# UBC-AWP/vision-sam3-yolo-lameless

Hardware: AMD Instinct MI355X
Metric: frames/sec (whole node) for YOLO+SAM3+DINOv3 feature extraction, 1080p clips (higher is better)
Workload: dtype f16; 1 GPU; BASELINE cfg#5, dense schedule: fused per-frame path on a synthetic 5 s @ 30 fps 1080p clip (150 unique BGR frames resident in HBM): YOLOv8-l detect (letterbox 384x640, NMS, scale_boxes; f16 plan) -> SAM (Hiera-B+ image encoder + FPN at 1024x1024, box-prompted mask decoder, 1080p mask + statistics + contour features) + DINOv3 ViT-L/16 embed (224x224) on EVERY frame; per-frame records packed, gathe; parallelism=one clip per GPU, 1 GPU(s), one gather per step, streams=7

## Files before the change

### include/lmx.h

```cpp
#ifndef LMX_H
#define LMX_H
#include <stdint.h>
#ifdef __cplusplus
extern "C" {
#endif

#define LMX_VERSION 100

#define LMX_OK 0
#define LMX_EINVAL (-1)
#define LMX_EHIP (-2)

typedef void* lmx_stream_t;

int lmx_version(void);
const char* lmx_last_error(void);
int lmx_device_count(void);

enum { LMX_F16 = 0, LMX_F32 = 1 };
enum { LMX_ACT_NONE = 0, LMX_ACT_SILU = 1, LMX_ACT_GELU = 2 , LMX_ACT_RELU = 3,
       LMX_ACT_SWIGLU = 4  };

typedef struct {
  const void* A;
  const void* W;
  const float* bias;
  const float* scale;
  const void* res;
  void* C;
  int64_t lda, ldc, ldr;
  int32_t M, N, K;
  int32_t act;
  int32_t out_dtype;
  int32_t a_mode;
  int32_t H, W_, Cin, conv_stride, Ho, Wo;
  int32_t res_rows;
  int32_t a_rep;
  int32_t split_k;
  int64_t split_stride;
  void* ln_out;
  const float* ln_gamma;
  const float* ln_beta;
  int64_t ld_ln;
  float ln_eps;
} lmx_gemm_desc;
int lmx_k_gemm(const lmx_gemm_desc* d, lmx_stream_t stream);
void lmx_dbg_set_gemm2_variant(int v);
int lmx_h_gemm_route(const lmx_gemm_desc* d, char* name, int cap);

int lmx_k_layernorm(const void* x, int in_dtype, int64_t ldx, const float* gamma, const float* beta,
                    void* y, int out_dtype, int64_t ldy, int rows, int D, float eps, int act, lmx_stream_t stream);
int lmx_h_layernorm_route(int in_dtype, int out_dtype, int rows, int D, int act, char* name, int cap);

int lmx_k_swiglu(const void* gu, int64_t ldg, void* out, int64_t ldo, int rows, int I, lmx_stream_t stream);

int lmx_k_hiera_attn8(const void* h, float* x, int64_t ldx, const float* gamma, const float* beta, float eps, const void* wqkv_p,
                      const float* bqkv_p, const void* wo_p, const float* bo, int n_img, int Gh, int Gw, int D, int heads, float scale,
                      lmx_stream_t stream);

int lmx_k_hiera_attn4(const void* h, float* x, int64_t ldx, const void* w_img, const float* bias, int n_img, int Gh, int Gw, int D,
                      int heads, float scale, lmx_stream_t stream);

int lmx_k_hiera_attn_pool(const void* h, float* out, const void* w_img, const float* bias, int n_img, int Gh, int Gw, int Din, int Dout,
                          int heads, float scale, lmx_stream_t stream);

int lmx_k_ln_mlp(float* x, int64_t ldx, const float* gamma, const float* beta, const void* w1, const float* b1,
                 const void* w2, const float* b2, int64_t rows, int D, float eps, void* workspace, void* x16,
                 const float* gamma_next, const float* beta_next, void* h_next, lmx_stream_t stream);
int lmx_k_ln_mlp_img(float* x, int64_t ldx, const void* w_img, const float* bias, int64_t rows, int D, float eps, void* x16, void* h_next,
                     lmx_stream_t stream);

typedef struct {
  const void* Q; const void* K; const void* V; void* O;
  int64_t ldq, ldk, ldv, ldo;
  int32_t B, H, Tq, Tk, hd;
  float scale;
  int32_t mode;
  int32_t Gh, Gw, ws, q_stride;
  const void* pad_k; const void* pad_v;
  const void* rel; int32_t rel_S;
} lmx_attn_desc;
int lmx_k_attention(const lmx_attn_desc* d, lmx_stream_t stream);
int lmx_h_attn_route(const lmx_attn_desc* d, char* name, int cap);
int lmx_k_relpos_tables(const lmx_attn_desc* d, const float* rel_pos_h, const float* rel_pos_w, int S, void* out,
                        lmx_stream_t stream);

int lmx_k_rope(void* x, int64_t ld, int B, int T, int H, int hd, int n_prefix, const float* cos_t,
               const float* sin_t, lmx_stream_t stream);

int lmx_k_pil_resize_h(const uint8_t* src, uint8_t* dst, int n, int sh, int sw, int dw, const int32_t* bounds,
                       const int32_t* kk, int ksize, int swap_rb, lmx_stream_t stream);
int lmx_k_pil_resize_v(const uint8_t* src, uint8_t* dst, int n, int sh, int dh, int w, const int32_t* bounds,
                       const int32_t* kk, int ksize, lmx_stream_t stream);

int lmx_k_patchify_norm(const uint8_t* img, void* out, int n, int ih, int iw, int top, int left, int gh, int gw,
                        int P, int64_t ldo, const float* lut, lmx_stream_t stream);

// ... 2 lines not shown
                                const float* kk_v, int ksize_v, int seg_cols, float rescale, const float* mean_std,
                                int swap_rb, lmx_stream_t stream);

int lmx_k_assemble_tokens(const void* patch_f16, const float* prefix, const float* pos, float* out, int B, int np,
                          int n_prefix, int D, lmx_stream_t stream);

int lmx_k_token_mean(const void* x, int in_dtype, float* out, int B, int T, int D, lmx_stream_t stream);

int64_t lmx_nms_workspace_bytes(int n, int A);
int lmx_k_nms(const float* pred, int n, int A, int nc, float conf, double iou, int max_det, float max_wh,
              float* boxes, float* scores, int32_t* cls, int32_t* src, int32_t* counts, void* workspace,
              lmx_stream_t stream);

int lmx_k_letterbox(const uint8_t* src, uint8_t* dst, int n, int sh, int sw, int rh, int rw, int top, int left,
                    int oh, int ow, const int32_t* xofs, const int16_t* ialpha, const int32_t* yofs,
                    const int16_t* ibeta, int swap_rb, lmx_stream_t stream);
int lmx_k_stem_conv(const uint8_t* img, const float* w, const float* bias, void* out, int n, int H, int W, int Cout,
                    lmx_stream_t stream);
int lmx_k_maxpool5(const void* src, int64_t lds, void* dst, int64_t ldd, int n, int H, int W, int C,
                   lmx_stream_t stream);
int lmx_k_upsample2(const void* src, int64_t lds, void* dst, int64_t ldd, int n, int H, int W, int C,
                    lmx_stream_t stream);
int lmx_k_detect_decode(const float* head, int64_t ldh, float* pred, int n, int H, int W, int nc, float stride,
                        int a_off, int A, lmx_stream_t stream);
int lmx_k_scale_boxes(float* boxes, int total, float padx, float pady, float gain, float w, float h,
                      lmx_stream_t stream);

int lmx_k_split3(const float* x, int64_t ldx, int act, const void* res3, int64_t ldr, void* out3, int64_t ldo, int64_t rows,
                 int N, int g, int nsum, int64_t sum_stride, lmx_stream_t stream);
int lmx_k_maxpool5_x3(const void* src3, int64_t lds, void* dst3, int64_t ldd, int n, int H, int W, int C, lmx_stream_t stream);
int lmx_k_stem_conv_x3(const uint8_t* img, const float* w, const float* bias, void* out3, int n, int H, int W, int Cout,
                       lmx_stream_t stream);
int lmx_k_attention_f32(const float* q, int64_t ldq, const float* k, int64_t ldk, const float* v, int64_t ldv, float* o,
                        int64_t ldo, int B, int H, int Tq, int Tk, int hd, float scale, lmx_stream_t stream);
int lmx_k_hyper_mask_f32(const float* up, const float* hyper, float* logits, int n, int G, int C, int act, lmx_stream_t stream);

int lmx_k_pose_gather(const float* raw0, const float* raw1, const float* raw2, int64_t ldk, const int32_t* hw,
                      const float* strides, const int32_t* src, const int32_t* counts, int n, int max_det, int K, int ndim,
                      float padx, float pady, float gain, float w, float h, float* out, lmx_stream_t stream);

int lmx_k_im2col_u8(const uint8_t* img, const float* lut, void* out, int n, int rh, int rw, int IH, int IW, int KH,
                    int KW, int stride, int pad, int64_t ldo, lmx_stream_t stream);
int lmx_k_maxpool2(const void* src, int64_t lds, void* dst, int64_t ldd, int dtype, int n, int H, int W, int C,
                   lmx_stream_t stream);
int lmx_k_cast_f32_f16(const float* src, int64_t lds, void* dst, int64_t ldd, int64_t rows, int cols,
                       lmx_stream_t stream);
int lmx_h_hiera_band(const int* window, const int* q_stride, int n_blocks, int grid, int nh, int nw, int* band);
int lmx_h_hiera_bands(const int* window, const int* q_stride, int n_blocks, int grid, int nh, int nw, int* rows);
int lmx_k_band_join(const void* band, const void* table, void* out, int dtype, int n, int H, int Hb, int W, int D,
                    lmx_stream_t stream);

int lmx_k_add_bcast(const void* a, int a_dtype, int64_t lda, const float* b, int64_t ldb, int b_rows, void* out,
                    int out_dtype, int64_t ldo, int64_t rows, int D, lmx_stream_t stream);
int lmx_k_prompt_box(const float* boxes, int64_t ldb, float* sparse, int n, double sx, double sy, float S,
                     const float* gauss, const float* corner, int F, lmx_stream_t stream);
int lmx_k_hyper_mask(const void* up, const float* hyper, float* logits, int n, int G, int C, lmx_stream_t stream);
int lmx_k_mask_post(const float* logits, int n, int L, int T, int nh, int nw, int h, int w, uint8_t* mask,
                    int64_t* stats, float* workspace, lmx_stream_t stream);
int lmx_k_prompt_points(const float* points, const int32_t* labels, int Np, const float* boxes, int64_t ldb, float* sparse, int n,
                        double sx, double sy, float S, const float* gauss, const float* point_embed, const float* not_a_point,
                        const float* corner, int F, lmx_stream_t stream);
#define LMX_MASK_EMBED_PARAMS 4684
int lmx_k_mask_embed(const float* mask_input, const void* emb, int emb_dtype, int64_t lde, const float* params, float* keys,
                     int64_t ldk, int n, int G, lmx_stream_t stream);
int lmx_k_hyper_mask_multi(const void* up, const float* hyper, float* logits, int n, int M, int G, int C, lmx_stream_t stream);
int lmx_k_hyper_mask_multi_f32(const float* up, const float* hyper, float* logits, int n, int M, int G, int C, int act,
                               lmx_stream_t stream);
int lmx_k_mask_logits(const float* logits, int n, int L, int T, int nh, int nw, int h, int w, float* out, lmx_stream_t stream);

int lmx_k_mask_score(const float* logits, int n, int L, int T, int nh, int nw, int h, int w, double thr, double off,
                     const int32_t* idx, int64_t* out, lmx_stream_t stream);
int lmx_k_nms_boxes(const float* boxes, int64_t ldb, const float* scores, const uint8_t* valid, int n, double iou, int32_t* keep_out,
                    int32_t* count_out, void* workspace, lmx_stream_t stream);
int lmx_k_pack_bits(const uint8_t* src, int64_t rows, int w, uint8_t* dst, lmx_stream_t stream);

int64_t lmx_contour_workspace_bytes(int n, int h, int w);
int lmx_k_contour_features(const uint8_t* mask, int n, int h, int w, int64_t* out, void* workspace, lmx_stream_t stream);

int lmx_h_mask_features(const uint8_t* mask_host, int h, int w, double* out_host);

int lmx_h_iou_matrix(const double* a, int n, const double* b, int m, double* out);
int lmx_h_assign(const double* cost, int n, int m, int* row_to_col, int* col_to_row);

enum { LMX_FILT_BILINEAR = 2, LMX_FILT_BICUBIC = 3 };
int lmx_h_pil_tables(int in_size, int out_size, int filt, int32_t* bounds_host, int32_t* kk_host, int64_t cap, int* ksize_host);
int lmx_h_aa_tables(int in_size, int out_size, int filt, int32_t* bounds_host, float* kk_host, int64_t cap, int* ksize_host);
int lmx_h_identity_table(int n, int32_t* bounds_host, int32_t* kk_host);
int lmx_h_segment_cols(const int32_t* bounds_host, int n_out, int tile);

typedef struct lmx_dino lmx_dino;
enum { LMX_DINO_V2 = 0, LMX_DINO_V3 = 1 };
enum { LMX_RECIPE_PIL = 0, LMX_RECIPE_FLOAT = 1 };
typedef struct { int32_t arch, hidden, heads, layers, tokens, image, patch, gated, recipe_kind, max_batch; } lmx_dino_info_t;
int lmx_dino_image_check_host(const char* path_host, lmx_dino_info_t* info_host);
int lmx_dino_open_host(const char* path_host, int max_batch, lmx_dino** out_host);
void lmx_dino_close(lmx_dino* m);
int lmx_dino_info(const lmx_dino* m, lmx_dino_info_t* info_host);
int lmx_dino_prepare(lmx_dino* m, int h, int w);
int lmx_dino_embed(lmx_dino* m, const uint8_t* frames, int n, int h, int w, int rgb, float* emb, lmx_stream_t stream);
int lmx_dino_embed_host(lmx_dino* m, const uint8_t* frames_host, int n, int h, int w, int rgb, float* emb_host);

typedef struct { int32_t sh, sw, rh, rw, top, left, oh, ow; double gain, pad_x, pad_y; } lmx_letterbox_geo_t;
int lmx_h_letterbox_geometry(int sh, int sw, int imgsz, int stride, int auto_, lmx_letterbox_geo_t* out_host);
int lmx_h_letterbox_tables(int sh, int sw, int rh, int rw, int32_t* xofs_host, int16_t* ialpha_host, int32_t* yofs_host, int16_t* ibeta_host);
int lmx_h_conv_split_k(int64_t px_per_frame, int N, int K, int cin);

// ... 22 lines not shown
```

### vision-sam3-yolo-lameless_amd/csrc/attn.hip

```cpp
#include "common.h"
#include <type_traits>
#include <stdlib.h>

#ifdef LMX_DBG_TIMELINE
__device__ unsigned long long lmx_attn_tl[64 * 8 * 8];
extern "C" int lmx_dbg_get_attn_timeline(void* host, int64_t bytes) { return (int)hipMemcpyFromSymbol(host, HIP_SYMBOL(lmx_attn_tl), bytes); }
#define ATL(i) if (blockIdx.x == 0 && lane == 0 && tl_it < 64) lmx_attn_tl[(tl_it * 8 + wave) * 8 + (i)] = __builtin_readcyclecounter()
#else
#define ATL(i)
#endif
namespace {

struct Geo {
  int mode, Tq, Tk, Gh, Gw, ws, nWy, nWx, Gqh, Gqw, wsq;
};

__device__ __forceinline__ int64_t key_row(const Geo& g, int b, int t) {
  if (g.mode == 0) return (int64_t)b * g.Tk + t;
  const int nW = g.nWy * g.nWx;
  const int img = b / nW;
  const int w = b - img * nW;
  const int wy = w / g.nWx, wx = w - wy * g.nWx;
  const int ty = t / g.ws, tx = t - ty * g.ws;
  const int y = wy * g.ws + ty, x = wx * g.ws + tx;
  if (y >= g.Gh || x >= g.Gw) return -1;
  return ((int64_t)img * g.Gh + y) * g.Gw + x;
}
__device__ __forceinline__ int64_t query_row(const Geo& g, int b, int t) {
  if (g.mode == 0) return (int64_t)b * g.Tq + t;
  const int nW = g.nWy * g.nWx;
  const int img = b / nW;
  const int w = b - img * nW;
  const int wy = w / g.nWx, wx = w - wy * g.nWx;
  const int ty = t / g.wsq, tx = t - ty * g.wsq;
  const int y = wy * g.wsq + ty, x = wx * g.wsq + tx;
  if (y >= g.Gqh || x >= g.Gqw) return -1;
  return ((int64_t)img * g.Gqh + y) * g.Gqw + x;
}

typedef __fp16 fp16x4_t __attribute__((__vector_size__(4 * sizeof(__fp16))));
typedef __attribute__((address_space(3))) fp16x4_t* lds_f16x4_ptr;

__device__ __forceinline__ half4_t lds_tr_read(const half_t* p) {
  const fp16x4_t v = __builtin_amdgcn_ds_read_tr16_b64_v4f16((lds_f16x4_ptr)(p));
  half4_t h;
  __builtin_memcpy(&h, &v, 8);
  return h;
}

typedef __attribute__((address_space(3))) const half8_t* lds_h8_cptr;
__device__ __forceinline__ unsigned lds_addr(const half_t* p) {
  unsigned a = (unsigned)(uintptr_t)(__attribute__((address_space(3))) const half_t*)p;
  asm volatile("" : "+v"(a));
  return a;
}
__device__ __forceinline__ half8_t lds_read8(unsigned base, int byte_off) { return *(lds_h8_cptr)(uintptr_t)(base + (unsigned)byte_off); }
__device__ __forceinline__ half4_t lds_tr_read_at(unsigned base, int byte_off) {
  const fp16x4_t v = __builtin_amdgcn_ds_read_tr16_b64_v4f16((lds_f16x4_ptr)(uintptr_t)(base + (unsigned)byte_off));
  half4_t h;
  __builtin_memcpy(&h, &v, 8);
  return h;
}

template <int QB, bool ONES, bool REL, bool DMA, int HDW>
__global__ __launch_bounds__(256, 2) void attn_kernel(const lmx_attn_desc p, const Geo geo, const int nQT) {
#ifndef LMX_ATTN_RING
#define LMX_ATTN_RING 3
#endif
  constexpr int NSL = DMA ? LMX_ATTN_RING : 2;
  constexpr int KS = HDW / 32;
  constexpr int NDB = HDW / 16;
  constexpr int RW = HDW <= 64 ? 64 : 128;
  constexpr int CPR = RW / 8;
  constexpr int NPASS = 64 * CPR / 256;
  static_assert(!(DMA && HDW != 64) && !(ONES && HDW != 64), "LDS-DMA ring and the ones column are built for 64-wide rows");
  __shared__ __attribute__((aligned(16))) half_t Ks[NSL][64 * RW];
  __shared__ __attribute__((aligned(16))) half_t Vs[NSL][64 * RW];
  static_assert(!(DMA && REL), "the relative-position bias is read from global memory inside the loop: vmcnt would not count DMAs only");

  const int tid = threadIdx.x, lane = tid & 63, wave = tid >> 6;
  const int fr = lane & 15, fg = lane >> 4;

  int bid;
  {
    const int n = gridDim.x, xcd = blockIdx.x & 7, idx = blockIdx.x >> 3, q = n >> 3, r = n & 7;
    bid = (xcd < r ? xcd * (q + 1) : r * (q + 1) + (xcd - r) * q) + idx;
  }
  const int nQTa = nQT < 0 ? -nQT : nQT;
  const int qt = bid % nQTa;
  bid /= nQTa;
  const int h = bid % p.H;
  const int b = bid / p.H;

  const half_t* Q = reinterpret_cast<const half_t*>(p.Q);
  const half_t* K = reinterpret_cast<const half_t*>(p.K);
  const half_t* V = reinterpret_cast<const half_t*>(p.V);
  const half_t* padk = reinterpret_cast<const half_t*>(p.pad_k);
  const half_t* padv = reinterpret_cast<const half_t*>(p.pad_v);
  half_t* O = reinterpret_cast<half_t*>(p.O);
  const int hd = p.hd;
  const half8_t zero8 = {0, 0, 0, 0, 0, 0, 0, 0};

  const int q_base = qt * (64 * QB) + wave * (16 * QB);
  half8_t qf[QB][KS];
  int64_t qrow[QB];
#pragma unroll
  for (int qb = 0; qb < QB; ++qb) {
    const int tq = q_base + qb * 16 + fr;
    qrow[qb] = (tq < p.Tq) ? query_row(geo, b, tq) : -1;
#pragma unroll
    for (int ks = 0; ks < KS; ++ks) {
      const int d = ks * 32 + fg * 8;
      const bool ok = qrow[qb] >= 0 && d < hd;
      const half8_t qv = *reinterpret_cast<const half8_t*>(Q + (ok ? qrow[qb] * p.ldq + (int64_t)h * hd + d : 0));
      qf[qb][ks] = ok ? qv : zero8;
    }
  }

  const half_t* relq[QB];
#pragma unroll
  for (int qb = 0; qb < QB; ++qb) {
    const int tq = q_base + qb * 16 + fr;
    relq[qb] = REL ? reinterpret_cast<const half_t*>(p.rel) + (((int64_t)b * p.H + h) * p.Tq + (tq < p.Tq ? tq : 0)) * (2 * p.rel_S)
                   : nullptr;
  }

  f32x4 oacc[QB][NDB];
  float m_run[QB], l_run[QB];
#pragma unroll
  for (int qb = 0; qb < QB; ++qb) {
    m_run[qb] = -INFINITY;
    l_run[qb] = 0.f;
#pragma unroll
    for (int db = 0; db < NDB; ++db) oacc[qb][db] = f32x4{0.f, 0.f, 0.f, 0.f};
  }

  const int sc = tid & (CPR - 1);
  const int sk = tid / CPR;
  constexpr int KPP = 256 / CPR;
  half8_t kst[NPASS], vst[NPASS];
  const int64_t hoff0 = (int64_t)h * hd + sc * 8;
  const half_t* Kb = K + hoff0 + (geo.mode == 0 ? (int64_t)b * p.Tk * p.ldk : 0);
  const half_t* Vb = V + hoff0 + (geo.mode == 0 ? (int64_t)b * p.Tk * p.ldv : 0);
  const bool d_ok = sc * 8 < hd;
  auto load_tile = [&](int t0) {
    if (geo.mode == 0) {
#pragma unroll
      for (int i = 0; i < NPASS; ++i) {
        const int t = t0 + sk + KPP * i;
        const bool in = d_ok && t < p.Tk;
        const int tt = in ? t : 0;
        const half8_t kv = *reinterpret_cast<const half8_t*>(Kb + (int64_t)tt * p.ldk);
        const half8_t vv = *reinterpret_cast<const half8_t*>(Vb + (int64_t)tt * p.ldv);
        kst[i] = in ? kv : zero8;
        vst[i] = in ? vv : zero8;
        if (ONES && sc == 7 && t < p.Tk) vst[i][7] = (half_t)1.0f;
      }
      return;
    }
#pragma unroll
    for (int i = 0; i < NPASS; ++i) {
      const int t = t0 + sk + KPP * i;
      const int d = sc * 8;
      const bool in = (t < p.Tk) && (d < hd);
      const int64_t row = key_row(geo, b, in ? t : 0);
      const bool pad = row < 0;
      const int64_t hoff = (int64_t)h * hd + d;
      const half_t* kp = pad ? (padk ? padk + hoff : K) : K + (in ? row * p.ldk + hoff : 0);
      const half_t* vp = pad ? (padv ? padv + hoff : V) : V + (in ? row * p.ldv + hoff : 0);
      const half8_t kv = *reinterpret_cast<const half8_t*>(kp);
      const half8_t vv = *reinterpret_cast<const half8_t*>(vp);
      kst[i] = (in && (!pad || padk)) ? kv : zero8;
      vst[i] = (in && (!pad || padv)) ? vv : zero8;
      if (ONES && sc == 7 && t < p.Tk) vst[i][7] = (half_t)1.0f;
    }
  };
  auto store_tile = [&](int buf) {
#pragma unroll
    for (int i = 0; i < NPASS; ++i) {
      const int kk = sk + KPP * i;
      const int off = kk * RW + ((sc ^ (kk & (CPR - 1))) << 3);
      *reinterpret_cast<half8_t*>(&Ks[buf][off]) = kst[i];
      *reinterpret_cast<half8_t*>(&Vs[buf][off]) = vst[i];
    }
  };

  const float sl2 = REL ? 1.44269504088896340736f : p.scale * 1.44269504088896340736f;
  const int ntile = (p.Tk + 63) / 64;
  const int q4 = fr >> 2, p4 = fr & 3;
  constexpr int LA = DMA ? NSL - 1 : 2, PT = 4;
  __amdgpu_buffer_rsrc_t k_rs, v_rs;
  unsigned kvo[2], vvo[2];
  if constexpr (DMA) {
    const int64_t kb = ((int64_t)(p.Tk - 1) * p.ldk + hd) * 2, vb = ((int64_t)(p.Tk - 1) * p.ldv + hd) * 2;
    k_rs = __builtin_amdgcn_make_buffer_rsrc(const_cast<half_t*>(K + (int64_t)b * p.Tk * p.ldk + (int64_t)h * hd), 0, (int)kb, 0x00020000);
    v_rs = __builtin_amdgcn_make_buffer_rsrc(const_cast<half_t*>(V + (int64_t)b * p.Tk * p.ldv + (int64_t)h * hd), 0, (int)vb, 0x00020000);
#pragma unroll
    for (int j = 0; j < 2; ++j) {
      const int row = (wave * 2 + j) * 8 + (lane >> 3);
      const int lc = (lane & 7) ^ (row & 7);
      const bool ok = lc * 8 < hd;
      kvo[j] = ok ? (unsigned)(row * (int)p.ldk * 2 + lc * 16) : 0x80000000u;
      vvo[j] = ok ? (unsigned)(row * (int)p.ldv * 2 + lc * 16) : 0x80000000u;
    }
  }
  auto issue = [&](int it, int slot) {
    const unsigned ko = (unsigned)(it * 64 * (int)p.ldk * 2), vo = (unsigned)(it * 64 * (int)p.ldv * 2);
#pragma unroll
    for (int j = 0; j < 2; ++j) {
      lds_dma16(k_rs, reinterpret_cast<char*>(&Ks[slot][0]) + (wave * 2 + j) * 1024, kvo[j] == 0x80000000u ? kvo[j] : kvo[j] + ko, 0);
      lds_dma16(v_rs, reinterpret_cast<char*>(&Vs[slot][0]) + (wave * 2 + j) * 1024, vvo[j] == 0x80000000u ? vvo[j] : vvo[j] + vo, 0);
    }
  };
  if constexpr (DMA) {
#pragma unroll
    for (int t = 0; t < LA; ++t)
      if (t < ntile) issue(t, t);
  } else {
    load_tile(0);
    store_tile(0);
    __syncthreads();
  }
  int k_lane[KS], v_lane[NDB];
#pragma unroll
  for (int ks = 0; ks < KS; ++ks) k_lane[ks] = fr * RW + ((((ks << 2) + fg) ^ (fr & (CPR - 1))) << 3);
#pragma unroll
  for (int db = 0; db < NDB; ++db) {
    const int chunk = db * 2 + (p4 >> 1), rl = fg * 4 + q4;
    v_lane[db] = rl * RW + ((chunk ^ (rl & (CPR - 1))) << 3) + (p4 & 1) * 4;
  }
  auto tile_body = [&](const int it, auto mask_tag) {
    constexpr bool MASK = decltype(mask_tag)::value;
    const int t0 = it * 64;
    int buf;
    if constexpr (DMA) {
      const int left = ntile - 1 - it;
      wait_tiles<PT>(left < LA - 1 ? left : LA - 1);
      __builtin_amdgcn_s_barrier();
      if (it + LA < ntile) issue(it + LA, (it + LA) % NSL);
      buf = it % NSL;
    } else {
      buf = it & 1;
      if (it + 1 < ntile) load_tile(t0 + 64);
    }

    unsigned kbase[KS], vbase[NDB];
#pragma unroll
    for (int ks = 0; ks < KS; ++ks) kbase[ks] = lds_addr(&Ks[buf][k_lane[ks]]);
#pragma unroll
    for (int db = 0; db < NDB; ++db) vbase[db] = lds_addr(&Vs[buf][v_lane[db]]);

    f32x4 sacc[QB][4];
#pragma unroll
    for (int qb = 0; qb < QB; ++qb)
#pragma unroll
      for (int kb = 0; kb < 4; ++kb) sacc[qb][kb] = f32x4{0.f, 0.f, 0.f, 0.f};
#pragma unroll
    for (int ks = 0; ks < KS; ++ks) {
#pragma unroll
      for (int kb = 0; kb < 4; ++kb) {
        const half8_t kf = lds_read8(kbase[ks], kb * 16 * RW * 2);
#pragma unroll
        for (int qb = 0; qb < QB; ++qb)
          sacc[qb][kb] = __builtin_amdgcn_mfma_f32_16x16x32_f16(kf, qf[qb][ks], sacc[qb][kb], 0, 0, 0);
      }
    }

    half8_t pf[QB][2];
#pragma unroll
    for (int qb = 0; qb < QB; ++qb) {
      if (REL) {
        if (p.rel_S == 64) {
          const float by = (float)relq[qb][it];
#pragma unroll
          for (int kb = 0; kb < 4; ++kb) {
            const half4_t bx = *reinterpret_cast<const half4_t*>(relq[qb] + 64 + kb * 16 + fg * 4);
#pragma unroll
            for (int r = 0; r < 4; ++r) sacc[qb][kb][r] = fmaf(sacc[qb][kb][r], p.scale, by + (float)bx[r]);
          }
        } else {
#pragma unroll
          for (int kb = 0; kb < 4; ++kb)
#pragma unroll
            for (int r = 0; r < 4; ++r) {
              int key = t0 + kb * 16 + fg * 4 + r;
              key = key < p.Tk ? key : 0;
              const int ky = key / p.rel_S, kx = key - ky * p.rel_S;
              const float bias = (float)relq[qb][ky] + (float)relq[qb][p.rel_S + kx];
              sacc[qb][kb][r] = fmaf(sacc[qb][kb][r], p.scale, bias);
            }
        }
      }
      if (MASK) {
#pragma unroll
        for (int kb = 0; kb < 4; ++kb)
#pragma unroll
          for (int r = 0; r < 4; ++r)
            if (t0 + kb * 16 + fg * 4 + r >= p.Tk) sacc[qb][kb][r] = -INFINITY;
      }
      float mx = fmaxf(fmaxf(sacc[qb][0][0], sacc[qb][0][1]), fmaxf(sacc[qb][0][2], sacc[qb][0][3]));
#pragma unroll
      for (int kb = 1; kb < 4; ++kb)
        mx = fmaxf(mx, fmaxf(fmaxf(sacc[qb][kb][0], sacc[qb][kb][1]), fmaxf(sacc[qb][kb][2], sacc[qb][kb][3])));
      mx = fmaxf(mx, __shfl_xor(mx, 16, 64));
      mx = fmaxf(mx, __shfl_xor(mx, 32, 64));
      const float m_new = fmaxf(m_run[qb], mx);
      const bool grew = nQT < 0 || __builtin_amdgcn_ballot_w64(m_new > m_run[qb]) != 0;
      const float alpha = grew ? __builtin_amdgcn_exp2f((m_run[qb] - m_new) * sl2) : 1.0f;
      m_run[qb] = m_new;
      const float mb = m_new * sl2;
      float rs = 0.f;
      const half2_t ones2 = {(half_t)1.0f, (half_t)1.0f};
#pragma unroll
      for (int kb = 0; kb < 4; ++kb)
#pragma unroll
        for (int r = 0; r < 4; r += 2) {
          const float e0 = __builtin_amdgcn_exp2f(fmaf(sacc[qb][kb][r], sl2, -mb));
          const float e1 = __builtin_amdgcn_exp2f(fmaf(sacc[qb][kb][r + 1], sl2, -mb));
          const half2_t e = {(half_t)e0, (half_t)e1};
          if (!ONES) rs = __builtin_amdgcn_fdot2(e, ones2, rs, false);
          pf[qb][kb >> 1][(kb & 1) * 4 + r] = e[0];
          pf[qb][kb >> 1][(kb & 1) * 4 + r + 1] = e[1];
        }
      if (!ONES) l_run[qb] = l_run[qb] * alpha + rs;
      if (grew) {
#pragma unroll
        for (int db = 0; db < NDB; ++db) oacc[qb][db] *= alpha;
      }
    }

#pragma unroll
    for (int ks = 0; ks < 2; ++ks) {
#pragma unroll
      for (int db = 0; db < NDB; ++db) {
        const half4_t lo = lds_tr_read_at(vbase[db], ks * 32 * RW * 2);
        const half4_t hi = lds_tr_read_at(vbase[db], (ks * 32 + 16) * RW * 2);
        half8_t vf = {lo[0], lo[1], lo[2], lo[3], hi[0], hi[1], hi[2], hi[3]};
        if (DMA && ONES && db == 3) {
          const half_t one = (half_t)1.0f;
          const half8_t ones8 = {one, one, one, one, one, one, one, one};
          vf = fr == 15 ? ones8 : vf;
        }
#pragma unroll
        for (int qb = 0; qb < QB; ++qb)
          oacc[qb][db] = __builtin_amdgcn_mfma_f32_16x16x32_f16(vf, pf[qb][ks], oacc[qb][db], 0, 0, 0);
      }
    }

    if constexpr (!DMA) {
      if (it + 1 < ntile) store_tile(buf ^ 1);
      __syncthreads();
    }
  };
  for (int it = 0; it + 1 < ntile; ++it) tile_body(it, std::false_type{});
  if (p.Tk & 63)
    tile_body(ntile - 1, std::true_type{});
  else
    tile_body(ntile - 1, std::false_type{});

#pragma unroll
  for (int qb = 0; qb < QB; ++qb) {
    float l;
    if (ONES) {
      l = __shfl(oacc[qb][3][3], 48 + fr, 64);
    } else {
      l = l_run[qb];
      l += __shfl_xor(l, 16, 64);
      l += __shfl_xor(l, 32, 64);
    }
    const float inv = 1.0f / l;
    if (qrow[qb] < 0) continue;
#pragma unroll
    for (int db = 0; db < NDB; ++db) {
      const int d = db * 16 + fg * 4;
      if (d >= hd) continue;
      half4_t o;
#pragma unroll
      for (int r = 0; r < 4; ++r) o[r] = (half_t)(oacc[qb][db][r] * inv);
      *reinterpret_cast<half4_t*>(O + qrow[qb] * p.ldo + (int64_t)h * hd + d) = o;
    }
  }
}


__device__ __forceinline__ float vmax3(float a, float b, float c) {
  return __builtin_amdgcn_fmed3f(__builtin_amdgcn_fmed3f(a, b, INFINITY), c, INFINITY);
}
__device__ __forceinline__ float row_max4(float ma, float mc) {
  typedef unsigned u32x2 __attribute__((ext_vector_type(2)));
  const unsigned u = __builtin_bit_cast(unsigned, fmaxf(ma, mc));
  const u32x2 a = __builtin_amdgcn_permlane16_swap(u, u, false, false);
  const unsigned a0 = a[0], a1 = a[1];
  const unsigned u1 = __builtin_bit_cast(unsigned, fmaxf(__builtin_bit_cast(float, a0), __builtin_bit_cast(float, a1)));
  const u32x2 b = __builtin_amdgcn_permlane32_swap(u1, u1, false, false);
  const unsigned b0 = b[0], b1 = b[1];
  return fmaxf(__builtin_bit_cast(float, b0), __builtin_bit_cast(float, b1));
}

#ifndef LMX_GP_DBG
#define LMX_GP_DBG 0
#endif
typedef unsigned u32x2_t __attribute__((ext_vector_type(2)));
typedef unsigned u32x4_t __attribute__((ext_vector_type(4)));
template <bool ONES, int NWV>
__global__ __launch_bounds__(NWV * 64, 2) void attn_gp_kernel(const lmx_attn_desc p, const int nQT) {
  constexpr int QB = 2, NSL = 3, RW = 64, NJ = 8 / NWV, PT = 2 * NJ;
  extern __shared__ __attribute__((aligned(16))) char smem[];
  half_t (*Ks)[64 * RW] = reinterpret_cast<half_t (*)[64 * RW]>(smem);
  half_t (*Vs)[64 * RW] = reinterpret_cast<half_t (*)[64 * RW]>(smem + NSL * 64 * RW * 2);
  const int tid = threadIdx.x, lane = tid & 63, wave = tid >> 6;
  const int fr = lane & 15, fg = lane >> 4;
// ... 881 lines not shown
        const float inv = 1.0f / l;
        if (qrow[qb] < 0) continue;
#pragma unroll
        for (int db = 0; db < 4; ++db) {
          const int d = db * 16 + fg * 4;
          if (d >= hd) continue;
          half4_t o;
#pragma unroll
          for (int r = 0; r < 4; ++r) o[r] = (half_t)(oacc[qb][db][r] * inv);
          *reinterpret_cast<half4_t*>(O + qrow[qb] * p.ldo + (int64_t)h * hd + d) = o;
        }
      }
      ATL(7);
    } else {
      asm volatile("s_waitcnt vmcnt(0)" ::: "memory");
      ATL(7);
    }
  }
}

}

static int build_geo(const lmx_attn_desc& d, Geo& g);

extern "C" int lmx_k_relpos_tables(const lmx_attn_desc* dp, const float* rel_pos_h, const float* rel_pos_w, int S, void* out,
                                   lmx_stream_t stream) {
  LMX_REQUIRE(dp && rel_pos_h && rel_pos_w && out, "lmx_k_relpos_tables: null pointer");
  const lmx_attn_desc& d = *dp;
  LMX_REQUIRE(d.Q && d.B > 0 && d.H > 0 && d.Tq > 0 && d.hd % 8 == 0 && d.hd <= 96 && d.ldq % 8 == 0 && aligned16(d.Q),
              "lmx_k_relpos_tables: descriptor");
  LMX_REQUIRE(S > 0 && S * S == d.Tq, "lmx_k_relpos_tables: S=%d vs Tq=%d", S, d.Tq);
  Geo g{};
  const int rc = build_geo(d, g);
  if (rc) return rc;
  const int64_t items = (int64_t)d.B * d.H * 2 * S;
  const int64_t grid = (items + 3) / 4;
  LMX_REQUIRE(grid < (1ll << 31) && aligned16(rel_pos_h) && aligned16(rel_pos_w), "lmx_k_relpos_tables: size / alignment");
  hipStream_t st = reinterpret_cast<hipStream_t>(stream);
  if (d.hd <= 64)
    hipLaunchKernelGGL((relpos_tables_kernel<2>), dim3((unsigned)grid), dim3(256), 0, st, d, g, rel_pos_h, rel_pos_w, S,
                       reinterpret_cast<half_t*>(out), items);
  else
    hipLaunchKernelGGL((relpos_tables_kernel<3>), dim3((unsigned)grid), dim3(256), 0, st, d, g, rel_pos_h, rel_pos_w, S,
                       reinterpret_cast<half_t*>(out), items);
  return lmx_launch_check("relpos_tables_kernel");
}

enum AttnKernel { ATTN_SMALL, ATTN_SP, ATTN_SPP, ATTN_GP, ATTN_TILED };
struct AttnRoute {
  AttnKernel kernel;
  int QB = 1;
  bool ONES = false, REL = false, DMA = false;
  int HDW = 64, NWV = 4;
  unsigned grid = 0, block = 256;
  int lds = 0;
  int arg = 0;
};

static int attn_route(const lmx_attn_desc* dp, AttnRoute& r, Geo& g) {
  LMX_REQUIRE(dp != nullptr, "lmx_k_attention: null descriptor");
  const lmx_attn_desc& d = *dp;
  LMX_REQUIRE(d.Q && d.K && d.V && d.O, "lmx_k_attention: null Q/K/V/O");
  LMX_REQUIRE(d.B > 0 && d.H > 0 && d.Tq > 0 && d.Tk > 0, "lmx_k_attention: empty problem");
  LMX_REQUIRE(d.hd % 8 == 0 && d.hd > 0 && d.hd <= 96, "lmx_k_attention: head dim %d (need multiple of 8, <=96)", d.hd);
  LMX_REQUIRE(d.ldq % 8 == 0 && d.ldk % 8 == 0 && d.ldv % 8 == 0 && d.ldo % 4 == 0, "lmx_k_attention: strides");
  LMX_REQUIRE(aligned16(d.Q) && aligned16(d.K) && aligned16(d.V) && ((((uintptr_t)d.O) & 7) == 0),
              "lmx_k_attention: alignment");
  LMX_TRY(build_geo(d, g));
  static const int no_sp = lmx_env_set("LMX_ATTN_NO_SP"), sp_qb = lmx_env_int("LMX_ATTN_SP_QB", 2), no_spp = lmx_env_set("LMX_ATTN_NO_SPP");
  static const int no_dma = lmx_env_set("LMX_ATTN_NO_DMA"), no_lazy = lmx_env_set("LMX_ATTN_NO_LAZY");
  static const int no_gp = lmx_env_set("LMX_ATTN_NO_GP");
  static const int gp_waves = lmx_env_int("LMX_ATTN_GP_WAVES", 4);

  r = AttnRoute{};
  r.ONES = d.hd <= 56;
  const int64_t items = (int64_t)d.B * d.H;
  const bool narrow = !d.rel && d.hd <= 64;
  if (narrow && d.Tq <= 16 && d.Tk <= 16) {
    LMX_REQUIRE(items < (1ll << 31), "lmx_k_attention: grid too large");
    r.kernel = ATTN_SMALL;
    r.ONES = false;
    r.grid = (unsigned)((items + 3) / 4);
    r.arg = (int)items;
    return LMX_OK;
  }
  if (!no_sp && narrow && d.Tk > 128 && d.Tk <= 208 && d.Tq > 64 && d.Tq <= 208) {
    LMX_REQUIRE(items < (1ll << 31), "lmx_k_attention: grid too large");
    r.grid = (unsigned)items;
    if (!no_spp && items >= 64 && (d.mode == 0 || (d.pad_k && d.pad_v))) {
      r.kernel = ATTN_SPP;
      r.block = 512;
      r.lds = 2 * 3 * 208 * 64 * 2;
      r.arg = (int)items;
    } else {
      r.kernel = ATTN_SP;
      r.QB = sp_qb == 2 ? 2 : 1;
    }
    return LMX_OK;
  }
  const bool wide = d.hd > 64;
  const bool big = d.Tq > 64 && !wide;
  const int nQT = (d.Tq + (big ? 128 : 64) - 1) / (big ? 128 : 64);
  const int64_t nblk = items * nQT;
  LMX_REQUIRE(nblk < (1ll << 31), "lmx_k_attention: grid too large");
  if (d.rel)
    LMX_REQUIRE(d.rel_S > 0 && d.rel_S * d.rel_S == d.Tk && d.Tq == d.Tk, "lmx_k_attention: rel_S=%d does not match Tq=%d Tk=%d",
                d.rel_S, d.Tq, d.Tk);
  const bool dma = !no_dma && !wide && d.mode == 0 && !d.rel && big && d.Tk >= 256 && (int64_t)d.Tk * d.ldk * 2 < 0x7fff0000ll &&
                   (int64_t)d.Tk * d.ldv * 2 < 0x7fff0000ll;
  if (dma && !no_gp) {
    r.kernel = ATTN_GP;
    r.NWV = gp_waves == 8 ? 8 : 4;
    const int nQTw = (d.Tq + r.NWV * 32 - 1) / (r.NWV * 32);
    r.grid = (unsigned)(items * nQTw);
    r.block = r.NWV * 64;
    r.lds = 2 * 3 * 64 * 64 * 2;
    r.arg = no_lazy ? -nQTw : nQTw;
    return LMX_OK;
  }
  r.kernel = ATTN_TILED;
  r.QB = big ? 2 : 1;
  r.ONES = r.ONES && !d.rel;
  r.REL = d.rel != nullptr;
  r.DMA = dma;
  r.HDW = wide ? 96 : 64;
  r.grid = (unsigned)nblk;
  r.arg = no_lazy ? -nQT : nQT;
  return LMX_OK;
}

static constexpr int attn_key(int kernel, int QB, bool ONES, bool REL, bool DMA, int HDW, int NWV) {
  return (((((kernel * 4 + QB) * 2 + ONES) * 2 + REL) * 2 + DMA) * 128 + HDW) * 16 + NWV;
}

extern "C" int lmx_k_attention(const lmx_attn_desc* dp, lmx_stream_t stream) {
  AttnRoute r;
  Geo g{};
  LMX_TRY(attn_route(dp, r, g));
  const lmx_attn_desc& d = *dp;
  hipStream_t st = reinterpret_cast<hipStream_t>(stream);
  const dim3 block(r.block);
  dim3 grid(r.grid);
  if (r.kernel == ATTN_SPP) {
    int dev;
    LMX_TRY(lmx_stream_device(st, &dev));
    LMX_TRY(lmx_allow_lds(reinterpret_cast<const void*>(&attn_spp_kernel<true>), r.lds, dev));
    LMX_TRY(lmx_allow_lds(reinterpret_cast<const void*>(&attn_spp_kernel<false>), r.lds, dev));
    LMX_TRY(lmx_persistent_grid(r.grid, dev, &grid.x));
  }
#define LMX_SP(QB, ONES) \
  case attn_key(ATTN_SP, QB, ONES, false, false, 64, 4): hipLaunchKernelGGL((attn_sp_kernel<QB, ONES>), grid, block, 0, st, d, g); break
#define LMX_SPP(ONES) \
  case attn_key(ATTN_SPP, 1, ONES, false, false, 64, 4): hipLaunchKernelGGL((attn_spp_kernel<ONES>), grid, block, r.lds, st, d, g, r.arg); break
#define LMX_GP(ONES, NWV) \
  case attn_key(ATTN_GP, 1, ONES, false, false, 64, NWV): hipLaunchKernelGGL((attn_gp_kernel<ONES, NWV>), grid, block, r.lds, st, d, r.arg); break
#define LMX_TILED(QB, ONES, REL, DMA, HDW) \
  case attn_key(ATTN_TILED, QB, ONES, REL, DMA, HDW, 4): hipLaunchKernelGGL((attn_kernel<QB, ONES, REL, DMA, HDW>), grid, block, 0, st, d, g, r.arg); break
  switch (attn_key(r.kernel, r.QB, r.ONES, r.REL, r.DMA, r.HDW, r.NWV)) {
    case attn_key(ATTN_SMALL, 1, false, false, false, 64, 4): hipLaunchKernelGGL(attn_small_kernel, grid, block, 0, st, d, g, r.arg); break;
    LMX_SPP(true);
    LMX_SPP(false);
    LMX_SP(2, true);
    LMX_SP(1, true);
    LMX_SP(2, false);
    LMX_SP(1, false);
    LMX_TILED(1, false, true, false, 96);
    LMX_TILED(2, false, true, false, 64);
    LMX_TILED(1, false, true, false, 64);
    LMX_TILED(1, false, false, false, 96);
    LMX_GP(true, 8);
    LMX_GP(true, 4);
    LMX_GP(false, 8);
    LMX_GP(false, 4);
    LMX_TILED(2, true, false, true, 64);
    LMX_TILED(2, false, false, true, 64);
    LMX_TILED(2, true, false, false, 64);
    LMX_TILED(2, false, false, false, 64);
    LMX_TILED(1, true, false, false, 64);
    LMX_TILED(1, false, false, false, 64);
    default: LMX_REQUIRE(false, "lmx_k_attention: no kernel for route %d", (int)r.kernel);
  }
#undef LMX_SP
#undef LMX_SPP
#undef LMX_GP
#undef LMX_TILED
  static const char* const what[] = {"attn_small_kernel", "attn_sp_kernel", "attn_spp_kernel", "attn_gp_kernel", "attn_kernel"};
  return lmx_launch_check(what[r.kernel]);
}

extern "C" int lmx_h_attn_route(const lmx_attn_desc* dp, char* name, int cap) {
  AttnRoute r;
  Geo g{};
  LMX_TRY(attn_route(dp, r, g));
  const char* sums = r.ONES ? "ones" : "dot2";
  switch (r.kernel) {
    case ATTN_SMALL: LMX_ROUTE_NAME(name, cap, "small"); break;
    case ATTN_SP: LMX_ROUTE_NAME(name, cap, "sp_qb%d_%s", r.QB, sums); break;
    case ATTN_SPP: LMX_ROUTE_NAME(name, cap, "spp_%s", sums); break;
    case ATTN_GP: LMX_ROUTE_NAME(name, cap, "gp%d_%s", r.NWV, sums); break;
    case ATTN_TILED:
      LMX_ROUTE_NAME(name, cap, "tiled_q%d_%s%s%s_hd%d", r.QB, sums, r.REL ? "_rel" : "", r.DMA ? "_dma" : "", r.HDW);
      break;
  }
  return LMX_OK;
}

static int build_geo(const lmx_attn_desc& d, Geo& g) {
  g.mode = d.mode;
  g.Tq = d.Tq;
  g.Tk = d.Tk;
  if (d.mode == 1) {
    LMX_REQUIRE(d.ws > 0 && d.Gh > 0 && d.Gw > 0, "lmx_k_attention: window geometry");
    const int qs = d.q_stride > 0 ? d.q_stride : 1;
    LMX_REQUIRE(qs == 1 || qs == 2, "lmx_k_attention: q_stride %d", qs);
    LMX_REQUIRE(d.ws % qs == 0 && d.Gh % qs == 0 && d.Gw % qs == 0, "lmx_k_attention: q_stride must divide ws/Gh/Gw");
    g.Gh = d.Gh;
    g.Gw = d.Gw;
    g.ws = d.ws;
    g.nWy = (d.Gh + d.ws - 1) / d.ws;
    g.nWx = (d.Gw + d.ws - 1) / d.ws;
    g.Gqh = d.Gh / qs;
    g.Gqw = d.Gw / qs;
    g.wsq = d.ws / qs;
    LMX_REQUIRE(d.Tk == d.ws * d.ws && d.Tq == g.wsq * g.wsq, "lmx_k_attention: Tq/Tk do not match window size");
    LMX_REQUIRE(d.B % (g.nWy * g.nWx) == 0, "lmx_k_attention: B=%d not a multiple of windows per image %d", d.B,
                g.nWy * g.nWx);
    if (d.pad_k) LMX_REQUIRE(aligned16(d.pad_k), "lmx_k_attention: pad_k alignment");
    if (d.pad_v) LMX_REQUIRE(aligned16(d.pad_v), "lmx_k_attention: pad_v alignment");
  } else {
    LMX_REQUIRE(d.mode == 0, "lmx_k_attention: bad mode %d", d.mode);
  }
  return LMX_OK;
}
```

### vision-sam3-yolo-lameless_amd/csrc/gemm.hip

```cpp
#include "common.h"
#include <stdlib.h>

namespace {

constexpr int BK = 64;

template <int BM, int BN, int AMODE, int OUT_DT>
__global__ __launch_bounds__(256, 2) void gemm_kernel(const lmx_gemm_desc p) {
  extern __shared__ __attribute__((aligned(16))) char smem[];
  half_t* As = reinterpret_cast<half_t*>(smem);
  half_t* Ws = As + 2 * BM * BK;
  constexpr int FM = BM / 32;
  constexpr int FN = BN / 32;
  constexpr int AI = BM / 32;
  constexpr int WI = BN / 32;

  const int tid = threadIdx.x;
  const int lane = tid & 63;
  const int wave = tid >> 6;
  const int wm = wave & 1, wn = wave >> 1;

  const int nwg = gridDim.x;
  const int bid = blockIdx.x;
  const int q = nwg >> 3, r = nwg & 7, xcd = bid & 7;
// ... 174 lines not shown
#pragma unroll
        for (int e = 0; e < 4; ++e) v[e] = __fmul_rn(v[e], s[e]);
      }
      if (OUT_DT == LMX_F32) {
        float* C = reinterpret_cast<float*>(p.C);
        if (p.res) {
          const f32x4 rr = *reinterpret_cast<const f32x4*>(reinterpret_cast<const float*>(p.res) + (int64_t)mr * p.ldr + n);
#pragma unroll
          for (int e = 0; e < 4; ++e) v[e] = __fadd_rn(v[e], rr[e]);
        }
        *reinterpret_cast<f32x4*>(C + (int64_t)m * p.ldc + n) = v;
      } else {
        half_t* C = reinterpret_cast<half_t*>(p.C);
        if (p.res) {
          const half4_t rr =
              *reinterpret_cast<const half4_t*>(reinterpret_cast<const half_t*>(p.res) + (int64_t)mr * p.ldr + n);
#pragma unroll
          for (int e = 0; e < 4; ++e) v[e] = __fadd_rn((float)(half_t)v[e], (float)rr[e]);
        }
        half4_t o;
#pragma unroll
        for (int e = 0; e < 4; ++e) o[e] = (half_t)v[e];
        *reinterpret_cast<half4_t*>(C + (int64_t)m * p.ldc + n) = o;
      }
    }
  }
}

template <int BM, int BN, int AMODE, int OUT_DT>
int launch(const lmx_gemm_desc& d, hipStream_t st) {
  const int MT = (d.M + BM - 1) / BM, NT = (d.N + BN - 1) / BN;
  const size_t smem = (size_t)2 * (BM + BN) * BK * sizeof(half_t);
  int dev;
  LMX_TRY(lmx_stream_device(st, &dev));
  LMX_TRY(lmx_allow_lds(reinterpret_cast<const void*>(&gemm_kernel<BM, BN, AMODE, OUT_DT>), (int)smem, dev));
  hipLaunchKernelGGL((gemm_kernel<BM, BN, AMODE, OUT_DT>), dim3(MT * NT), dim3(256), smem, st, d);
  return lmx_launch_check("gemm_kernel");
}

}

GemmRoute lmx_gemm2_tiling(const lmx_gemm_desc& d);
int lmx_gemm2_launch(const lmx_gemm_desc& d, const GemmRoute& r, hipStream_t st);

static bool dma_ok(const lmx_gemm_desc& d, int m_min, int n_min) {
  const bool a_ok = d.a_mode != 1 || (d.Cin % 32 == 0 && d.H < 32768 && d.W_ < 32768);
  return a_ok && d.M >= m_min && d.N >= n_min && d.N % 8 == 0 && d.ldc % 8 == 0 && aligned16(d.C) &&
         (!d.res || (d.ldr % 8 == 0 && aligned16(d.res)));
}

static int gemm_route(const lmx_gemm_desc* dp, GemmRoute& r) {
  LMX_REQUIRE(dp != nullptr, "lmx_k_gemm: null descriptor");
  const lmx_gemm_desc& d = *dp;
  LMX_REQUIRE(d.A && d.W && d.C, "lmx_k_gemm: null A/W/C");
  LMX_REQUIRE(d.M > 0 && d.N > 0 && d.K > 0, "lmx_k_gemm: empty problem M=%d N=%d K=%d", d.M, d.N, d.K);
  LMX_REQUIRE(d.K % 8 == 0, "lmx_k_gemm: K=%d must be a multiple of 8", d.K);
  LMX_REQUIRE(d.N % 4 == 0, "lmx_k_gemm: N=%d must be a multiple of 4", d.N);
  LMX_REQUIRE(d.lda % 8 == 0, "lmx_k_gemm: lda=%lld must be a multiple of 8", (long long)d.lda);
  const bool gated = d.act == LMX_ACT_SWIGLU;
  LMX_REQUIRE(d.ldc % 4 == 0 && d.ldc >= (gated ? d.N / 2 : d.N), "lmx_k_gemm: bad ldc=%lld", (long long)d.ldc);
  LMX_REQUIRE(aligned16(d.A) && aligned16(d.W), "lmx_k_gemm: A/W must be 16-byte aligned");
  LMX_REQUIRE((((uintptr_t)d.C) & 7) == 0, "lmx_k_gemm: C must be 8-byte aligned");
  LMX_REQUIRE(d.out_dtype == LMX_F16 || d.out_dtype == LMX_F32, "lmx_k_gemm: bad out_dtype %d", d.out_dtype);
  LMX_REQUIRE(d.out_dtype == LMX_F16 || aligned16(d.C), "lmx_k_gemm: f32 C must be 16-byte aligned");
  LMX_REQUIRE(d.act >= LMX_ACT_NONE && d.act <= LMX_ACT_SWIGLU, "lmx_k_gemm: bad act %d", d.act);
  if (gated) {
    LMX_REQUIRE(d.N % 32 == 0, "lmx_k_gemm: LMX_ACT_SWIGLU: N=%d (gate + up rows, interleaved by 16) must be a multiple of 32", d.N);
    LMX_REQUIRE(!d.res, "lmx_k_gemm: LMX_ACT_SWIGLU takes no residual");
    LMX_REQUIRE(d.a_mode == 0 && d.a_rep <= 1 && d.split_k <= 1, "lmx_k_gemm: LMX_ACT_SWIGLU: dense A only (a_mode 0; no pooled rows, convolution, a_rep or split_k); a_mode=%d", d.a_mode);
    LMX_REQUIRE(d.out_dtype == LMX_F16, "lmx_k_gemm: LMX_ACT_SWIGLU writes f16 (one rounding of the f32 product)");
  }
  if (d.bias) LMX_REQUIRE(aligned16(d.bias), "lmx_k_gemm: bias must be 16-byte aligned");
  if (d.scale) LMX_REQUIRE(aligned16(d.scale), "lmx_k_gemm: scale must be 16-byte aligned");
  if (d.res) LMX_REQUIRE(d.ldr % 4 == 0 && d.ldr >= d.N, "lmx_k_gemm: bad ldr=%lld", (long long)d.ldr);
  LMX_REQUIRE(d.res_rows >= 0, "lmx_k_gemm: res_rows");
  if (d.a_mode == 0) {
    LMX_REQUIRE(d.a_rep > 1 || d.lda >= d.K, "lmx_k_gemm: lda=%lld < K=%d", (long long)d.lda, d.K);
  } else if (d.a_mode == 1) {
    LMX_REQUIRE(d.Cin > 0 && d.Cin % 8 == 0, "lmx_k_gemm: conv Cin=%d must be a multiple of 8", d.Cin);
    LMX_REQUIRE(d.K == 9 * d.Cin, "lmx_k_gemm: conv K=%d != 9*Cin=%d", d.K, 9 * d.Cin);
    LMX_REQUIRE(d.conv_stride == 1 || d.conv_stride == 2, "lmx_k_gemm: conv stride %d", d.conv_stride);
    LMX_REQUIRE(d.H > 0 && d.W_ > 0, "lmx_k_gemm: conv H/W");
    LMX_REQUIRE(d.Ho == (d.H + 2 - 3) / d.conv_stride + 1 && d.Wo == (d.W_ + 2 - 3) / d.conv_stride + 1,
                "lmx_k_gemm: conv Ho/Wo (%d,%d) inconsistent with H/W (%d,%d) stride %d", d.Ho, d.Wo, d.H, d.W_,
                d.conv_stride);
    LMX_REQUIRE(d.M % (d.Ho * d.Wo) == 0, "lmx_k_gemm: conv M=%d not a multiple of Ho*Wo", d.M);
    LMX_REQUIRE(d.lda >= d.Cin, "lmx_k_gemm: conv pixel stride lda=%lld < Cin=%d", (long long)d.lda, d.Cin);
  } else if (d.a_mode == 2) {
    LMX_REQUIRE(d.lda >= d.K, "lmx_k_gemm: lda=%lld < K=%d", (long long)d.lda, d.K);
    LMX_REQUIRE(d.H > 0 && d.W_ > 0 && d.H % 2 == 0 && d.W_ % 2 == 0 && d.M % (d.H * d.W_) == 0,
                "lmx_k_gemm: pooled rows need an even H x W token grid that divides M (H=%d W=%d M=%d)", d.H, d.W_, d.M);
    LMX_REQUIRE(!d.res && !d.scale && d.act == LMX_ACT_NONE, "lmx_k_gemm: pooled rows: no residual / scale / activation");
    LMX_REQUIRE(((int64_t)d.M * d.lda + d.K) * 2 < 0x7fffffffll, "lmx_k_gemm: pooled rows: A must be smaller than 2 GB");
    LMX_REQUIRE(dma_ok(d, 512, 96),
                "lmx_k_gemm: pooled rows are built for the LDS-DMA kernel (M >= 512, N >= 96, N %% 8 == 0): use GEMM + maxpool2 for M=%d N=%d", d.M, d.N);
  } else {
    LMX_REQUIRE(false, "lmx_k_gemm: bad a_mode %d", d.a_mode);
  }
  LMX_REQUIRE(d.a_rep >= 0 && d.a_rep <= 3, "lmx_k_gemm: a_rep=%d (0..3)", d.a_rep);
  LMX_REQUIRE(d.split_k >= 0 && d.split_k <= 64, "lmx_k_gemm: split_k=%d (0..64)", d.split_k);
  static const int v1 = lmx_env_char("LMX_GEMM_V1") == '1';
  static const int n64 = lmx_env_char("LMX_GEMM_N64") != '0';
  if (d.ln_out) {
    LMX_REQUIRE(d.out_dtype == LMX_F32 && d.res && d.res_rows == 0, "lmx_k_gemm: ln_out needs f32 output with a full residual (out_dtype=%d res_rows=%d)", d.out_dtype, d.res_rows);
    LMX_REQUIRE(d.N <= 448 && d.N % 16 == 0 && d.K <= 448, "lmx_k_gemm: ln_out: a tile holds whole rows of N <= 448 (N %% 16 == 0) over K <= 448; N=%d K=%d", d.N, d.K);
    LMX_REQUIRE(d.a_mode == 0 && d.a_rep <= 1 && d.split_k <= 1, "lmx_k_gemm: ln_out: dense A only (a_mode=%d a_rep=%d split_k=%d)", d.a_mode, d.a_rep, d.split_k);
    LMX_REQUIRE(d.act == LMX_ACT_NONE && !d.scale, "lmx_k_gemm: ln_out takes no activation and no scale");
    LMX_REQUIRE(d.ln_gamma && d.ln_beta && aligned16(d.ln_gamma) && aligned16(d.ln_beta), "lmx_k_gemm: ln_gamma / ln_beta must be given, 16-byte aligned");
    LMX_REQUIRE(d.ld_ln % 4 == 0 && d.ld_ln >= d.N && (((uintptr_t)d.ln_out) & 7) == 0, "lmx_k_gemm: ln_out must be 8-byte aligned with ld_ln=%lld a multiple of 4, >= N", (long long)d.ld_ln);
    LMX_REQUIRE(aligned16(d.res), "lmx_k_gemm: ln_out: the residual must be 16-byte aligned");
    r = GemmRoute{true, 128, 448, BK, 2, 0, true};
    return LMX_OK;
  }
  bool dma;
  if (d.split_k > 1) {
    LMX_REQUIRE(d.out_dtype == LMX_F32 && d.act == LMX_ACT_NONE && d.a_mode != 2 && d.a_rep <= 1, "lmx_k_gemm: split_k needs f32 output, no activation, a_mode 0 or 1");
    LMX_REQUIRE(d.split_stride >= (int64_t)(d.M - 1) * d.ldc + d.N && d.split_stride % 4 == 0, "lmx_k_gemm: split_stride=%lld", (long long)d.split_stride);
    LMX_REQUIRE((d.K + 63) / 64 >= d.split_k, "lmx_k_gemm: split_k=%d exceeds the k-tiles of K=%d", d.split_k, d.K);
    LMX_REQUIRE(dma_ok(d, 1, 64),
                "lmx_k_gemm: split_k is built into the LDS-DMA kernel only (N >= 64, N %% 8 == 0; conv: Cin %% 32 == 0); M=%d N=%d", d.M, d.N);
    dma = true;
  } else if (d.a_rep > 1) {
    LMX_REQUIRE(d.a_mode == 0 && d.K % d.a_rep == 0 && (d.K / d.a_rep) % 64 == 0, "lmx_k_gemm: a_rep=%d needs a_mode 0 and K / a_rep a multiple of 64 (K=%d)", d.a_rep, d.K);
    LMX_REQUIRE(d.lda >= d.K / d.a_rep, "lmx_k_gemm: lda=%lld < K / a_rep", (long long)d.lda);
    LMX_REQUIRE(dma_ok(d, 512, 96),
                "lmx_k_gemm: a_rep is built into the LDS-DMA kernel only (M >= 512, N >= 96, N %% 8 == 0); M=%d N=%d", d.M, d.N);
    dma = true;
  } else if (d.a_mode == 2) {
    dma = true;
  } else {
    dma = !v1 && dma_ok(d, 512, d.a_mode == 1 && n64 && d.M >= 65536 ? 64 : 96);
  }
  if (dma) {
    r = lmx_gemm2_tiling(d);
  } else {
    const bool narrow = d.N <= 64 || (d.N < 128 && d.N % 128 != 0);
    r = GemmRoute{false, 128, narrow ? 64 : 128, BK, 2, 0};
  }
  return LMX_OK;
}

static constexpr int v1_key(int BN, int a_mode, int out_dtype) { return BN * 4 + a_mode * 2 + out_dtype; }

extern "C" int lmx_k_gemm(const lmx_gemm_desc* dp, lmx_stream_t stream) {
  GemmRoute r;
  LMX_TRY(gemm_route(dp, r));
  const lmx_gemm_desc& d = *dp;
  hipStream_t st = reinterpret_cast<hipStream_t>(stream);
  if (r.dma) return lmx_gemm2_launch(d, r, st);
#define LMX_V1(BN, AMODE, OUT_DT) \
  case v1_key(BN, AMODE, OUT_DT): return launch<128, BN, AMODE, OUT_DT>(d, st)
  switch (v1_key(r.BN, d.a_mode, d.out_dtype)) {
    LMX_V1(64, 0, LMX_F16);
    LMX_V1(128, 0, LMX_F16);
    LMX_V1(64, 0, LMX_F32);
    LMX_V1(128, 0, LMX_F32);
    LMX_V1(64, 1, LMX_F16);
    LMX_V1(128, 1, LMX_F16);
    LMX_V1(64, 1, LMX_F32);
    LMX_V1(128, 1, LMX_F32);
  }
#undef LMX_V1
  LMX_REQUIRE(false, "lmx_k_gemm: no register-staged kernel 128x%d for a_mode %d, out_dtype %d", r.BN, d.a_mode, d.out_dtype);
// ... 14 lines not shown
```

### vision-sam3-yolo-lameless_amd/csrc/gemm2.hip

```cpp
#include "common.h"
#include <stdlib.h>
#include <type_traits>

#ifdef LMX_DBG_TIMELINE
__device__ unsigned long long lmx_tl[8 * 16384];
extern "C" int lmx_dbg_get_timeline(void* host, int64_t bytes) { return (int)hipMemcpyFromSymbol(host, HIP_SYMBOL(lmx_tl), bytes); }
#define TL(i, v) if (threadIdx.x == 0 && swz < 16384) lmx_tl[swz * 8 + (i)] = (v)
#else
#define TL(i, v)
#endif
namespace lmx_gemm2 {

__device__ __forceinline__ float act_apply(float v, int act) { return lmx_act(v, act); }

constexpr int smem_bytes(int BM, int BN, int BK, int NSTAGE) { return NSTAGE * (BM + BN) * BK * 2 + 2 * BN * 4; }
constexpr int waves_per_simd(int BM, int BN, int BK, int NSTAGE) {
  const int smem = smem_bytes(BM, BN, BK, NSTAGE), nwave = (BM / 64) * (BN / 64);
  const int wps = (smem <= 80 * 1024 ? 2 : 1) * nwave / 4;
  return wps < 1 ? 1 : wps;
}
template <int OUT_DT, int BM, int BN, int BK, int NSTAGE, int AMODE, int STAG, bool GATED = false>
__global__ __launch_bounds__(waves_per_simd(BM, BN, BK, NSTAGE) * 256) void gemm2_kernel(const lmx_gemm_desc p, const int ntiles, const int nt_ok) {
  constexpr int NWAVE = (BM / 64) * (BN / 64);
  constexpr int STAGE_BYTES = (BM + BN) * BK * 2;
// ... 408 lines not shown
    }
  }
  __builtin_amdgcn_s_barrier();
  TL(4, wall_clock64());
  }
}

template <int BM, int BN, int BK, int NSTAGE, int AMODE, int STAG = 0>
int launch2(const lmx_gemm_desc& d, hipStream_t st) {
  const int MT = (d.M + BM - 1) / BM, NT = (d.N + BN - 1) / BN;
  const size_t smem = smem_bytes(BM, BN, BK, NSTAGE);
  int dev;
  LMX_TRY(lmx_stream_device(st, &dev));
  LMX_TRY(lmx_allow_lds(reinterpret_cast<const void*>(&gemm2_kernel<LMX_F16, BM, BN, BK, NSTAGE, AMODE, STAG>), (int)smem, dev));
  LMX_TRY(lmx_allow_lds(reinterpret_cast<const void*>(&gemm2_kernel<LMX_F32, BM, BN, BK, NSTAGE, AMODE, STAG>), (int)smem, dev));
  const int ntiles = MT * NT * (d.split_k > 1 ? d.split_k : 1);
  int grid = ntiles;
  static const int persist = lmx_env_int("LMX_GEMM2_PERSIST", 0);
  static const int nt_ok = !lmx_env_set("LMX_GEMM2_NO_NT");
  if (persist > 0 && grid > 256 * persist) grid = 256 * persist;
  if (d.act == LMX_ACT_SWIGLU) {
    if constexpr (AMODE == 0) {
      LMX_TRY(lmx_allow_lds(reinterpret_cast<const void*>(&gemm2_kernel<LMX_F16, BM, BN, BK, NSTAGE, AMODE, STAG, true>), (int)smem, dev));
      hipLaunchKernelGGL((gemm2_kernel<LMX_F16, BM, BN, BK, NSTAGE, AMODE, STAG, true>), dim3(grid), dim3(BM * BN / 64), smem, st, d, ntiles, nt_ok);
      return lmx_launch_check("gemm2_kernel (gated)");
    } else {
      return LMX_EINVAL;
    }
  }
  if (d.out_dtype == LMX_F16)
    hipLaunchKernelGGL((gemm2_kernel<LMX_F16, BM, BN, BK, NSTAGE, AMODE, STAG>), dim3(grid), dim3(BM * BN / 64), smem, st, d, ntiles, nt_ok);
  else
    hipLaunchKernelGGL((gemm2_kernel<LMX_F32, BM, BN, BK, NSTAGE, AMODE, STAG>), dim3(grid), dim3(BM * BN / 64), smem, st, d, ntiles, nt_ok);
  return lmx_launch_check("gemm2_kernel");
}

constexpr int RL_BM = 128, RL_BN = 448, RL_BK = 64, RL_NSTAGE = 2;
constexpr int RL_STAGE_BYTES = (RL_BM + RL_BN) * RL_BK * 2;
constexpr int RL_RS = RL_BN + 4;
constexpr int RL_SMEM = RL_NSTAGE * RL_STAGE_BYTES + 3 * RL_BN * 4;
static_assert(2 * 32 * RL_RS * 4 <= RL_NSTAGE * RL_STAGE_BYTES, "two 32-row epilogue buffers inside the ring");

__device__ __forceinline__ void wave_sum4(float (&v)[4]) {
#pragma unroll
  for (int o = 32; o > 0; o >>= 1) {
    float t[4];
#pragma unroll
    for (int r = 0; r < 4; ++r) t[r] = __shfl_xor(v[r], o, 64);
#pragma unroll
    for (int r = 0; r < 4; ++r) v[r] += t[r];
  }
}

__global__ __launch_bounds__(512) void gemm2_rowln_kernel(const lmx_gemm_desc p) {
  constexpr int BM = RL_BM, BN = RL_BN, BK = RL_BK, NSTAGE = RL_NSTAGE, STAGE_BYTES = RL_STAGE_BYTES;
  constexpr int NWAVE = 8;
  constexpr int A_INSTR = BM * BK * 2 / 1024 / NWAVE;
  constexpr int W_INSTR = BN * BK * 2 / 1024 / NWAVE;
  constexpr int FJ = BN / 4 / 16;
  extern __shared__ __attribute__((aligned(16))) char smem[];
  const int tid = threadIdx.x;
  const int lane = tid & 63;
  const int wave = __builtin_amdgcn_readfirstlane(tid >> 6);
  const int wm = wave & 1, wn = wave >> 1;
  const int swz = blockIdx.x;
  const int m0 = swz * BM;
  TL(0, (unsigned long long)__builtin_amdgcn_s_getreg((31 << 11) | 4));
  TL(1, (unsigned long long)__builtin_amdgcn_s_getreg((31 << 11) | 20));
  TL(2, wall_clock64());
  TL(5, (unsigned long long)swz);

  const char* Ab = reinterpret_cast<const char*>(p.A) + (int64_t)m0 * p.lda * 2;
  int64_t a_bytes = ((int64_t)(p.M - m0 - 1) * p.lda + p.K) * 2;
  if (a_bytes > 0x7FFFFFF0ll) a_bytes = 0x7FFFFFF0ll;
  const int w_bytes = p.N * p.K * 2;
  const __amdgpu_buffer_rsrc_t a_rs = __builtin_amdgcn_make_buffer_rsrc(const_cast<char*>(Ab), 0, (int)a_bytes, 0x00020000);
  const __amdgpu_buffer_rsrc_t w_rs = __builtin_amdgcn_make_buffer_rsrc(const_cast<void*>(p.W), 0, w_bytes, 0x00020000);

  const int lrow = lane >> 3;
  const int lchunk = (lane & 7) ^ lrow;
  unsigned a_off[A_INSTR], w_off[W_INSTR];
#pragma unroll
  for (int j = 0; j < A_INSTR; ++j) a_off[j] = (unsigned)(((wave * A_INSTR + j) * 8 + lrow) * (int)p.lda * 2 + lchunk * 16);
#pragma unroll
  for (int j = 0; j < W_INSTR; ++j) w_off[j] = (unsigned)(((wave * W_INSTR + j) * 8 + lrow) * p.K * 2 + lchunk * 16);
  const unsigned OOB = 0x80000000u;
  const int nk = (p.K + BK - 1) / BK;
  const bool k_tail_lane = (nk - 1) * BK + lchunk * 8 >= p.K;
  auto issue = [&](int kt, int slot) {
    char* st = smem + slot * STAGE_BYTES;
    const bool kill = (kt == nk - 1) && k_tail_lane;
    const int soff = kt * (BK * 2);
#pragma unroll
    for (int j = 0; j < A_INSTR; ++j) lds_dma16(a_rs, st + (wave * A_INSTR + j) * 1024, kill ? OOB : a_off[j], soff);
#pragma unroll
    for (int j = 0; j < W_INSTR; ++j) lds_dma16(w_rs, st + BM * BK * 2 + (wave * W_INSTR + j) * 1024, kill ? OOB : w_off[j], soff);
  };

  f32x4 acc[4][FJ];
#pragma unroll
  for (int i = 0; i < 4; ++i)
#pragma unroll
    for (int j = 0; j < FJ; ++j) acc[i][j] = f32x4{0.f, 0.f, 0.f, 0.f};

  float* bl = reinterpret_cast<float*>(smem + NSTAGE * STAGE_BYTES);
  float bias_v = 0.f, gamma_v = 0.f, beta_v = 0.f;
  if (tid < p.N) {
    if (p.bias) bias_v = p.bias[tid];
    gamma_v = p.ln_gamma[tid];
    beta_v = p.ln_beta[tid];
  }

  issue(0, 0);
  const int frow = lane & 15, fq = lane >> 4;
  const int fsw = frow & 7;
  for (int kt = 0; kt < nk; ++kt) {
    wait_vmcnt<0>();
    __builtin_amdgcn_s_barrier();
    if (kt + 1 < nk) issue(kt + 1, (kt + 1) % NSTAGE);
    const char* st = smem + (kt % NSTAGE) * STAGE_BYTES;
    const half_t* as = reinterpret_cast<const half_t*>(st) + (wm * 64 + frow) * BK;
    const half_t* ws = reinterpret_cast<const half_t*>(st + BM * BK * 2) + (wn * (BN / 4) + frow) * BK;
#pragma unroll
    for (int ks = 0; ks < BK / 32; ++ks) {
      const int coff = (((ks << 2) + fq) ^ fsw) << 3;
      half8_t af[4], wf[FJ];
#pragma unroll
      for (int j = 0; j < FJ; ++j) wf[j] = *reinterpret_cast<const half8_t*>(ws + j * 16 * BK + coff);
#pragma unroll
      for (int i = 0; i < 4; ++i) af[i] = *reinterpret_cast<const half8_t*>(as + i * 16 * BK + coff);
      __builtin_amdgcn_s_setprio(1);
#pragma unroll
      for (int i = 0; i < 4; ++i)
#pragma unroll
        for (int j = 0; j < FJ; ++j)
          acc[i][j] = __builtin_amdgcn_mfma_f32_16x16x32_f16(wf[j], af[i], acc[i][j], 0, 0, 0);
      __builtin_amdgcn_s_setprio(0);
    }
  }

  if (tid < BN) {
    bl[tid] = bias_v;
    bl[BN + tid] = gamma_v;
    bl[2 * BN + tid] = beta_v;
  }
  asm volatile("s_waitcnt lgkmcnt(0)" ::: "memory");
  __builtin_amdgcn_s_barrier();
  TL(3, wall_clock64());

  const int D = p.N;
  const int c0 = lane * 4, c1 = (64 + lane) * 4;
  const bool ok0 = c0 < D, ok1 = c1 < D;
  const f32x4 z4 = {0.f, 0.f, 0.f, 0.f};
  const f32x4 g0 = ok0 ? *reinterpret_cast<const f32x4*>(bl + BN + c0) : z4, g1 = ok1 ? *reinterpret_cast<const f32x4*>(bl + BN + c1) : z4;
  const f32x4 b0 = ok0 ? *reinterpret_cast<const f32x4*>(bl + 2 * BN + c0) : z4, b1 = ok1 ? *reinterpret_cast<const f32x4*>(bl + 2 * BN + c1) : z4;
  const float* blj = bl + wn * (BN / 4) + fq * 4;
  const float* res = reinterpret_cast<const float*>(p.res);
  float* Cf = reinterpret_cast<float*>(p.C);
  half_t* Lh = reinterpret_cast<half_t*>(p.ln_out);
#pragma unroll
  for (int ps = 0; ps < 4; ++ps) {
    float* buf = reinterpret_cast<float*>(smem) + (ps & 1) * 32 * RL_RS;
    f32x4 r0[4], r1[4];
#pragma unroll
    for (int rr = 0; rr < 4; ++rr) {
      const int lr = wave * 4 + rr;
      const int m = m0 + (lr >> 4) * 64 + ps * 16 + (lr & 15);
      r0[rr] = r1[rr] = z4;
      if (m < p.M) {
        if (ok0) r0[rr] = *reinterpret_cast<const f32x4*>(res + (int64_t)m * p.ldr + c0);
        if (ok1) r1[rr] = *reinterpret_cast<const f32x4*>(res + (int64_t)m * p.ldr + c1);
      }
    }
#pragma unroll
    for (int j = 0; j < FJ; ++j)
      *reinterpret_cast<f32x4*>(buf + (wm * 16 + frow) * RL_RS + wn * (BN / 4) + j * 16 + fq * 4) = acc[ps][j] + *reinterpret_cast<const f32x4*>(blj + j * 16);
    asm volatile("s_waitcnt lgkmcnt(0)" ::: "memory");
    __builtin_amdgcn_s_barrier();
    f32x4 v0[4], v1[4];
    float s[4], q[4], mean[4], rstd[4];
#pragma unroll
    for (int rr = 0; rr < 4; ++rr) {
      const int lr = wave * 4 + rr;
      const f32x4 t0 = *reinterpret_cast<const f32x4*>(buf + lr * RL_RS + (ok0 ? c0 : 0)), t1 = *reinterpret_cast<const f32x4*>(buf + lr * RL_RS + (ok1 ? c1 : 0));
      v0[rr] = (ok0 ? t0 : z4) + r0[rr];
      v1[rr] = (ok1 ? t1 : z4) + r1[rr];
      s[rr] = 0.f;
      s[rr] += (v0[rr][0] + v0[rr][1]) + (v0[rr][2] + v0[rr][3]);
      s[rr] += (v1[rr][0] + v1[rr][1]) + (v1[rr][2] + v1[rr][3]);
    }
    wave_sum4(s);
#pragma unroll
    for (int rr = 0; rr < 4; ++rr) {
      mean[rr] = s[rr] / (float)D;
      q[rr] = 0.f;
      {
        const f32x4 dlt = v0[rr] - mean[rr];
        const float t = (dlt[0] * dlt[0] + dlt[1] * dlt[1]) + (dlt[2] * dlt[2] + dlt[3] * dlt[3]);
        q[rr] += ok0 ? t : 0.f;
      }
      {
        const f32x4 dlt = v1[rr] - mean[rr];
        const float t = (dlt[0] * dlt[0] + dlt[1] * dlt[1]) + (dlt[2] * dlt[2] + dlt[3] * dlt[3]);
        q[rr] += ok1 ? t : 0.f;
      }
    }
    wave_sum4(q);
#pragma unroll
    for (int rr = 0; rr < 4; ++rr) {
      const int lr = wave * 4 + rr;
      const int m = m0 + (lr >> 4) * 64 + ps * 16 + (lr & 15);
      rstd[rr] = 1.0f / sqrtf(q[rr] / (float)D + p.ln_eps);
      if (m < p.M) {
        if (ok0) *reinterpret_cast<f32x4*>(Cf + (int64_t)m * p.ldc + c0) = v0[rr];
        if (ok1) *reinterpret_cast<f32x4*>(Cf + (int64_t)m * p.ldc + c1) = v1[rr];
        if (ok0) {
          const f32x4 o = (v0[rr] - mean[rr]) * rstd[rr] * g0 + b0;
          *reinterpret_cast<half4_t*>(Lh + (int64_t)m * p.ld_ln + c0) = half4_t{(half_t)o[0], (half_t)o[1], (half_t)o[2], (half_t)o[3]};
        }
        if (ok1) {
          const f32x4 o = (v1[rr] - mean[rr]) * rstd[rr] * g1 + b1;
          *reinterpret_cast<half4_t*>(Lh + (int64_t)m * p.ld_ln + c1) = half4_t{(half_t)o[0], (half_t)o[1], (half_t)o[2], (half_t)o[3]};
        }
      }
    }
  }
  TL(4, wall_clock64());
}

int launch_rowln(const lmx_gemm_desc& d, hipStream_t st) {
  int dev;
  LMX_TRY(lmx_stream_device(st, &dev));
  LMX_TRY(lmx_allow_lds(reinterpret_cast<const void*>(&gemm2_rowln_kernel), RL_SMEM, dev));
  hipLaunchKernelGGL(gemm2_rowln_kernel, dim3((d.M + RL_BM - 1) / RL_BM), dim3(512), RL_SMEM, st, d);
  return lmx_launch_check("gemm2_rowln_kernel");
}

}
using namespace lmx_gemm2;

static int g_variant = -1;
extern "C" void lmx_dbg_set_gemm2_variant(int v) { g_variant = v; }

static constexpr GemmRoute tiling(int BM, int BN, int BK, int NSTAGE, int STAG = 0) { return GemmRoute{true, BM, BN, BK, NSTAGE, STAG}; }

GemmRoute lmx_gemm2_tiling(const lmx_gemm_desc& d) {
  if (g_variant < 0) g_variant = lmx_env_char("LMX_GEMM2_VARIANT");
  if (d.a_mode == 2) return tiling(256, 256, 64, 2);
  if (d.a_mode == 1) {
    static const int conv_small = lmx_env_set("LMX_GEMM2_CONV_SMALL");
    const int64_t t256 = (int64_t)((d.M + 255) / 256) * ((d.N + 255) / 256);
    const double q256 = (double)t256 / (double)(((t256 + 255) / 256) * 256);
    if (!conv_small && d.N % 256 == 0 && t256 >= 230 && q256 >= 0.75) return tiling(256, 256, 32, 3, 1);
    return tiling(256, 128, 32, 3);
  }
  switch (g_variant) {
    case 'A': return tiling(256, 128, 64, 3);
    case 'B': return tiling(128, 128, 64, 2);
    case 'C': return tiling(256, 128, 32, 3);
    case 'D': return tiling(256, 128, 32, 2);
    case 'E': return tiling(256, 256, 32, 3);
    case 'F': return tiling(256, 256, 32, 4);
    case 'H': return tiling(128, 128, 32, 2);
    case 'I': return tiling(128, 128, 32, 3);
    case 'S': return tiling(256, 128, 32, 6, 1);
    case 'T': return tiling(256, 128, 64, 3, 1);
    case 'U': return tiling(256, 128, 32, 3, 1);
    case 'V': return tiling(256, 128, 32, 4, 1);
    case 'W': return tiling(256, 256, 32, 4, 1);
    case 'Y': return tiling(256, 256, 32, 3, 1);
    case 'Z': return tiling(256, 256, 64, 2);
  }
  const int64_t nt256 = (d.N + 255) / 256, tiles256 = (int64_t)((d.M + 255) / 256) * nt256;
  const double nfrac = (double)d.N / (double)(nt256 * 256);
  const double q256 = (double)tiles256 / (double)(((tiles256 + 255) / 256) * 256);
  if (d.K >= 448 && tiles256 >= 200 && q256 >= 0.75 && nfrac >= 0.85) {
    return tiling(256, 256, 64, 2);
  }
  if (d.K < 448 && d.N >= 224 && d.N <= 1536 && d.N % 256 != 0 && nfrac >= 0.85 && tiles256 >= 200 && q256 >= 0.75)
    return d.K > 128 ? tiling(256, 256, 32, 3) : tiling(256, 256, 64, 2);
  const int64_t tiles = (int64_t)((d.M + 255) / 256) * ((d.N + 127) / 128);
  return (d.K >= 1792 || tiles <= 256) ? tiling(256, 128, 64, 3, 1) : tiling(256, 128, 32, 3);
}

static constexpr int64_t tiling_key(int BM, int BN, int BK, int NSTAGE, int a_mode, int STAG) {
  return ((((int64_t)BM * 1024 + BN) * 1024 + BK) * 16 + NSTAGE) * 16 + a_mode * 2 + STAG;
}
// ... 29 lines not shown
```

### vision-sam3-yolo-lameless_amd/csrc/sam.hip

```cpp
#include "common.h"

namespace {

inline int grid_for(int64_t total, int block = 256) {
  int64_t g = (total + block - 1) / block;
  if (g > 256 * 8) g = 256 * 8;
  if (g < 1) g = 1;
  return (int)g;
}

template <int KW_T>
__global__ __launch_bounds__(256) void im2col_u8_kernel(const uint8_t* __restrict__ img, const float* __restrict__ lut,
                                                        half_t* __restrict__ out, int n, int rh, int rw, int OH, int OW, int KH,
                                                        int KW_rt, int stride, int pad, int64_t ldo) {
  __shared__ float lut_s[768];
  for (int i = threadIdx.x; i < 768; i += blockDim.x) lut_s[i] = lut[i];
  __syncthreads();
  const int KW = KW_T > 0 ? KW_T : KW_rt;
  const int chunks = (int)(ldo / 8);
  const int K = KH * KW * 3;
  const int64_t total = (int64_t)n * OH * OW * chunks;
  for (int64_t i = (int64_t)blockIdx.x * blockDim.x + threadIdx.x; i < total; i += (int64_t)gridDim.x * blockDim.x) {
    const int ck = (int)(i % chunks);
    const int64_t tok = i / chunks;
// ... 42 lines not shown
    for (int e = 0; e < VEC; ++e) {
      T t0 = a0[e] > a1[e] ? a0[e] : a1[e];
      T t1 = a2[e] > a3[e] ? a2[e] : a3[e];
      m[e] = t0 > t1 ? t0 : t1;
    }
    *reinterpret_cast<vec_t*>(dst + p * ldd + c) = m;
  }
}

__global__ __launch_bounds__(256) void cast_kernel(const float* __restrict__ src, int64_t lds, half_t* __restrict__ dst, int64_t ldd,
                                                   int64_t rows, int cols) {
  const int cc = cols / 4;
  const int64_t total = rows * cc;
  for (int64_t i = (int64_t)blockIdx.x * blockDim.x + threadIdx.x; i < total; i += (int64_t)gridDim.x * blockDim.x) {
    const int c = (int)(i % cc) * 4;
    const int64_t r = i / cc;
    const f32x4 v = *reinterpret_cast<const f32x4*>(src + r * lds + c);
    half4_t h = {(half_t)v[0], (half_t)v[1], (half_t)v[2], (half_t)v[3]};
    *reinterpret_cast<half4_t*>(dst + r * ldd + c) = h;
  }
}

__global__ __launch_bounds__(256) void band_join_kernel(const u32x4* __restrict__ band, const u32x4* __restrict__ table,
                                                        u32x4* __restrict__ out, int64_t ci, int64_t cb) {
  const u32x4* bsrc = band + (int64_t)blockIdx.y * cb;
  u32x4* o = out + (int64_t)blockIdx.y * ci;
  for (int64_t i = (int64_t)blockIdx.x * blockDim.x + threadIdx.x; i < ci; i += (int64_t)gridDim.x * blockDim.x)
    o[i] = i < cb ? bsrc[i] : table[i - cb];
}

template <int IN_DT, int OUT_DT>
__global__ __launch_bounds__(256) void add_bcast_kernel(const void* __restrict__ av, int64_t lda, const float* __restrict__ b,
                                                        int64_t ldb, int b_rows, void* __restrict__ out, int64_t ldo, int64_t rows,
                                                        int D) {
  const int cc = D / 4;
  const int64_t total = rows * cc;
  for (int64_t i = (int64_t)blockIdx.x * blockDim.x + threadIdx.x; i < total; i += (int64_t)gridDim.x * blockDim.x) {
    const int c = (int)(i % cc) * 4;
    const int64_t r = i / cc;
    f32x4 v;
    if (IN_DT == LMX_F32) {
      v = *reinterpret_cast<const f32x4*>(reinterpret_cast<const float*>(av) + r * lda + c);
    } else {
      const half4_t hv = *reinterpret_cast<const half4_t*>(reinterpret_cast<const half_t*>(av) + r * lda + c);
      v = f32x4{(float)hv[0], (float)hv[1], (float)hv[2], (float)hv[3]};
    }
    v += *reinterpret_cast<const f32x4*>(b + (r % b_rows) * ldb + c);
    if (OUT_DT == LMX_F32) {
      *reinterpret_cast<f32x4*>(reinterpret_cast<float*>(out) + r * ldo + c) = v;
    } else {
      half4_t h = {(half_t)v[0], (half_t)v[1], (half_t)v[2], (half_t)v[3]};
      *reinterpret_cast<half4_t*>(reinterpret_cast<half_t*>(out) + r * ldo + c) = h;
    }
  }
}

__global__ __launch_bounds__(256) void hyper_mask_kernel(const half_t* __restrict__ up, const float* __restrict__ hyper,
                                                         float* __restrict__ logits, int n, int G, int C) {
  const int64_t total = (int64_t)n * G * G * 16;
  const int S = 4 * G;
  for (int64_t i = (int64_t)blockIdx.x * blockDim.x + threadIdx.x; i < total; i += (int64_t)gridDim.x * blockDim.x) {
    const int q2 = (int)(i & 3), q1 = (int)((i >> 2) & 3);
    const int64_t cell = i >> 4;
    const int x = (int)(cell % G);
    const int64_t r = cell / G;
    const int y = (int)(r % G);
    const int b = (int)(r / G);
    const half_t* u = up + i * C;
    const float* hy = hyper + (int64_t)b * C;
    float acc = 0.f;
    for (int c = 0; c < C; c += 8) {
      const half8_t v = *reinterpret_cast<const half8_t*>(u + c);
#pragma unroll
      for (int e = 0; e < 8; ++e) acc = fmaf((float)v[e], hy[c + e], acc);
    }
    const int Y = 4 * y + 2 * (q1 >> 1) + (q2 >> 1), X = 4 * x + 2 * (q1 & 1) + (q2 & 1);
    logits[((int64_t)b * S + Y) * S + X] = acc;
  }
}

template <int DBG>
__global__ __launch_bounds__(256) void mask_mid_kernel(const float* __restrict__ logits, float* __restrict__ mid, int n, int L,
                                                       int T, int nh, int nw, unsigned long long* dbg) {
  const float sLT = (float)L / (float)T;
  const int64_t total = (int64_t)n * nh * nw;
  for (int64_t i = (int64_t)blockIdx.x * blockDim.x + threadIdx.x; i < total; i += (int64_t)gridDim.x * blockDim.x) {
    const int X = (int)(i % nw);
    const int64_t r = i / nw;
    const int Y = (int)(r % nh);
    const int b = (int)(r / nh);
    mid[i] = sample_mid(logits + (int64_t)b * L * L, L, T, sLT, Y, X);
  }
  if (DBG == 2) {
    __threadfence();
    __syncthreads();
    if (threadIdx.x == 0) atomicAdd(&dbg[7], 1ull);
  }
  if (DBG == 3 || DBG == 5) __atomic_thread_fence(__ATOMIC_RELEASE);
}

template <int DBG>
__device__ __forceinline__ float ld_mid(const float* p) {
  if (DBG == 9) return __hip_atomic_load(p, __ATOMIC_RELAXED, __HIP_MEMORY_SCOPE_SYSTEM);
  if (DBG == 6) return __hip_atomic_load(p, __ATOMIC_RELAXED, __HIP_MEMORY_SCOPE_AGENT);
  if (DBG == 7) return __hip_atomic_load(p, __ATOMIC_RELAXED, __HIP_MEMORY_SCOPE_WORKGROUP);
  return *p;
// ... 258 lines not shown
    }
  }
  return LMX_OK;
}

extern "C" int lmx_k_band_join(const void* band, const void* table, void* out, int dtype, int n, int H, int Hb, int W, int D,
                               lmx_stream_t stream) {
  LMX_REQUIRE(band && table && out, "lmx_k_band_join: null pointer");
  LMX_REQUIRE(dtype == LMX_F16 || dtype == LMX_F32, "lmx_k_band_join: dtype %d", dtype);
  LMX_REQUIRE(n > 0 && n <= 65535 && H > 0 && W > 0 && D > 0, "lmx_k_band_join: n=%d H=%d W=%d D=%d", n, H, W, D);
  LMX_REQUIRE(Hb >= 1 && Hb <= H - 1, "lmx_k_band_join: Hb=%d outside 1 .. H - 1 = %d", Hb, H - 1);
  const int64_t row_bytes = (int64_t)D * (dtype == LMX_F32 ? 4 : 2);
  LMX_REQUIRE(row_bytes % 16 == 0, "lmx_k_band_join: a row of %lld bytes is not a multiple of 16", (long long)row_bytes);
  LMX_REQUIRE(aligned16(band) && aligned16(table) && aligned16(out), "lmx_k_band_join: alignment");
  const int64_t ci = (int64_t)H * W * (row_bytes / 16), cb = (int64_t)Hb * W * (row_bytes / 16);
  int gx = grid_for(ci);
  const int cap = 256 * 32 / n > 0 ? 256 * 32 / n : 1;
  if (gx > cap) gx = cap;
  hipLaunchKernelGGL(band_join_kernel, dim3(gx, n), dim3(256), 0, reinterpret_cast<hipStream_t>(stream),
                     reinterpret_cast<const u32x4*>(band), reinterpret_cast<const u32x4*>(table), reinterpret_cast<u32x4*>(out), ci, cb);
  return lmx_launch_check("band_join_kernel");
}

extern "C" int lmx_k_prompt_box(const float* boxes, int64_t ldb, float* sparse, int n, double sx, double sy, float S,
                                const float* gauss, const float* corner, int F, lmx_stream_t stream) {
  LMX_REQUIRE(boxes && sparse && gauss && corner && n > 0 && F > 0 && ldb >= 4 && S > 0.f, "lmx_k_prompt_box: arguments");
  hipLaunchKernelGGL(prompt_box_kernel, dim3((n * 2 * F + 255) / 256), dim3(256), 0, reinterpret_cast<hipStream_t>(stream), boxes, ldb,
                     sparse, n, sx, sy, S, gauss, corner, F);
  return lmx_launch_check("prompt_box_kernel");
}

extern "C" int lmx_k_add_bcast(const void* a, int a_dtype, int64_t lda, const float* b, int64_t ldb, int b_rows, void* out,
                               int out_dtype, int64_t ldo, int64_t rows, int D, lmx_stream_t stream) {
  LMX_REQUIRE(a && b && out, "lmx_k_add_bcast: null pointer");
  LMX_REQUIRE(rows > 0 && D > 0 && D % 4 == 0 && b_rows > 0 && lda >= D && ldb >= D && ldo >= D && lda % 4 == 0 && ldb % 4 == 0 &&
                  ldo % 4 == 0, "lmx_k_add_bcast: shape");
  LMX_REQUIRE(((((uintptr_t)a) & (a_dtype == LMX_F32 ? 15 : 7)) == 0) && aligned16(b) &&
                  ((((uintptr_t)out) & (out_dtype == LMX_F32 ? 15 : 7)) == 0), "lmx_k_add_bcast: alignment");
  hipStream_t st = reinterpret_cast<hipStream_t>(stream);
  const int g = grid_for(rows * (D / 4));
  if (a_dtype == LMX_F32 && out_dtype == LMX_F32)
    hipLaunchKernelGGL((add_bcast_kernel<LMX_F32, LMX_F32>), dim3(g), dim3(256), 0, st, a, lda, b, ldb, b_rows, out, ldo, rows, D);
  else if (a_dtype == LMX_F32 && out_dtype == LMX_F16)
    hipLaunchKernelGGL((add_bcast_kernel<LMX_F32, LMX_F16>), dim3(g), dim3(256), 0, st, a, lda, b, ldb, b_rows, out, ldo, rows, D);
  else if (a_dtype == LMX_F16 && out_dtype == LMX_F32)
    hipLaunchKernelGGL((add_bcast_kernel<LMX_F16, LMX_F32>), dim3(g), dim3(256), 0, st, a, lda, b, ldb, b_rows, out, ldo, rows, D);
  else if (a_dtype == LMX_F16 && out_dtype == LMX_F16)
    hipLaunchKernelGGL((add_bcast_kernel<LMX_F16, LMX_F16>), dim3(g), dim3(256), 0, st, a, lda, b, ldb, b_rows, out, ldo, rows, D);
  else
    LMX_REQUIRE(false, "lmx_k_add_bcast: dtypes %d -> %d", a_dtype, out_dtype);
  return lmx_launch_check("add_bcast_kernel");
}

extern "C" int lmx_k_hyper_mask(const void* up, const float* hyper, float* logits, int n, int G, int C, lmx_stream_t stream) {
  LMX_REQUIRE(up && hyper && logits, "lmx_k_hyper_mask: null pointer");
  LMX_REQUIRE(n > 0 && G > 0 && C > 0 && C % 8 == 0 && C <= 64 && aligned16(up), "lmx_k_hyper_mask: shape");
  hipLaunchKernelGGL(hyper_mask_kernel, dim3(grid_for((int64_t)n * G * G * 16)), dim3(256), 0, reinterpret_cast<hipStream_t>(stream),
                     reinterpret_cast<const half_t*>(up), hyper, logits, n, G, C);
  return lmx_launch_check("hyper_mask_kernel");
}

extern "C" int lmx_k_mask_post(const float* logits, int n, int L, int T, int nh, int nw, int h, int w, uint8_t* mask, int64_t* stats,
                               float* workspace, lmx_stream_t stream) {
  LMX_REQUIRE(logits && mask && stats && workspace, "lmx_k_mask_post: null pointer");
  LMX_REQUIRE(n > 0 && L > 0 && T >= L && nh > 0 && nw > 0 && nh <= T && nw <= T && h > 0 && w > 0 &&
                  (int64_t)h * ((w + 3) / 4) < 0x7fffffffll - 96 * 256 && n <= 65535, "lmx_k_mask_post: geometry");
  hipStream_t st = reinterpret_cast<hipStream_t>(stream);
  hipLaunchKernelGGL(mask_stats_init_kernel, dim3((n * 8 + 255) / 256), dim3(256), 0, st, reinterpret_cast<long long*>(stats), n);
  int gx = (int)(((int64_t)h * ((w + 3) / 4) + 255) / 256);
  if (gx > 96) gx = 96;
  const unsigned gmid = grid_for((int64_t)n * nh * nw);
  unsigned long long* su = reinterpret_cast<unsigned long long*>(stats);
#ifdef LMX_DBG_VARIANTS
  static const int dbg = lmx_env_int("LMX_DBG_MASK", 0);
#define LMX_MASK_VARIANT(M, P)                                                                                         \
  {                                                                                                                    \
    hipLaunchKernelGGL(mask_mid_kernel<M>, dim3(gmid), dim3(256), 0, st, logits, workspace, n, L, T, nh, nw, su);      \
    hipLaunchKernelGGL(mask_post_kernel<P>, dim3(gx, n), dim3(256), 0, st, workspace, n, nh, nw, h, w, mask, su, gmid); \
  }
  if (dbg == 2 && n >= 2) LMX_MASK_VARIANT(2, 2)
  else if (dbg == 3) LMX_MASK_VARIANT(3, 3)
  else if (dbg == 4) LMX_MASK_VARIANT(4, 4)
  else if (dbg == 5) LMX_MASK_VARIANT(5, 5)
  else if (dbg == 8) LMX_MASK_VARIANT(1, 8)
  else if (dbg == 6) LMX_MASK_VARIANT(1, 6)
  else if (dbg == 7) LMX_MASK_VARIANT(1, 7)
  else if (dbg == 1) LMX_MASK_VARIANT(1, 1)
  else if (dbg == 9) LMX_MASK_VARIANT(1, 9)
  else LMX_MASK_VARIANT(0, 0)
#undef LMX_MASK_VARIANT
#else
  hipLaunchKernelGGL(mask_mid_kernel<0>, dim3(gmid), dim3(256), 0, st, logits, workspace, n, L, T, nh, nw, su);
  hipLaunchKernelGGL(mask_post_kernel<0>, dim3(gx, n), dim3(256), 0, st, workspace, n, nh, nw, h, w, mask, su, gmid);
#endif
  return lmx_launch_check("mask_post_kernel");
}

extern "C" int lmx_k_pack_bits(const uint8_t* src, int64_t rows, int w, uint8_t* dst, lmx_stream_t stream) {
  LMX_REQUIRE(src && dst, "lmx_k_pack_bits: null pointer");
  LMX_REQUIRE(rows > 0 && w > 0, "lmx_k_pack_bits: rows=%lld w=%d", (long long)rows, w);
  const int wb = (w + 7) / 8;
  hipLaunchKernelGGL(pack_bits_kernel, dim3(grid_for(rows * wb)), dim3(256), 0, reinterpret_cast<hipStream_t>(stream), src, rows, w, wb, dst);
  return lmx_launch_check("pack_bits_kernel");
}
```

### vision-sam3-yolo-lameless_amd/lmx/_lib.py

```python
import ctypes as C
import os

_HERE = os.path.dirname(os.path.abspath(__file__))
LIB_PATH = os.environ.get("LMX_LIB") or os.path.join(_HERE, "liblmx.so")


class LmxError(RuntimeError):
    pass


class GemmDesc(C.Structure):
    _fields_ = [
        ("A", C.c_void_p), ("W", C.c_void_p), ("bias", C.c_void_p), ("scale", C.c_void_p), ("res", C.c_void_p),
        ("C", C.c_void_p),
        ("lda", C.c_int64), ("ldc", C.c_int64), ("ldr", C.c_int64),
        ("M", C.c_int32), ("N", C.c_int32), ("K", C.c_int32),
        ("act", C.c_int32), ("out_dtype", C.c_int32), ("a_mode", C.c_int32),
        ("H", C.c_int32), ("W_", C.c_int32), ("Cin", C.c_int32), ("conv_stride", C.c_int32),
        ("Ho", C.c_int32), ("Wo", C.c_int32), ("res_rows", C.c_int32), ("a_rep", C.c_int32), ("split_k", C.c_int32), ("split_stride", C.c_int64),
        ("ln_out", C.c_void_p), ("ln_gamma", C.c_void_p), ("ln_beta", C.c_void_p), ("ld_ln", C.c_int64), ("ln_eps", C.c_float),
    ]


class DinoInfo(C.Structure):
    _fields_ = [(n, C.c_int32) for n in ("arch", "hidden", "heads", "layers", "tokens", "image", "patch", "gated", "recipe_kind", "max_batch")]


class YoloInfo(C.Structure):
    _fields_ = [(n, C.c_int32) for n in ("scale", "nc", "imgsz", "kpt_k", "kpt_ndim", "plans", "max_batch")]


class LetterboxGeo(C.Structure):
    _fields_ = [(n, C.c_int32) for n in ("sh", "sw", "rh", "rw", "top", "left", "oh", "ow")] + [(n, C.c_double) for n in ("gain", "pad_x", "pad_y")]


class AttnDesc(C.Structure):
    _fields_ = [
        ("Q", C.c_void_p), ("K", C.c_void_p), ("V", C.c_void_p), ("O", C.c_void_p),
        ("ldq", C.c_int64), ("ldk", C.c_int64), ("ldv", C.c_int64), ("ldo", C.c_int64),
        ("B", C.c_int32), ("H", C.c_int32), ("Tq", C.c_int32), ("Tk", C.c_int32), ("hd", C.c_int32),
        ("scale", C.c_float), ("mode", C.c_int32),
        ("Gh", C.c_int32), ("Gw", C.c_int32), ("ws", C.c_int32), ("q_stride", C.c_int32),
        ("pad_k", C.c_void_p), ("pad_v", C.c_void_p),
        ("rel", C.c_void_p), ("rel_S", C.c_int32),
    ]


_VP, _I, _I64, _F, _D = C.c_void_p, C.c_int, C.c_int64, C.c_float, C.c_double
SIGNATURES = {
    "lmx_version": (_I, []),
    "lmx_last_error": (C.c_char_p, []),
    "lmx_device_count": (_I, []),
    "lmx_k_gemm": (_I, [C.POINTER(GemmDesc), _VP]),
    "lmx_dbg_set_gemm2_variant": (None, [_I]),
    "lmx_h_gemm_route": (_I, [C.POINTER(GemmDesc), C.c_char_p, _I]),
    "lmx_h_attn_route": (_I, [C.POINTER(AttnDesc), C.c_char_p, _I]),
    "lmx_h_layernorm_route": (_I, [_I, _I, _I, _I, _I, C.c_char_p, _I]),
    "lmx_k_pose_gather": (_I, [_VP, _VP, _VP, _I64, _VP, _VP, _VP, _VP, _I, _I, _I, _I, _F, _F, _F, _F, _F, _VP, _VP]),
    "lmx_k_pack_bits": (_I, [_VP, _I64, _I, _VP, _VP]),
    "lmx_k_ln_mlp": (_I, [_VP, _I64, _VP, _VP, _VP, _VP, _VP, _VP, _I64, _I, _F, _VP, _VP, _VP, _VP, _VP, _VP]),
    "lmx_k_hiera_attn8": (_I, [_VP, _VP, _I64, _VP, _VP, _F, _VP, _VP, _VP, _VP, _I, _I, _I, _I, _I, _F, _VP]),
    "lmx_k_hiera_attn4": (_I, [_VP, _VP, _I64, _VP, _VP, _I, _I, _I, _I, _I, _F, _VP]),
    "lmx_k_hiera_attn_pool": (_I, [_VP, _VP, _VP, _VP, _I, _I, _I, _I, _I, _I, _F, _VP]),
    "lmx_k_ln_mlp_img": (_I, [_VP, _I64, _VP, _VP, _I64, _I, _F, _VP, _VP, _VP]),
    "lmx_k_layernorm": (_I, [_VP, _I, _I64, _VP, _VP, _VP, _I, _I64, _I, _I, _F, _I, _VP]),
    "lmx_k_attention": (_I, [C.POINTER(AttnDesc), _VP]),
    "lmx_k_relpos_tables": (_I, [C.POINTER(AttnDesc), _VP, _VP, _I, _VP, _VP]),
    "lmx_k_rope": (_I, [_VP, _I64, _I, _I, _I, _I, _I, _VP, _VP, _VP]),
    "lmx_k_pil_resize_h": (_I, [_VP, _VP, _I, _I, _I, _I, _VP, _VP, _I, _I, _VP]),
    "lmx_k_pil_resize_v": (_I, [_VP, _VP, _I, _I, _I, _I, _VP, _VP, _I, _VP]),
    "lmx_k_patchify_norm": (_I, [_VP, _VP, _I, _I, _I, _I, _I, _I, _I, _I, _I64, _VP, _VP]),
    "lmx_k_float_resize_patchify": (_I, [_VP, _VP, _I, _I, _I, _I, _I, _I, _I64, _VP, _VP, _I, _VP, _VP, _I, _I, _F, _VP, _I, _VP]),
    "lmx_k_assemble_tokens": (_I, [_VP, _VP, _VP, _VP, _I, _I, _I, _I, _VP]),
    "lmx_k_token_mean": (_I, [_VP, _I, _VP, _I, _I, _I, _VP]),
    "lmx_k_swiglu": (_I, [_VP, _I64, _VP, _I64, _I, _I, _VP]),
    "lmx_nms_workspace_bytes": (_I64, [_I, _I]),
    "lmx_k_nms": (_I, [_VP, _I, _I, _I, _F, _D, _I, _F, _VP, _VP, _VP, _VP, _VP, _VP, _VP]),
    "lmx_k_letterbox": (_I, [_VP, _VP, _I, _I, _I, _I, _I, _I, _I, _I, _I, _VP, _VP, _VP, _VP, _I, _VP]),
    "lmx_k_stem_conv": (_I, [_VP, _VP, _VP, _VP, _I, _I, _I, _I, _VP]),
    "lmx_k_split3": (_I, [_VP, _I64, _I, _VP, _I64, _VP, _I64, _I64, _I, _I, _I, _I64, _VP]),
    "lmx_k_maxpool5_x3": (_I, [_VP, _I64, _VP, _I64, _I, _I, _I, _I, _VP]),
    "lmx_k_stem_conv_x3": (_I, [_VP, _VP, _VP, _VP, _I, _I, _I, _I, _VP]),
    "lmx_k_attention_f32": (_I, [_VP, _I64, _VP, _I64, _VP, _I64, _VP, _I64, _I, _I, _I, _I, _I, _F, _VP]),
    "lmx_k_hyper_mask_f32": (_I, [_VP, _VP, _VP, _I, _I, _I, _I, _VP]),
    "lmx_k_maxpool5": (_I, [_VP, _I64, _VP, _I64, _I, _I, _I, _I, _VP]),
    "lmx_k_upsample2": (_I, [_VP, _I64, _VP, _I64, _I, _I, _I, _I, _VP]),
    "lmx_k_detect_decode": (_I, [_VP, _I64, _VP, _I, _I, _I, _I, _F, _I, _I, _VP]),
    "lmx_k_scale_boxes": (_I, [_VP, _I, _F, _F, _F, _F, _F, _VP]),
    "lmx_k_im2col_u8": (_I, [_VP, _VP, _VP, _I, _I, _I, _I, _I, _I, _I, _I, _I, _I64, _VP]),
    "lmx_k_maxpool2": (_I, [_VP, _I64, _VP, _I64, _I, _I, _I, _I, _I, _VP]),
    "lmx_k_cast_f32_f16": (_I, [_VP, _I64, _VP, _I64, _I64, _I, _VP]),
    "lmx_h_hiera_band": (_I, [C.POINTER(C.c_int), C.POINTER(C.c_int), _I, _I, _I, _I, C.POINTER(C.c_int)]),
    "lmx_h_hiera_bands": (_I, [C.POINTER(C.c_int), C.POINTER(C.c_int), _I, _I, _I, _I, C.POINTER(C.c_int)]),
    "lmx_k_band_join": (_I, [_VP, _VP, _VP, _I, _I, _I, _I, _I, _I, _VP]),
    "lmx_k_add_bcast":(_I, [_VP, _I, _I64, _VP, _I64, _I, _VP, _I, _I64, _I64, _I, _VP]),
    "lmx_h_mask_features": (_I, [_VP, _I, _I, _VP]),
    "lmx_h_iou_matrix": (_I, [_VP, _I, _VP, _I, _VP]),
    "lmx_h_assign": (_I, [_VP, _I, _I, _VP, _VP]),
    "lmx_contour_workspace_bytes": (_I64, [_I, _I, _I]),
    "lmx_k_contour_features": (_I, [_VP, _I, _I, _I, _VP, _VP, _VP]),
    "lmx_k_prompt_box": (_I, [_VP, _I64, _VP, _I, _D, _D, _F, _VP, _VP, _I, _VP]),
    "lmx_k_hyper_mask": (_I, [_VP, _VP, _VP, _I, _I, _I, _VP]),
    "lmx_k_mask_post": (_I, [_VP, _I, _I, _I, _I, _I, _I, _I, _VP, _VP, _VP, _VP]),
    "lmx_k_prompt_points": (_I, [_VP, _VP, _I, _VP, _I64, _VP, _I, _D, _D, _F, _VP, _VP, _VP, _VP, _I, _VP]),
    "lmx_k_mask_embed": (_I, [_VP, _VP, _I, _I64, _VP, _VP, _I64, _I, _I, _VP]),
    "lmx_k_hyper_mask_multi": (_I, [_VP, _VP, _VP, _I, _I, _I, _I, _VP]),
    "lmx_k_hyper_mask_multi_f32": (_I, [_VP, _VP, _VP, _I, _I, _I, _I, _I, _VP]),
    "lmx_k_mask_logits": (_I, [_VP, _I, _I, _I, _I, _I, _I, _I, _VP, _VP]),
    "lmx_k_mask_score": (_I, [_VP, _I, _I, _I, _I, _I, _I, _I, _D, _D, _VP, _VP, _VP]),
    "lmx_k_nms_boxes": (_I, [_VP, _I64, _VP, _VP, _I, _D, _VP, _VP, _VP, _VP]),
    "lmx_h_pil_tables": (_I, [_I, _I, _I, _VP, _VP, _I64, C.POINTER(C.c_int)]),
    "lmx_h_aa_tables": (_I, [_I, _I, _I, _VP, _VP, _I64, C.POINTER(C.c_int)]),
    "lmx_h_identity_table": (_I, [_I, _VP, _VP]),
    "lmx_h_segment_cols": (_I, [_VP, _I, _I]),
    "lmx_dino_image_check_host": (_I, [C.c_char_p, C.POINTER(DinoInfo)]),
    "lmx_dino_open_host": (_I, [C.c_char_p, _I, C.POINTER(_VP)]),
    "lmx_dino_close": (None, [_VP]),
    "lmx_dino_info": (_I, [_VP, C.POINTER(DinoInfo)]),
    "lmx_dino_prepare": (_I, [_VP, _I, _I]),
    "lmx_dino_embed": (_I, [_VP, _VP, _I, _I, _I, _I, _VP, _VP]),
    "lmx_dino_embed_host": (_I, [_VP, _VP, _I, _I, _I, _I, _VP]),
    "lmx_h_letterbox_geometry": (_I, [_I, _I, _I, _I, _I, C.POINTER(LetterboxGeo)]),
    "lmx_h_letterbox_tables": (_I, [_I, _I, _I, _I, _VP, _VP, _VP, _VP]),
    "lmx_h_conv_split_k": (_I, [_I64, _I, _I, _I]),
    "lmx_yolo_image_check_host": (_I, [C.c_char_p, C.POINTER(YoloInfo)]),
    "lmx_yolo_open_host": (_I, [C.c_char_p, _I, C.POINTER(_VP)]),
    "lmx_yolo_close": (None, [_VP]),
    "lmx_yolo_info": (_I, [_VP, C.POINTER(YoloInfo)]),
    "lmx_yolo_class_name": (C.c_char_p, [_VP, _I]),
    "lmx_yolo_prepare": (_I, [_VP, _I, _I, _I]),
    "lmx_yolo_anchors": (_I, [_VP, _I, _I, C.POINTER(C.c_int), C.POINTER(C.c_int), C.POINTER(C.c_int)]),
    "lmx_yolo_predict": (_I, [_VP, _VP, _I, _I, _I, _I, _VP, _VP]),
    "lmx_yolo_detect": (_I, [_VP, _VP, _I, _I, _I, _I, _F, _D, _I, _VP, _VP, _VP, _VP, _VP, _VP, _VP]),
    "lmx_yolo_detect_host": (_I, [_VP, _VP, _I, _I, _I, _I, _F, _D, _I, _VP, _VP, _VP, _VP, _VP, _VP]),
}

_lib = None


def load():
    global _lib
    if _lib is not None:
        return _lib
    if not os.path.exists(LIB_PATH):
        raise ImportError(
            f"{LIB_PATH} not found: build it with `python -c 'import __graft_entry__ as g; g.build()'` "
            "(hipcc --offload-arch=gfx950).  lmx has no CPU fallback.")
    import torch
# ... 15 lines not shown
```

### vision-sam3-yolo-lameless_amd/lmx/kernels.py

```python
import ctypes as C
import os
import threading

import torch

from . import _lib
from ._lib import AttnDesc, GemmDesc, LmxError, check

F16, F32 = 0, 1
ACT_NONE, ACT_SILU, ACT_GELU, ACT_RELU, ACT_SWIGLU = 0, 1, 2, 3, 4
_DT = {torch.float16: F16, torch.float32: F32}


_tls = threading.local()


def _stream(dev):
    _tls.dev = dev
    return C.c_void_p(torch.cuda.current_stream(dev).cuda_stream)


def _ptr(t):
    return C.c_void_p(t.data_ptr()) if t is not None else C.c_void_p(0)


def _dev(*ts):
    dev = None
    for t in ts:
        if t is None:
            continue
        if not t.is_cuda:
            raise LmxError("lmx kernels take device (HBM) tensors only; got a CPU tensor")
        if dev is None:
            dev = t.device
        elif t.device != dev:
            raise LmxError(f"lmx kernels: operands on different devices ({dev} and {t.device})")
    if dev is None:
        raise LmxError("lmx kernels: no device operand")
    return dev


def _rows(t, what):
    if t.dim() != 2 or t.stride(1) != 1:
        raise LmxError(f"{what}: expected a 2-D tensor with contiguous last dim, got shape {tuple(t.shape)} "
                       f"strides {t.stride()}")
    return t.shape[0], t.shape[1], t.stride(0)


_ROUTE_PTR = 4096


def _route_name(fn, *args):
    name = C.create_string_buffer(64)
    check(fn(*args, name, len(name)), fn.__name__)
    return name.value.decode()


def gemm_route(M, N, K, *, out_dtype=torch.float16, act=ACT_NONE, scale=False, res=False, res_rows=0, a_rep=1, pool_hw=None,
               lda=None, ldc=None, ldr=None, ln_out=False, split_k=1):
    d = GemmDesc()
    d.A = d.W = d.C = d.bias = _ROUTE_PTR
    d.scale = _ROUTE_PTR if scale else None
    d.res = _ROUTE_PTR if res else None
    d.M, d.N, d.K = M, N, a_rep * K
    d.lda = K if lda is None else lda
    d.ldc = (N // 2 if act == ACT_SWIGLU else N) if ldc is None else ldc
    d.ldr = (N if ldr is None else ldr) if res else 0
    d.res_rows, d.a_rep = res_rows, a_rep
    d.act, d.out_dtype, d.a_mode = act, _DT[out_dtype], 0
    if pool_hw:
        d.a_mode, d.H, d.W_ = 2, int(pool_hw[0]), int(pool_hw[1])
    if ln_out:
        d.ln_out = d.ln_gamma = d.ln_beta = _ROUTE_PTR
        d.ld_ln, d.ln_eps = N, 1e-6
    if split_k > 1:
        d.split_k, d.split_stride = split_k, M * d.ldc
    return _route_name(_lib.load().lmx_h_gemm_route, C.byref(d))


def conv3x3_route(n, H, W, cin, cout, *, stride=1, out_dtype=torch.float16, act=ACT_SILU, res=False, scale=False, split_k=1):
    Ho, Wo = (H + 2 - 3) // stride + 1, (W + 2 - 3) // stride + 1
    d = GemmDesc()
    d.A = d.W = d.C = d.bias = _ROUTE_PTR
    d.scale = _ROUTE_PTR if scale else None
    d.res = _ROUTE_PTR if res else None
    d.lda, d.ldc, d.ldr = cin, cout, (cout if res else 0)
    d.M, d.N, d.K = n * Ho * Wo, cout, 9 * cin
    d.act, d.out_dtype, d.a_mode = act, _DT[out_dtype], 1
    d.H, d.W_, d.Cin, d.conv_stride, d.Ho, d.Wo = H, W, cin, stride, Ho, Wo
    if split_k > 1:
        d.split_k, d.split_stride = split_k, n * Ho * Wo * cout
    return _route_name(_lib.load().lmx_h_gemm_route, C.byref(d))


def attention_route(B, H, Tq, Tk, hd, *, window=None, pad=False, rel_S=0, ld=None):
    d = AttnDesc()
    d.Q = d.K = d.V = d.O = _ROUTE_PTR
    d.ldq = d.ldk = d.ldv = d.ldo = H * hd if ld is None else ld
    d.B, d.H, d.Tq, d.Tk, d.hd = B, H, Tq, Tk, hd
    d.scale = 1.0
    if window is not None:
        d.mode = 1
        d.Gh, d.Gw, d.ws, d.q_stride = window["Gh"], window["Gw"], window["ws"], window.get("q_stride", 1)
        d.pad_k = d.pad_v = _ROUTE_PTR if pad else None
    if rel_S:
        d.rel, d.rel_S = _ROUTE_PTR, rel_S
    return _route_name(_lib.load().lmx_h_attn_route, C.byref(d))


def layernorm_route(rows, D, in_dtype=torch.float32, out_dtype=torch.float16, act=ACT_NONE):
    return _route_name(_lib.load().lmx_h_layernorm_route, _DT[in_dtype], _DT[out_dtype], rows, D, act)


def pooled_gemm_ok(M, N):
    return M >= 512 and N >= 96 and N % 8 == 0


def gemm(a, w, bias=None, act=ACT_NONE, scale=None, res=None, out=None, out_dtype=torch.float16, res_rows=0, pool_hw=None, a_rep=1,
         ln_out=None):
    dev = _dev(a, w, bias, scale, res, out, *(ln_out[:3] if ln_out is not None else ()))
    M, K, lda = _rows(a, "gemm A")
    N, K2, ldw = _rows(w, "gemm W")
    if K2 != a_rep * K or ldw != K2:
        raise LmxError(f"gemm: W must be contiguous [N,{a_rep}*K]; A K={K}, W shape {tuple(w.shape)}")
    if a.dtype != torch.float16 or w.dtype != torch.float16:
        raise LmxError("gemm: A and W must be float16")
    Mout = M // 4 if pool_hw else M
    Nout = N // 2 if act == ACT_SWIGLU else N
    if out is None:
        out = torch.empty((Mout, Nout), dtype=out_dtype, device=a.device)
    Mo, No, ldc = _rows(out, "gemm C")
    if (Mo, No) != (Mout, Nout):
        raise LmxError(f"gemm: out shape {tuple(out.shape)} != ({Mout},{Nout})")
    d = GemmDesc()
    d.A, d.W, d.C = a.data_ptr(), w.data_ptr(), out.data_ptr()
    d.bias = bias.data_ptr() if bias is not None else None
    d.scale = scale.data_ptr() if scale is not None else None
    d.lda, d.ldc, d.ldr = lda, ldc, 0
    if bias is not None and (bias.dtype != torch.float32 or bias.numel() != N):
        raise LmxError("gemm: bias must be float32 [N]")
    if scale is not None and (scale.dtype != torch.float32 or scale.numel() != Nout):
        raise LmxError("gemm: scale must be float32 [N] (ACT_SWIGLU: [N/2])")
    if res is not None:
        Mr, Nr, ldr = _rows(res, "gemm res")
        if (Mr, Nr) != ((res_rows or M), N) or res.dtype != out.dtype:
            raise LmxError("gemm: residual must match out's shape and dtype")
        d.res, d.ldr = res.data_ptr(), ldr
    d.res_rows = res_rows
    d.M, d.N, d.K = M, N, a_rep * K
    d.act, d.out_dtype, d.a_mode, d.a_rep = act, _DT[out.dtype], 0, a_rep
    if pool_hw:
        d.a_mode, d.H, d.W_ = 2, int(pool_hw[0]), int(pool_hw[1])
    if ln_out is not None:
        h, g, b, eps = ln_out
        Mh, Nh, ldh = _rows(h, "gemm ln_out")
        if (Mh, Nh) != (Mout, Nout) or h.dtype != torch.float16:
            raise LmxError(f"gemm: ln_out must be float16 [{Mout},{Nout}], got {h.dtype} {tuple(h.shape)}")
        if any(t.dtype != torch.float32 or t.numel() != Nout or not t.is_contiguous() for t in (g, b)):
            raise LmxError("gemm: ln_out's gamma and beta must be contiguous float32 [N]")
        d.ln_out, d.ln_gamma, d.ln_beta, d.ld_ln, d.ln_eps = h.data_ptr(), g.data_ptr(), b.data_ptr(), ldh, float(eps)
    check(_lib.load().lmx_k_gemm(C.byref(d), _stream(dev)), "lmx_k_gemm")
    return out


def im2col_u8(img, lut, IH, IW, KH, KW, stride, pad, ldo):
    dev = _dev(img, lut)
    n, rh, rw, c = img.shape
    if c != 3 or img.dtype != torch.uint8 or not img.is_contiguous():
        raise LmxError("im2col_u8: img must be contiguous uint8 [n,h,w,3]")
    OH, OW = (IH + 2 * pad - KH) // stride + 1, (IW + 2 * pad - KW) // stride + 1
    out = torch.empty((n * OH * OW, ldo), dtype=torch.float16, device=img.device)
    check(_lib.load().lmx_k_im2col_u8(_ptr(img), _ptr(lut), _ptr(out), n, rh, rw, IH, IW, KH, KW, stride, pad, ldo,
                                      _stream(dev)), "lmx_k_im2col_u8")
    return out


def maxpool2(x, out):
    dev = _dev(x, out)
    n, H, W, Cc, ps = _nhwc(x, "maxpool2 x")
    no, Ho, Wo, Co, pso = _nhwc(out, "maxpool2 out")
    if (no, Ho, Wo, Co) != (n, H // 2, W // 2, Cc) or x.dtype != out.dtype:
        raise LmxError("maxpool2: shape/dtype mismatch")
    check(_lib.load().lmx_k_maxpool2(_ptr(x), ps, _ptr(out), pso, _DT[x.dtype], n, H, W, Cc, _stream(dev)), "lmx_k_maxpool2")
    return out


def cast_f16(x, out=None):
    dev = _dev(x, out)
    rows, cols, lds = _rows(x, "cast src")
    if out is None:
        out = torch.empty((rows, cols), dtype=torch.float16, device=x.device)
    check(_lib.load().lmx_k_cast_f32_f16(_ptr(x), lds, _ptr(out), out.stride(0), rows, cols, _stream(dev)),
          "lmx_k_cast_f32_f16")
    return out


def hiera_band(windows, q_strides, grid, nh, nw):
    nb = len(windows)
    if nb != len(q_strides):
        raise LmxError("hiera_band: windows and q_strides must be the same length")
    band = C.c_int(0)
    check(_lib.load().lmx_h_hiera_band((C.c_int * nb)(*windows), (C.c_int * nb)(*q_strides), nb, grid, nh, nw, C.byref(band)),
          "lmx_h_hiera_band")
    return band.value


def hiera_bands(windows, q_strides, grid, nh, nw):
    nb = len(windows)
    if nb != len(q_strides):
        raise LmxError("hiera_bands: windows and q_strides must be the same length")
    rows = (C.c_int * nb)()
    check(_lib.load().lmx_h_hiera_bands((C.c_int * nb)(*windows), (C.c_int * nb)(*q_strides), nb, grid, nh, nw, rows), "lmx_h_hiera_bands")
    return tuple(rows)


def band_join(band, table, H):
    dev = _dev(band, table)
# ... 460 lines not shown

def detect_decode(head, pred, nc, stride, a_off):
    dev = _dev(head, pred)
    n, H, W, ldh = head.shape
    A = pred.shape[1]
    if not head.is_contiguous() or not pred.is_contiguous() or pred.shape[2] != 4 + nc:
        raise LmxError("detect_decode: head/pred must be dense")
    check(_lib.load().lmx_k_detect_decode(_ptr(head), ldh, _ptr(pred), n, H, W, nc, float(stride), a_off, A, _stream(dev)),
          "lmx_k_detect_decode")
    return pred


def scale_boxes(boxes, padx, pady, gain, w, h):
    dev = _dev(boxes)
    if boxes.dtype != torch.float32 or not boxes.is_contiguous() or boxes.shape[-1] != 4:
        raise LmxError("scale_boxes: boxes must be dense float32 [...,4]")
    check(_lib.load().lmx_k_scale_boxes(_ptr(boxes), boxes.numel() // 4, float(padx), float(pady), float(gain), float(w),
                                        float(h), _stream(dev)), "lmx_k_scale_boxes")
    return boxes


def pose_gather(raws, strides, src, counts, kpt_shape, padx, pady, gain, w, h):
    dev = _dev(*raws, src, counts)
    K_, ndim = kpt_shape
    ldk = raws[0].shape[-1]
    for r in raws:
        if r.dtype != torch.float32 or not r.is_contiguous() or r.dim() != 4 or r.shape[-1] != ldk:
            raise LmxError("pose_gather: levels must be dense float32 [n,h,w,ldk]")
    if src.dtype != torch.int32 or counts.dtype != torch.int32 or not src.is_contiguous():
        raise LmxError("pose_gather: src / counts must be int32")
    n, max_det = src.shape
    hw = (C.c_int32 * 6)(*[v for r in raws for v in (r.shape[1], r.shape[2])])
    st = (C.c_float * 3)(*[float(v) for v in strides])
    out = torch.empty((n, max_det, K_, ndim), dtype=torch.float32, device=src.device)
    check(_lib.load().lmx_k_pose_gather(_ptr(raws[0]), _ptr(raws[1]), _ptr(raws[2]), ldk, C.cast(hw, C.c_void_p),
                                        C.cast(st, C.c_void_p), _ptr(src), _ptr(counts), n, max_det, K_, ndim, float(padx),
                                        float(pady), float(gain), float(w), float(h), _ptr(out), _stream(dev)), "lmx_k_pose_gather")
    return out


def add_bcast(a, b, out=None, out_dtype=torch.float32):
    dev = _dev(a, b, out)
    rows, D_, lda = _rows(a, "add_bcast a")
    b_rows, Db, ldb = _rows(b, "add_bcast b")
    if Db != D_ or a.dtype not in _DT or b.dtype != torch.float32:
        raise LmxError("add_bcast: a must be float16/float32, b float32, equal width")
    if out is None:
        out = torch.empty((rows, D_), dtype=out_dtype, device=a.device)
    check(_lib.load().lmx_k_add_bcast(_ptr(a), _DT[a.dtype], lda, _ptr(b), ldb, b_rows, _ptr(out), _DT[out.dtype], out.stride(0),
                                      rows, D_, _stream(dev)), "lmx_k_add_bcast")
    return out


def attention_f32(q, k, v, B, H, Tq, Tk, hd, scale):
    dev = _dev(q, k, v)
    for t in (q, k, v):
        if t.dtype != torch.float32 or t.dim() != 2 or t.stride(1) != 1:
            raise LmxError("attention_f32: q/k/v must be float32 2-D row views")
    out = torch.empty((B * Tq, H * hd), dtype=torch.float32, device=q.device)
    check(_lib.load().lmx_k_attention_f32(_ptr(q), q.stride(0), _ptr(k), k.stride(0), _ptr(v), v.stride(0), _ptr(out), out.stride(0),
                                          B, H, Tq, Tk, hd, float(scale), _stream(dev)), "lmx_k_attention_f32")
    return out


def hyper_mask_f32(up, hyper, n, G, C_, act=ACT_NONE):
    dev = _dev(up, hyper)
    if up.dtype != torch.float32 or not up.is_contiguous():
        raise LmxError("hyper_mask_f32: up must be contiguous float32")
    logits = torch.empty((n, 4 * G, 4 * G), dtype=torch.float32, device=up.device)
    check(_lib.load().lmx_k_hyper_mask_f32(_ptr(up), _ptr(hyper), _ptr(logits), n, G, C_, act, _stream(dev)), "lmx_k_hyper_mask_f32")
    return logits


def split3_rows(x, act=ACT_NONE):
    dev = _dev(x)
    rows, N, ldx = _rows(x, "split3_rows x")
    if x.dtype != torch.float32 or N % 8:
        raise LmxError("split3_rows: float32 rows with N % 8 == 0 expected")
    out = torch.empty((rows, 3 * N), dtype=torch.float16, device=x.device)
    check(_lib.load().lmx_k_split3(_ptr(x), ldx, act, None, 0, _ptr(out), 3 * N, rows, N, N, 1, 0, _stream(dev)), "lmx_k_split3")
    return out


def prompt_box(boxes, sx, sy, S, gauss, corner):
    dev = _dev(boxes, gauss, corner)
    n = boxes.shape[0]
    Fq = gauss.shape[1]
    out = torch.empty((n, 2, 2 * Fq), dtype=torch.float32, device=boxes.device)
    check(_lib.load().lmx_k_prompt_box(_ptr(boxes), boxes.stride(0), _ptr(out), n, float(sx), float(sy), float(S), _ptr(gauss),
                                       _ptr(corner), Fq, _stream(dev)), "lmx_k_prompt_box")
    return out


def hyper_mask(up, hyper, n, G, C_):
    dev = _dev(up, hyper)
    logits = torch.empty((n, 4 * G, 4 * G), dtype=torch.float32, device=up.device)
    check(_lib.load().lmx_k_hyper_mask(_ptr(up), _ptr(hyper), _ptr(logits), n, G, C_, _stream(dev)), "lmx_k_hyper_mask")
    return logits


def mask_post(logits, T, nh, nw, h, w):
    dev = _dev(logits)
    n, L, _ = logits.shape
    mask = torch.empty((n, h, w), dtype=torch.uint8, device=logits.device)
    stats = torch.empty((n, 8), dtype=torch.int64, device=logits.device)
    ws = torch.empty((n, nh, nw), dtype=torch.float32, device=logits.device)
# ... 93 lines not shown
        src = logits[s:s + k] if idx is None else logits
        check(lib.lmx_k_mask_score(_ptr(src), k, L, T, nh, nw, h, w, float(thr), float(off), _ptr(None if idx is None else idx[s:s + k]),
                                   _ptr(out[s:s + k]), _stream(dev)), "lmx_k_mask_score")
    return out


NMS_BOXES_MAX = 16384


def nms_boxes(boxes, scores, iou, valid=None):
    dev = _dev(boxes, scores, valid)
    n, cols, ldb = _rows(boxes, "nms_boxes boxes")
    if boxes.dtype != torch.float32 or cols < 4 or scores.dtype != torch.float32 or tuple(scores.shape) != (n,) or not scores.is_contiguous():
        raise LmxError("nms_boxes: boxes f32 [n,>=4] and scores contiguous f32 [n] expected")
    if not 0 < n <= NMS_BOXES_MAX:
        raise LmxError(f"nms_boxes: {n} candidates (1..{NMS_BOXES_MAX})")
    if valid is not None:
        if valid.dtype not in (torch.bool, torch.uint8) or tuple(valid.shape) != (n,):
            raise LmxError("nms_boxes: valid must be bool / uint8 [n]")
        valid = valid.contiguous().view(torch.uint8)
    keep = torch.empty((n,), dtype=torch.int32, device=boxes.device)
    count = torch.empty((1,), dtype=torch.int32, device=boxes.device)
    ws = torch.empty((n * 5,), dtype=torch.float32, device=boxes.device)
    check(_lib.load().lmx_k_nms_boxes(_ptr(boxes), ldb, _ptr(scores), _ptr(valid), n, float(iou), _ptr(keep), _ptr(count), _ptr(ws),
                                      _stream(dev)), "lmx_k_nms_boxes")
    return keep, count


def contour_features(mask):
    dev = _dev(mask)
    if mask.dtype != torch.uint8 or mask.dim() != 3 or not mask.is_contiguous():
        raise LmxError("contour_features: mask must be contiguous uint8 [n,h,w]")
    n, h, w = mask.shape
    lib = _lib.load()
    ws = torch.empty((int(lib.lmx_contour_workspace_bytes(n, h, w)),), dtype=torch.uint8, device=mask.device)
    out = torch.empty((n, 8), dtype=torch.int64, device=mask.device)
    check(lib.lmx_k_contour_features(_ptr(mask), n, h, w, _ptr(out), _ptr(ws), _stream(dev)), "lmx_k_contour_features")
    return out


LAUNCH_TRACE = None
_raw_lib = None
RIDGE_FLOP_PER_BYTE = 2500e12 / 8e12


def _work(name, args):
    if name == "lmx_k_gemm":
        d = args[0]._obj
        M, N, Kd = d.M, d.N, d.K
        osz = 4 if d.out_dtype == F32 else 2
        a_bytes = 2 * M * (Kd // max(d.a_rep, 1))
        if d.a_mode == 1:
            a_bytes = 2 * (M // max(d.Ho * d.Wo, 1)) * d.H * d.W_ * d.Cin
        by = a_bytes + 2 * N * Kd + osz * (M // 4 if d.a_mode == 2 else M) * (N // 2 if d.act == ACT_SWIGLU else N) + (osz * (d.res_rows or M) * N if d.res else 0)
        by += 2 * M * N if d.ln_out else 0
        fl = 2.0 * M * N * Kd
        key = f"gemm M={M} N={N} K={Kd} out={'f32' if osz == 4 else 'f16'} conv3x3={d.a_mode} act={d.act} res={int(bool(d.res))}" + (" ln_out" if d.ln_out else "")
        return ("gemm/mfma-bound" if fl / by >= RIDGE_FLOP_PER_BYTE else "gemm/hbm-bound"), fl, by, key
    if name == "lmx_k_attention":
        d = args[0]._obj
        fl = 4.0 * d.B * d.H * d.Tq * d.Tk * d.hd
        by = 2 * d.H * d.hd * d.B * (2 * d.Tq + 2 * d.Tk)
        key = f"attention B={d.B} H={d.H} Tq={d.Tq} Tk={d.Tk} hd={d.hd} mode={d.mode} ws={d.ws} qs={d.q_stride} rel={int(bool(d.rel))}"
        return ("attention/mfma-bound" if fl / by >= RIDGE_FLOP_PER_BYTE else "attention/hbm-bound"), fl, by, key
    if name == "lmx_k_layernorm":
        in_dt, out_dt, rows, D = args[1], args[6], args[8], args[9]
        return "layernorm", 0.0, rows * D * ((4 if in_dt == F32 else 2) + (4 if out_dt == F32 else 2)), f"layernorm rows={rows} D={D} in={in_dt} out={out_dt}"
    if name == "lmx_k_ln_mlp_img":
        rows, D = args[4], args[5]
        return "fused ln+mlp", 16.0 * D * D * rows, (8 + (2 if args[7] else 0) + (2 if args[8] else 0)) * D * rows, f"ln_mlp_img rows={rows} D={D}"
    if name == "lmx_k_ln_mlp":
        rows, D = args[8], args[9]
        return "fused ln+mlp", 16.0 * D * D * rows, (16 + (2 if args[12] else 0) + (2 if args[15] else 0)) * D * rows, f"ln_mlp rows={rows} D={D}"
    if name == "lmx_k_hiera_attn8":
        n_, Gh, Gw, D = args[10], args[11], args[12], args[13]
        rows = n_ * Gh * Gw
        return "fused attention half", rows * (8.0 * D * D + 256.0 * D), rows * D * (8 + (2 if args[0] else 0)), f"hiera_attn8 rows={rows} D={D} ln_inside={int(not args[0])}"
    if name == "lmx_k_hiera_attn4":
        n_, Gh, Gw, D = args[5], args[6], args[7], args[8]
        rows = n_ * Gh * Gw
        return "fused attention half", rows * (8.0 * D * D + 64.0 * D), rows * D * 10, f"hiera_attn4 rows={rows} D={D}"
    if name == "lmx_k_hiera_attn_pool":
        n_, Gh, Gw, Di, Do = args[4], args[5], args[6], args[7], args[8]
        rows = n_ * Gh * Gw
        keys = 64 if Di == 112 else 16
        return "fused attention half", rows * (8.0 * Di * Do + keys * Do + 0.5 * Do * Do), rows * (2 * Di + Do), f"hiera_attn_pool rows={rows} {Di}->{Do}"
    if name == "lmx_k_cast_f32_f16":
        rows, cols = args[4], args[5]
        return "streaming glue", 0.0, 6 * rows * cols, f"cast_f32_f16 rows={rows} cols={cols}"
    if name == "lmx_k_maxpool2":
        dt, n_, H, W, C_ = args[4], args[5], args[6], args[7], args[8]
        esz = 4 if dt == F32 else 2
        return "streaming glue", 0.0, esz * n_ * H * W * C_ * 5 // 4, f"maxpool2 n={n_} H={H} W={W} C={C_} dtype={dt}"
    if name == "lmx_k_upsample2":
        n_, H, W, C_ = args[4], args[5], args[6], args[7]
        return "streaming glue", 0.0, 2 * n_ * H * W * C_ * 5, f"upsample2 n={n_} H={H} W={W} C={C_}"
    if name == "lmx_k_add_bcast":
        a_dt, o_dt, rows, D = args[1], args[7], args[9], args[10]
        return "streaming glue", 0.0, rows * D * ((4 if a_dt == F32 else 2) + (4 if o_dt == F32 else 2)), f"add_bcast rows={rows} D={D}"
    if name == "lmx_k_band_join":
        dt, n_, H, Hb, W, D = args[3:9]
        return "streaming glue", 0.0, 2 * (4 if dt == F32 else 2) * n_ * H * W * D, f"band_join n={n_} H={H} Hb={Hb} W={W} D={D} dtype={dt}"
    if name == "lmx_k_rope":
        B, T, H, hd = args[2], args[3], args[4], args[5]
        return "streaming glue", 0.0, 2 * 2 * 2 * B * T * H * hd, f"rope B={B} T={T} H={H} hd={hd}"
    return "pre/post-processing and glue", 0.0, None, name


def _install_trace():
    global _raw_lib
    if _raw_lib is not None:
        return
    lib = _raw_lib = _lib.load()

    def make(name, fn):
        def traced(*args):
            if LAUNCH_TRACE is None:
                return fn(*args)
            cls, fl, by, key = _work(name, args)
            st = torch.cuda.current_stream(_tls.dev)
            e0, e1 = torch.cuda.Event(enable_timing=True), torch.cuda.Event(enable_timing=True)
            e0.record(st)
            rc = fn(*args)
            e1.record(st)
            LAUNCH_TRACE.append((cls, key, fl, by, e0, e1))
            return rc

        return traced

    class _Proxy:
        def __getattr__(self, name):
            fn = getattr(lib, name)
            if name.startswith("lmx_k_"):
                fn = make(name, fn)
            setattr(self, name, fn)
            return fn

    _lib._lib = _Proxy()


def start_launch_trace():
    global LAUNCH_TRACE
    _install_trace()
    LAUNCH_TRACE = []


def stop_launch_trace(by_shape=False):
    global LAUNCH_TRACE
    tr, LAUNCH_TRACE = LAUNCH_TRACE or [], None
    torch.cuda.synchronize()
    out, shapes = {}, {}
    for cls, key, fl, by, e0, e1 in tr:
# ... 9 lines not shown
```

### vision-sam3-yolo-lameless_amd/lmx/sam_decoder.py

```python
import math

import numpy as np
import torch

from . import kernels as K

D = 256
HEADS = 8


def param_spec():
    s = {}
    s["shared_image_embedding.positional_embedding"] = ((2, 128), "tok")
    s["prompt_encoder.shared_embedding.positional_embedding"] = ((2, 128), "tok")
    s["prompt_encoder.no_mask_embed.weight"] = ((1, D), "tok")
    for i in range(4):
        s[f"prompt_encoder.point_embed.{i}.weight"] = ((1, D), "tok")
    s["prompt_encoder.not_a_point_embed.weight"] = ((1, D), "tok")
    s["mask_decoder.iou_token.weight"] = ((1, D), "tok")
    s["mask_decoder.mask_tokens.weight"] = ((4, D), "tok")

    def attn(p, inner):
        for n_ in ("q_proj", "k_proj", "v_proj"):
            s[p + n_ + ".weight"] = ((inner, D), "w")
# ... 58 lines not shown
    sd = weights.synth_state_dict(param_spec(), seed)
    sd["prompt_encoder.shared_embedding.positional_embedding"] = sd["shared_image_embedding.positional_embedding"].copy()
    return sd


class MaskDecoder:

    def __init__(self, state_dict, device="cuda", image_size=1024, grid=64, precision="exact"):
        if precision not in ("exact", "f16"):
            raise ValueError(f"precision {precision!r}: expected 'exact' or 'f16'")
        self.precision = precision
        self.device = torch.device(device)
        self.S, self.G = image_size, grid
        dev = self.device
        sd = state_dict
        self._sd = {k: np.asarray(v, np.float32) for k, v in sd.items() if k.startswith("mask_decoder.")}
        self._wx = {}

        def t32(a):
            return torch.from_numpy(np.ascontiguousarray(a, dtype=np.float32)).to(dev)

        def t16(a):
            return t32(a).to(torch.float16).contiguous()

        gauss = sd["shared_image_embedding.positional_embedding"].astype(np.float32)
        self.gauss = t32(gauss)
        self.corner = t32(np.concatenate([sd["prompt_encoder.point_embed.2.weight"], sd["prompt_encoder.point_embed.3.weight"]], 0))
        g = torch.ones((grid, grid), dtype=torch.float32)
        yx = torch.stack([(g.cumsum(1) - 0.5) / grid, (g.cumsum(0) - 0.5) / grid], -1)
        c = 2 * np.pi * ((2 * yx - 1) @ torch.from_numpy(gauss))
        self.key_pe = torch.cat([torch.sin(c), torch.cos(c)], -1).reshape(grid * grid, D).contiguous().to(dev)
        self.no_mask = t32(sd["prompt_encoder.no_mask_embed.weight"])
        self.point_embed = t32(np.concatenate([sd["prompt_encoder.point_embed.0.weight"], sd["prompt_encoder.point_embed.1.weight"]], 0))
        self.not_a_point = t32(sd["prompt_encoder.not_a_point_embed.weight"][0])
        me = mask_embed_param_spec()
        self.mask_params = t32(np.concatenate([np.asarray(sd[k], np.float32).ravel() for k in me])) if all(k in sd for k in me) else None
        self.out_tokens = t32(np.concatenate([sd["mask_decoder.iou_token.weight"], sd["mask_decoder.mask_tokens.weight"]], 0))

        def attn(p):
            return {n_: (t16(sd[p + n_ + ".weight"]), t32(sd[p + n_ + ".bias"])) for n_ in ("q_proj", "k_proj", "v_proj", "out_proj")}

        def ln(p):
            return t32(sd[p + "weight"]), t32(sd[p + "bias"])

        self.layers = []
        for i in range(2):
            p = f"mask_decoder.transformer.layers.{i}."
            self.layers.append(dict(sa=attn(p + "self_attn."), ln1=ln(p + "layer_norm1."),
                                    t2i=attn(p + "cross_attn_token_to_image."), ln2=ln(p + "layer_norm2."),
                                    w1=(t16(sd[p + "mlp.lin1.weight"]), t32(sd[p + "mlp.lin1.bias"])),
                                    w2=(t16(sd[p + "mlp.lin2.weight"]), t32(sd[p + "mlp.lin2.bias"])),
                                    ln3=ln(p + "layer_norm3."), ln4=ln(p + "layer_norm4."),
                                    i2t=attn(p + "cross_attn_image_to_token.")))
        self.final = attn("mask_decoder.transformer.final_attn_token_to_image.")
        self.ln_final = ln("mask_decoder.transformer.layer_norm_final_attn.")
        w1 = sd["mask_decoder.upscale_conv1.weight"]
        w2 = sd["mask_decoder.upscale_conv2.weight"]
        self.up1 = (t16(np.transpose(w1, (2, 3, 1, 0)).reshape(4 * w1.shape[1], w1.shape[0])), t32(np.tile(sd["mask_decoder.upscale_conv1.bias"], 4)))
        self.up2 = (t16(np.transpose(w2, (2, 3, 1, 0)).reshape(4 * w2.shape[1], w2.shape[0])), t32(np.tile(sd["mask_decoder.upscale_conv2.bias"], 4)))
        self.up_ln = ln("mask_decoder.upscale_layer_norm.")

        def ffn(p):
            return [(t16(sd[p + n_ + ".weight"]), t32(sd[p + n_ + ".bias"])) for n_ in ("proj_in", "layers.0", "proj_out")]

        self.hypers = [ffn(f"mask_decoder.output_hypernetworks_mlps.{m}.") for m in range(4)]
        self.iou_head = ffn("mask_decoder.iou_prediction_head.")

    def _attn(self, W, q16, k16, v16, n, tq, tk, res):
        q = K.gemm(q16, *W["q_proj"])
        k = K.gemm(k16, *W["k_proj"])
        v = K.gemm(v16, *W["v_proj"])
        inner = q.shape[1]
        hd = inner // HEADS
        a = torch.empty((n * tq, inner), dtype=torch.float16, device=q.device)
        K.attention(q, k, v, a, n, HEADS, tq, tk, hd, hd ** -0.5)
        return K.gemm(a, W["out_proj"][0], bias=W["out_proj"][1], res=res, out_dtype=torch.float32)

    @staticmethod
    def _ffn(layers, x16):
        h = K.gemm(x16, *layers[0], act=K.ACT_RELU)
        h = K.gemm(h, *layers[1], act=K.ACT_RELU)
        return K.gemm(h, *layers[2], out_dtype=torch.float32)

    def lowres(self, emb, sparse, keys=None, masks=None):
        n = sparse.shape[0]
        T, P = 5 + sparse.shape[1], self.G * self.G
        sel = (0,) if masks is None else tuple(masks)
        eps = 1e-6
        tokens = torch.cat([self.out_tokens[None].expand(n, -1, -1), sparse], dim=1).reshape(n * T, D).contiguous()
        if keys is None:
            keys = K.add_bcast(emb, self.no_mask)
        queries, qpe = tokens, tokens
        for i, L in enumerate(self.layers):
            if i == 0:
                q16 = K.cast_f16(queries)
                queries = self._attn(L["sa"], q16, q16, q16, n, T, T, None)
            else:
                q16 = K.add_bcast(queries, qpe, out_dtype=torch.float16)
                queries = self._attn(L["sa"], q16, q16, K.cast_f16(queries), n, T, T, queries)
            queries = K.layernorm(queries, *L["ln1"], eps, out_dtype=torch.float32)
            q16 = K.add_bcast(queries, qpe, out_dtype=torch.float16)
            k16 = K.add_bcast(keys, self.key_pe, out_dtype=torch.float16)
            queries = self._attn(L["t2i"], q16, k16, K.cast_f16(keys), n, T, P, queries)
            queries = K.layernorm(queries, *L["ln2"], eps, out_dtype=torch.float32)
            h = K.gemm(K.cast_f16(queries), *L["w1"], act=K.ACT_RELU)
            queries = K.gemm(h, *L["w2"], res=queries, out_dtype=torch.float32)
            queries = K.layernorm(queries, *L["ln3"], eps, out_dtype=torch.float32)
            q16 = K.add_bcast(queries, qpe, out_dtype=torch.float16)
            keys = self._attn(L["i2t"], k16, q16, K.cast_f16(queries), n, P, T, keys)
            keys = K.layernorm(keys, *L["ln4"], eps, out_dtype=torch.float32)
        q16 = K.add_bcast(queries, qpe, out_dtype=torch.float16)
        k16 = K.add_bcast(keys, self.key_pe, out_dtype=torch.float16)
        keys16 = K.cast_f16(keys)
        queries = self._attn(self.final, q16, k16, keys16, n, T, P, queries)
        queries = K.layernorm(queries, *self.ln_final, 1e-5, out_dtype=torch.float32)
        q3 = queries.view(n, T, D)
        iou_tok = K.cast_f16(q3[:, 0].contiguous())
        u = K.gemm(keys16, *self.up1, out_dtype=torch.float32)
        u = K.layernorm(u.view(n * P * 4, 64), *self.up_ln, eps, act=K.ACT_GELU)
        u = K.gemm(u, *self.up2, act=K.ACT_GELU)
        hs = [self._ffn(self.hypers[m], K.cast_f16(q3[:, 1 + m].contiguous())) for m in sel]
        hyper = hs[0][:, None] if len(hs) == 1 else torch.stack(hs, 1)
        logits = K.hyper_mask_multi(u, hyper, n, self.G, 32)
        iou = self._ffn(self.iou_head, iou_tok)
        return (logits[:, 0], iou[:, 0]) if masks is None else (logits, iou)

    def _lin(self, x, name, act_in=K.ACT_NONE, act=K.ACT_NONE, res=None, w2d=None, bias=None):
        from .exact import split_rows_x3

        if name not in self._wx:
            w = self._sd[name + ".weight"] if w2d is None else w2d
            b = self._sd[name + ".bias"] if bias is None else bias
            x3, sc, e = split_rows_x3(w, [w.shape[1]])
            dev = self.device
            self._wx[name] = (torch.from_numpy(x3).to(dev), torch.from_numpy(np.ldexp(b.astype(np.float32), e).astype(np.float32)).to(dev),
                              torch.from_numpy(sc).to(dev))
        w3, b3, sc = self._wx[name]
        return K.gemm(K.split3_rows(x, act_in), w3, bias=b3, act=act, scale=sc, res=res, out_dtype=torch.float32)

    def _attn_exact(self, p, q_in, k_in, v_in, n, tq, tk, res):
        q = self._lin(q_in, p + "q_proj")
        k = self._lin(k_in, p + "k_proj")
        v = self._lin(v_in, p + "v_proj")
        hd = q.shape[1] // HEADS
        a = K.attention_f32(q, k, v, n, HEADS, tq, tk, hd, hd ** -0.5)
        return self._lin(a, p + "out_proj", res=res)

    def _ffn_exact(self, p, x):
        h = self._lin(x, p + "proj_in", act=K.ACT_RELU)
        h = self._lin(h, p + "layers.0", act=K.ACT_RELU)
        return self._lin(h, p + "proj_out")

    def lowres_exact(self, emb, sparse, keys=None, masks=None):
        n = sparse.shape[0]
        T, P = 5 + sparse.shape[1], self.G * self.G
        sel = (0,) if masks is None else tuple(masks)
        eps = 1e-6
        f32 = torch.float32
        tokens = torch.cat([self.out_tokens[None].expand(n, -1, -1), sparse], dim=1).reshape(n * T, D).contiguous()
        if keys is None:
            keys = K.add_bcast(emb, self.no_mask)
        queries, qpe = tokens, tokens
        for i in range(2):
            p = f"mask_decoder.transformer.layers.{i}."
            L = self.layers[i]
            if i == 0:
                queries = self._attn_exact(p + "self_attn.", queries, queries, queries, n, T, T, None)
            else:
                q_ = K.add_bcast(queries, qpe, out_dtype=f32)
                queries = self._attn_exact(p + "self_attn.", q_, q_, queries, n, T, T, queries)
            queries = K.layernorm(queries, *L["ln1"], eps, out_dtype=f32)
            q_ = K.add_bcast(queries, qpe, out_dtype=f32)
# ... 86 lines not shown
```

Before: 802.4 frames/s.

## Fuse SAM decoder glue into GEMM-LayerNorm epilogues and add register-ring K/V prefetch

The SAM mask decoder now fuses several small glue kernels into existing kernels. The i2t out-projection GEMM's LayerNorm epilogue writes f32 keys, f16 keys and keys+PE together. A new add_bcast3 kernel produces keys, keys16 and keys+PE in one pass. The t2i k_proj and i2t q_proj are merged into one concatenated GEMM, and the upscale conv1 GEMM applies a grouped LayerNorm+GELU epilogue. Separately, the tiled attention kernel gains a 4-slot register ring that prefetches K/V tiles several iterations ahead for small grids, which raises register pressure and template complexity.

```diff
diff --git a/include/lmx.h b/include/lmx.h
--- a/include/lmx.h
+++ b/include/lmx.h
@@ -43,6 +43,14 @@
   const float* ln_beta;
   int64_t ld_ln;
   float ln_eps;
+  void* ln_out_f32;
+  int64_t ld_ln_f32;
+  void* ln_out_add;
+  int64_t ld_ln_add;
+  const float* ln_add;
+  int64_t ld_add;
+  int32_t ln_add_rows;
+  int32_t ln_group;
 } lmx_gemm_desc;
 int lmx_k_gemm(const lmx_gemm_desc* d, lmx_stream_t stream);
 void lmx_dbg_set_gemm2_variant(int v);
@@ -151,6 +159,9 @@
 
 int lmx_k_add_bcast(const void* a, int a_dtype, int64_t lda, const float* b, int64_t ldb, int b_rows, void* out,
                     int out_dtype, int64_t ldo, int64_t rows, int D, lmx_stream_t stream);
+int lmx_k_add_bcast3(const void* a, int a_dtype, int64_t lda, const float* b, int64_t ldb, int b_rows, const float* pe, int64_t ldp,
+                     int pe_rows, float* keys, int64_t ldk, void* keys16, int64_t ld16, void* kpe16, int64_t ldkp, int64_t rows, int D,
+                     lmx_stream_t stream);
 int lmx_k_prompt_box(const float* boxes, int64_t ldb, float* sparse, int n, double sx, double sy, float S,
                      const float* gauss, const float* corner, int F, lmx_stream_t stream);
 int lmx_k_hyper_mask(const void* up, const float* hyper, float* logits, int n, int G, int C, lmx_stream_t stream);
diff --git a/vision-sam3-yolo-lameless_amd/csrc/attn.hip b/vision-sam3-yolo-lameless_amd/csrc/attn.hip
--- a/vision-sam3-yolo-lameless_amd/csrc/attn.hip
+++ b/vision-sam3-yolo-lameless_amd/csrc/attn.hip
@@ -62,7 +62,7 @@
   return h;
 }
 
-template <int QB, bool ONES, bool REL, bool DMA, int HDW>
+template <int QB, bool ONES, bool REL, bool DMA, int HDW, int RING = 1>
 __global__ __launch_bounds__(256, 2) void attn_kernel(const lmx_attn_desc p, const Geo geo, const int nQT) {
 #ifndef LMX_ATTN_RING
 #define LMX_ATTN_RING 3
@@ -138,12 +138,52 @@
   const int sc = tid & (CPR - 1);
   const int sk = tid / CPR;
   constexpr int KPP = 256 / CPR;
-  half8_t kst[NPASS], vst[NPASS];
+  static_assert(RING == 1 || (!DMA && !REL && QB == 1 && HDW == 64), "the ring is built (and its registers budgeted) for the one-block forms at 64-half rows");
+  static_assert(RING >= 1 && RING <= 4, "for_slots below spells out four slots");
+  half8_t kst[RING][NPASS], vst[RING][NPASS];
+  unsigned stm[RING];
   const int64_t hoff0 = (int64_t)h * hd + sc * 8;
   const half_t* Kb = K + hoff0 + (geo.mode == 0 ? (int64_t)b * p.Tk * p.ldk : 0);
   const half_t* Vb = V + hoff0 + (geo.mode == 0 ? (int64_t)b * p.Tk * p.ldv : 0);
   const bool d_ok = sc * 8 < hd;
-  auto load_tile = [&](int t0) {
+  auto load_tile = [&](int t0, auto slot_tag) {
+    constexpr int SL = decltype(slot_tag)::value;
+    if constexpr (RING > 1) {
+      typedef const __attribute__((address_space(1))) half8_t* gptr8;
+      gptr8 kp[NPASS], vp[NPASS];
+      unsigned m = 0;
+      if (geo.mode == 0) {
+#pragma unroll
+        for (int i = 0; i < NPASS; ++i) {
+          const int t = t0 + sk + KPP * i;
+          const bool in = d_ok && t < p.Tk;
+          const int tt = in ? t : 0;
+          kp[i] = (gptr8)(Kb + (int64_t)tt * p.ldk);
+          vp[i] = (gptr8)(Vb + (int64_t)tt * p.ldv);
+          m |= (in ? 0x101u << i : 0u) | (ONES && sc == 7 && t < p.Tk ? 0x10000u << i : 0u);
+        }
+      } else {
+#pragma unroll
+        for (int i = 0; i < NPASS; ++i) {
+          const int t = t0 + sk + KPP * i;
+          const int d = sc * 8;
+          const bool in = (t < p.Tk) && (d < hd);
+          const int64_t row = key_row(geo, b, in ? t : 0);
+          const bool pad = row < 0;
+          const int64_t hoff = (int64_t)h * hd + d;
+          kp[i] = (gptr8)(pad ? (padk ? padk + hoff : K) : K + (in ? row * p.ldk + hoff : 0));
+          vp[i] = (gptr8)(pad ? (padv ? padv + hoff : V) : V + (in ? row * p.ldv + hoff : 0));
+          m |= ((in && (!pad || padk)) ? 1u << i : 0u) | ((in && (!pad || padv)) ? 0x100u << i : 0u) | (ONES && sc == 7 && t < p.Tk ? 0x10000u << i : 0u);
+        }
+      }
+#pragma unroll
+      for (int i = 0; i < NPASS; ++i) {
+        kst[SL][i] = *kp[i];
+        vst[SL][i] = *vp[i];
+      }
+      stm[SL] = m;
+      return;
+    }
     if (geo.mode == 0) {
 #pragma unroll
       for (int i = 0; i < NPASS; ++i) {
@@ -152,9 +192,9 @@
         const int tt = in ? t : 0;
         const half8_t kv = *reinterpret_cast<const half8_t*>(Kb + (int64_t)tt * p.ldk);
         const half8_t vv = *reinterpret_cast<const half8_t*>(Vb + (int64_t)tt * p.ldv);
-        kst[i] = in ? kv : zero8;
-        vst[i] = in ? vv : zero8;
-        if (ONES && sc == 7 && t < p.Tk) vst[i][7] = (half_t)1.0f;
+        kst[SL][i] = in ? kv : zero8;
+        vst[SL][i] = in ? vv : zero8;
+        if (ONES && sc == 7 && t < p.Tk) vst[SL][i][7] = (half_t)1.0f;
       }
       return;
     }
@@ -170,19 +210,34 @@
       const half_t* vp = pad ? (padv ? padv + hoff : V) : V + (in ? row * p.ldv + hoff : 0);
       const half8_t kv = *reinterpret_cast<const half8_t*>(kp);
       const half8_t vv = *reinterpret_cast<const half8_t*>(vp);
-      kst[i] = (in && (!pad || padk)) ? kv : zero8;
-      vst[i] = (in && (!pad || padv)) ? vv : zero8;
-      if (ONES && sc == 7 && t < p.Tk) vst[i][7] = (half_t)1.0f;
+      kst[SL][i] = (in && (!pad || padk)) ? kv : zero8;
+      vst[SL][i] = (in && (!pad || padv)) ? vv : zero8;
+      if (ONES && sc == 7 && t < p.Tk) vst[SL][i][7] = (half_t)1.0f;
     }
   };
-  auto store_tile = [&](int buf) {
+  auto store_tile = [&](int buf, auto slot_tag) {
+    constexpr int SL = decltype(slot_tag)::value;
 #pragma unroll
     for (int i = 0; i < NPASS; ++i) {
       const int kk = sk + KPP * i;
       const int off = kk * RW + ((sc ^ (kk & (CPR - 1))) << 3);
-      *reinterpret_cast<half8_t*>(&Ks[buf][off]) = kst[i];
-      *reinterpret_cast<half8_t*>(&Vs[buf][off]) = vst[i];
-    }
+      if constexpr (RING == 1) {
+        *reinterpret_cast<half8_t*>(&Ks[buf][off]) = kst[SL][i];
+        *reinterpret_cast<half8_t*>(&Vs[buf][off]) = vst[SL][i];
+      } else {
+        const unsigned m = stm[SL];
+        half8_t vv = (m >> (8 + i)) & 1 ? vst[SL][i] : zero8;
+        if (ONES && ((m >> (16 + i)) & 1)) vv[7] = (half_t)1.0f;
+        *reinterpret_cast<half8_t*>(&Ks[buf][off]) = (m >> i) & 1 ? kst[SL][i] : zero8;
+        *reinterpret_cast<half8_t*>(&Vs[buf][off]) = vv;
+      }
+    }
+  };
+  auto for_slots = [&](auto f) {
+    f(std::integral_constant<int, 0>{});
+    if constexpr (RING > 1) f(std::integral_constant<int, 1>{});
+    if constexpr (RING > 2) f(std::integral_constant<int, 2>{});
+    if constexpr (RING > 3) f(std::integral_constant<int, 3>{});
   };
 
   const float sl2 = REL ? 1.44269504088896340736f : p.scale * 1.44269504088896340736f;
@@ -217,8 +272,14 @@
     for (int t = 0; t < LA; ++t)
       if (t < ntile) issue(t, t);
   } else {
-    load_tile(0);
-    store_tile(0);
+    load_tile(0, std::integral_constant<int, 0>{});
+    store_tile(0, std::integral_constant<int, 0>{});
+    if constexpr (RING > 1) {
+      for_slots([&](auto j) {
+        constexpr int t = decltype(j)::value + 1;
+        load_tile(t * 64, std::integral_constant<int, t % RING>{});
+      });
+    }
     __syncthreads();
   }
   int k_lane[KS], v_lane[NDB];
@@ -229,7 +290,7 @@
     const int chunk = db * 2 + (p4 >> 1), rl = fg * 4 + q4;
     v_lane[db] = rl * RW + ((chunk ^ (rl & (CPR - 1))) << 3) + (p4 & 1) * 4;
   }
-  auto tile_body = [&](const int it, auto mask_tag) {
+  auto tile_body = [&](const int it, auto mask_tag, auto slot_tag) {
     constexpr bool MASK = decltype(mask_tag)::value;
     const int t0 = it * 64;
     int buf;
@@ -241,7 +302,9 @@
       buf = it % NSL;
     } else {
       buf = it & 1;
-      if (it + 1 < ntile) load_tile(t0 + 64);
+      if constexpr (RING == 1) {
+        if (it + 1 < ntile) load_tile(t0 + 64, slot_tag);
+      }
     }
 
     unsigned kbase[KS], vbase[NDB];
@@ -348,15 +411,27 @@
     }
 
     if constexpr (!DMA) {
-      if (it + 1 < ntile) store_tile(buf ^ 1);
+      if (it + 1 < ntile) {
+        store_tile(buf ^ 1, slot_tag);
+        if constexpr (RING > 1) load_tile(t0 + (1 + RING) * 64, slot_tag);
+      }
       __syncthreads();
     }
   };
-  for (int it = 0; it + 1 < ntile; ++it) tile_body(it, std::false_type{});
+  const std::integral_constant<int, 0> slot0{};
+  if constexpr (RING == 1) {
+    for (int it = 0; it + 1 < ntile; ++it) tile_body(it, std::false_type{}, slot0);
+  } else {
+    for (int it0 = 0; it0 + 1 < ntile; it0 += RING)
+      for_slots([&](auto j) {
+        constexpr int J = decltype(j)::value;
+        if (it0 + J + 1 < ntile) tile_body(it0 + J, std::false_type{}, std::integral_constant<int, (J + 1) % RING>{});
+      });
+  }
   if (p.Tk & 63)
-    tile_body(ntile - 1, std::true_type{});
+    tile_body(ntile - 1, std::true_type{}, slot0);
   else
-    tile_body(ntile - 1, std::false_type{});
+    tile_body(ntile - 1, std::false_type{}, slot0);
 
 #pragma unroll
   for (int qb = 0; qb < QB; ++qb) {
@@ -1344,6 +1419,7 @@
   int QB = 1;
   bool ONES = false, REL = false, DMA = false;
   int HDW = 64, NWV = 4;
+  int RING = 1;
   unsigned grid = 0, block = 256;
   int lds = 0;
   int arg = 0;
@@ -1418,11 +1494,12 @@
   r.HDW = wide ? 96 : 64;
   r.grid = (unsigned)nblk;
   r.arg = no_lazy ? -nQT : nQT;
+  if (r.QB == 1 && !r.REL && !r.DMA && r.HDW == 64 && nblk <= 512 && (d.Tk + 63) / 64 > 4) r.RING = 4;
   return LMX_OK;
 }
 
-static constexpr int attn_key(int kernel, int QB, bool ONES, bool REL, bool DMA, int HDW, int NWV) {
-  return (((((kernel * 4 + QB) * 2 + ONES) * 2 + REL) * 2 + DMA) * 128 + HDW) * 16 + NWV;
+static constexpr int attn_key(int kernel, int QB, bool ONES, bool REL, bool DMA, int HDW, int NWV, int RING = 1) {
+  return ((((((kernel * 4 + QB) * 2 + ONES) * 2 + REL) * 2 + DMA) * 128 + HDW) * 16 + NWV) * 8 + RING;
 }
 
 extern "C" int lmx_k_attention(const lmx_attn_desc* dp, lmx_stream_t stream) {
@@ -1448,7 +1525,9 @@
   case attn_key(ATTN_GP, 1, ONES, false, false, 64, NWV): hipLaunchKernelGGL((attn_gp_kernel<ONES, NWV>), grid, block, r.lds, st, d, r.arg); break
 #define LMX_TILED(QB, ONES, REL, DMA, HDW) \
   case attn_key(ATTN_TILED, QB, ONES, REL, DMA, HDW, 4): hipLaunchKernelGGL((attn_kernel<QB, ONES, REL, DMA, HDW>), grid, block, 0, st, d, g, r.arg); break
-  switch (attn_key(r.kernel, r.QB, r.ONES, r.REL, r.DMA, r.HDW, r.NWV)) {
+#define LMX_TILED_RING(ONES) \
+  case attn_key(ATTN_TILED, 1, ONES, false, false, 64, 4, 4): hipLaunchKernelGGL((attn_kernel<1, ONES, false, false, 64, 4>), grid, block, 0, st, d, g, r.arg); break
+  switch (attn_key(r.kernel, r.QB, r.ONES, r.REL, r.DMA, r.HDW, r.NWV, r.RING)) {
     case attn_key(ATTN_SMALL, 1, false, false, false, 64, 4): hipLaunchKernelGGL(attn_small_kernel, grid, block, 0, st, d, g, r.arg); break;
     LMX_SPP(true);
     LMX_SPP(false);
@@ -1470,12 +1549,15 @@
     LMX_TILED(2, false, false, false, 64);
     LMX_TILED(1, true, false, false, 64);
     LMX_TILED(1, false, false, false, 64);
+    LMX_TILED_RING(true);
+    LMX_TILED_RING(false);
     default: LMX_REQUIRE(false, "lmx_k_attention: no kernel for route %d", (int)r.kernel);
   }
 #undef LMX_SP
 #undef LMX_SPP
 #undef LMX_GP
 #undef LMX_TILED
+#undef LMX_TILED_RING
   static const char* const what[] = {"attn_small_kernel", "attn_sp_kernel", "attn_spp_kernel", "attn_gp_kernel", "attn_kernel"};
   return lmx_launch_check(what[r.kernel]);
 }
diff --git a/vision-sam3-yolo-lameless_amd/csrc/gemm.hip b/vision-sam3-yolo-lameless_amd/csrc/gemm.hip
--- a/vision-sam3-yolo-lameless_amd/csrc/gemm.hip
+++ b/vision-sam3-yolo-lameless_amd/csrc/gemm.hip
@@ -250,13 +250,15 @@
 static int gemm_route(const lmx_gemm_desc* dp, GemmRoute& r) {
   LMX_REQUIRE(dp != nullptr, "lmx_k_gemm: null descriptor");
   const lmx_gemm_desc& d = *dp;
-  LMX_REQUIRE(d.A && d.W && d.C, "lmx_k_gemm: null A/W/C");
+  const bool ln_req = d.ln_out || d.ln_out_f32 || d.ln_out_add;
+  LMX_REQUIRE(d.A && d.W && (d.C || ln_req), "lmx_k_gemm: null A/W/C (C may be null only beside a LayerNorm output)");
+  LMX_REQUIRE(ln_req || (!d.ln_add && d.ln_group == 0), "lmx_k_gemm: ln_add / ln_group without a LayerNorm output");
   LMX_REQUIRE(d.M > 0 && d.N > 0 && d.K > 0, "lmx_k_gemm: empty problem M=%d N=%d K=%d", d.M, d.N, d.K);
   LMX_REQUIRE(d.K % 8 == 0, "lmx_k_gemm: K=%d must be a multiple of 8", d.K);
   LMX_REQUIRE(d.N % 4 == 0, "lmx_k_gemm: N=%d must be a multiple of 4", d.N);
   LMX_REQUIRE(d.lda % 8 == 0, "lmx_k_gemm: lda=%lld must be a multiple of 8", (long long)d.lda);
   const bool gated = d.act == LMX_ACT_SWIGLU;
-  LMX_REQUIRE(d.ldc % 4 == 0 && d.ldc >= (gated ? d.N / 2 : d.N), "lmx_k_gemm: bad ldc=%lld", (long long)d.ldc);
+  LMX_REQUIRE(!d.C || (d.ldc % 4 == 0 && d.ldc >= (gated ? d.N / 2 : d.N)), "lmx_k_gemm: bad ldc=%lld", (long long)d.ldc);
   LMX_REQUIRE(aligned16(d.A) && aligned16(d.W), "lmx_k_gemm: A/W must be 16-byte aligned");
   LMX_REQUIRE((((uintptr_t)d.C) & 7) == 0, "lmx_k_gemm: C must be 8-byte aligned");
   LMX_REQUIRE(d.out_dtype == LMX_F16 || d.out_dtype == LMX_F32, "lmx_k_gemm: bad out_dtype %d", d.out_dtype);
@@ -299,14 +301,29 @@
   LMX_REQUIRE(d.split_k >= 0 && d.split_k <= 64, "lmx_k_gemm: split_k=%d (0..64)", d.split_k);
   static const int v1 = lmx_env_char("LMX_GEMM_V1") == '1';
   static const int n64 = lmx_env_char("LMX_GEMM_N64") != '0';
-  if (d.ln_out) {
-    LMX_REQUIRE(d.out_dtype == LMX_F32 && d.res && d.res_rows == 0, "lmx_k_gemm: ln_out needs f32 output with a full residual (out_dtype=%d res_rows=%d)", d.out_dtype, d.res_rows);
+  if (ln_req) {
+    LMX_REQUIRE(d.out_dtype == LMX_F32, "lmx_k_gemm: ln_out needs out_dtype f32 (out_dtype=%d)", d.out_dtype);
     LMX_REQUIRE(d.N <= 448 && d.N % 16 == 0 && d.K <= 448, "lmx_k_gemm: ln_out: a tile holds whole rows of N <= 448 (N %% 16 == 0) over K <= 448; N=%d K=%d", d.N, d.K);
     LMX_REQUIRE(d.a_mode == 0 && d.a_rep <= 1 && d.split_k <= 1, "lmx_k_gemm: ln_out: dense A only (a_mode=%d a_rep=%d split_k=%d)", d.a_mode, d.a_rep, d.split_k);
     LMX_REQUIRE(d.act == LMX_ACT_NONE && !d.scale, "lmx_k_gemm: ln_out takes no activation and no scale");
     LMX_REQUIRE(d.ln_gamma && d.ln_beta && aligned16(d.ln_gamma) && aligned16(d.ln_beta), "lmx_k_gemm: ln_gamma / ln_beta must be given, 16-byte aligned");
-    LMX_REQUIRE(d.ld_ln % 4 == 0 && d.ld_ln >= d.N && (((uintptr_t)d.ln_out) & 7) == 0, "lmx_k_gemm: ln_out must be 8-byte aligned with ld_ln=%lld a multiple of 4, >= N", (long long)d.ld_ln);
-    LMX_REQUIRE(aligned16(d.res), "lmx_k_gemm: ln_out: the residual must be 16-byte aligned");
+    if (d.ln_out)
+      LMX_REQUIRE(d.ld_ln % 4 == 0 && d.ld_ln >= d.N && (((uintptr_t)d.ln_out) & 7) == 0, "lmx_k_gemm: ln_out must be 8-byte aligned with ld_ln=%lld a multiple of 4, >= N", (long long)d.ld_ln);
+    if (d.ln_group) {
+      LMX_REQUIRE(d.ln_group == 64 && d.N % 64 == 0, "lmx_k_gemm: ln_group=%d: groups of 64 columns, N=%d a multiple of 64", d.ln_group, d.N);
+      LMX_REQUIRE(d.ln_out && !d.ln_out_f32 && !d.ln_out_add && !d.ln_add, "lmx_k_gemm: ln_group writes ln_out (f16) only");
+      LMX_REQUIRE(!d.res && !d.C, "lmx_k_gemm: ln_group takes no residual and stores no C");
+    } else {
+      LMX_REQUIRE(d.res && d.res_rows == 0, "lmx_k_gemm: ln_out needs a full residual (res_rows=%d)", d.res_rows);
+      LMX_REQUIRE(aligned16(d.res), "lmx_k_gemm: ln_out: the residual must be 16-byte aligned");
+      if (d.ln_out_f32)
+        LMX_REQUIRE(d.ld_ln_f32 % 4 == 0 && d.ld_ln_f32 >= d.N && aligned16(d.ln_out_f32), "lmx_k_gemm: ln_out_f32 must be 16-byte aligned with ld_ln_f32=%lld a multiple of 4, >= N", (long long)d.ld_ln_f32);
+      LMX_REQUIRE(!d.ln_out_add == !d.ln_add, "lmx_k_gemm: ln_out_add and ln_add go together");
+      if (d.ln_out_add) {
+        LMX_REQUIRE(d.ld_ln_add % 4 == 0 && d.ld_ln_add >= d.N && (((uintptr_t)d.ln_out_add) & 7) == 0, "lmx_k_gemm: ln_out_add must be 8-byte aligned with ld_ln_add=%lld a multiple of 4, >= N", (long long)d.ld_ln_add);
+        LMX_REQUIRE(d.ln_add_rows > 0 && d.ld_add % 4 == 0 && d.ld_add >= d.N && aligned16(d.ln_add), "lmx_k_gemm: ln_add must be 16-byte aligned [ln_add_rows=%d][N] with ld_add=%lld a multiple of 4, >= N", d.ln_add_rows, (long long)d.ld_add);
+      }
+    }
     r = GemmRoute{true, 128, 448, BK, 2, 0, true};
     return LMX_OK;
   }
diff --git a/vision-sam3-yolo-lameless_amd/csrc/gemm2.hip b/vision-sam3-yolo-lameless_amd/csrc/gemm2.hip
--- a/vision-sam3-yolo-lameless_amd/csrc/gemm2.hip
+++ b/vision-sam3-yolo-lameless_amd/csrc/gemm2.hip
@@ -484,6 +484,7 @@
   }
 }
 
+template <int MODE>
 __global__ __launch_bounds__(512) void gemm2_rowln_kernel(const lmx_gemm_desc p) {
   constexpr int BM = RL_BM, BN = RL_BN, BK = RL_BK, NSTAGE = RL_NSTAGE, STAGE_BYTES = RL_STAGE_BYTES;
   constexpr int NWAVE = 8;
@@ -539,8 +540,10 @@
   float bias_v = 0.f, gamma_v = 0.f, beta_v = 0.f;
   if (tid < p.N) {
     if (p.bias) bias_v = p.bias[tid];
-    gamma_v = p.ln_gamma[tid];
-    beta_v = p.ln_beta[tid];
+    if (MODE != 2 || tid < 64) {
+      gamma_v = p.ln_gamma[tid];
+      beta_v = p.ln_beta[tid];
+    }
   }
 
   issue(0, 0);
@@ -584,12 +587,15 @@
   const int c0 = lane * 4, c1 = (64 + lane) * 4;
   const bool ok0 = c0 < D, ok1 = c1 < D;
   const f32x4 z4 = {0.f, 0.f, 0.f, 0.f};
-  const f32x4 g0 = ok0 ? *reinterpret_cast<const f32x4*>(bl + BN + c0) : z4, g1 = ok1 ? *reinterpret_cast<const f32x4*>(bl + BN + c1) : z4;
-  const f32x4 b0 = ok0 ? *reinterpret_cast<const f32x4*>(bl + 2 * BN + c0) : z4, b1 = ok1 ? *reinterpret_cast<const f32x4*>(bl + 2 * BN + c1) : z4;
+  const int gc0 = MODE == 2 ? (c0 & 63) : c0, gc1 = MODE == 2 ? (c1 & 63) : c1;
+  const f32x4 g0 = ok0 ? *reinterpret_cast<const f32x4*>(bl + BN + gc0) : z4, g1 = ok1 ? *reinterpret_cast<const f32x4*>(bl + BN + gc1) : z4;
+  const f32x4 b0 = ok0 ? *reinterpret_cast<const f32x4*>(bl + 2 * BN + gc0) : z4, b1 = ok1 ? *reinterpret_cast<const f32x4*>(bl + 2 * BN + gc1) : z4;
   const float* blj = bl + wn * (BN / 4) + fq * 4;
   const float* res = reinterpret_cast<const float*>(p.res);
   float* Cf = reinterpret_cast<float*>(p.C);
   half_t* Lh = reinterpret_cast<half_t*>(p.ln_out);
+  float* Lf = reinterpret_cast<float*>(p.ln_out_f32);
+  half_t* La = reinterpret_cast<half_t*>(p.ln_out_add);
 #pragma unroll
   for (int ps = 0; ps < 4; ++ps) {
     float* buf = reinterpret_cast<float*>(smem) + (ps & 1) * 32 * RL_RS;
@@ -599,9 +605,23 @@
       const int lr = wave * 4 + rr;
       const int m = m0 + (lr >> 4) * 64 + ps * 16 + (lr & 15);
       r0[rr] = r1[rr] = z4;
-      if (m < p.M) {
+      if (MODE != 2 && m < p.M) {
         if (ok0) r0[rr] = *reinterpret_cast<const f32x4*>(res + (int64_t)m * p.ldr + c0);
         if (ok1) r1[rr] = *reinterpret_cast<const f32x4*>(res + (int64_t)m * p.ldr + c1);
+      }
+    }
+    f32x4 a0[MODE == 1 ? 4 : 1], a1[MODE == 1 ? 4 : 1];
+    if constexpr (MODE == 1) {
+#pragma unroll
+      for (int rr = 0; rr < 4; ++rr) {
+        const int lr = wave * 4 + rr;
+        const int m = m0 + (lr >> 4) * 64 + ps * 16 + (lr & 15);
+        a0[rr] = a1[rr] = z4;
+        if (La && m < p.M) {
+          const float* ar = p.ln_add + (int64_t)(m % p.ln_add_rows) * p.ld_add;
+          if (ok0) a0[rr] = *reinterpret_cast<const f32x4*>(ar + c0);
+          if (ok1) a1[rr] = *reinterpret_cast<const f32x4*>(ar + c1);
+        }
       }
     }
 #pragma unroll
@@ -609,50 +629,94 @@
       *reinterpret_cast<f32x4*>(buf + (wm * 16 + frow) * RL_RS + wn * (BN / 4) + j * 16 + fq * 4) = acc[ps][j] + *reinterpret_cast<const f32x4*>(blj + j * 16);
     asm volatile("s_waitcnt lgkmcnt(0)" ::: "memory");
     __builtin_amdgcn_s_barrier();
-    f32x4 v0[4], v1[4];
-    float s[4], q[4], mean[4], rstd[4];
-#pragma unroll
-    for (int rr = 0; rr < 4; ++rr) {
-      const int lr = wave * 4 + rr;
-      const f32x4 t0 = *reinterpret_cast<const f32x4*>(buf + lr * RL_RS + (ok0 ? c0 : 0)), t1 = *reinterpret_cast<const f32x4*>(buf + lr * RL_RS + (ok1 ? c1 : 0));
-      v0[rr] = (ok0 ? t0 : z4) + r0[rr];
-      v1[rr] = (ok1 ? t1 : z4) + r1[rr];
-      s[rr] = 0.f;
-      s[rr] += (v0[rr][0] + v0[rr][1]) + (v0[rr][2] + v0[rr][3]);
-      s[rr] += (v1[rr][0] + v1[rr][1]) + (v1[rr][2] + v1[rr][3]);
-    }
-    wave_sum4(s);
-#pragma unroll
-    for (int rr = 0; rr < 4; ++rr) {
-      mean[rr] = s[rr] / (float)D;
-      q[rr] = 0.f;
-      {
-        const f32x4 dlt = v0[rr] - mean[rr];
-        const float t = (dlt[0] * dlt[0] + dlt[1] * dlt[1]) + (dlt[2] * dlt[2] + dlt[3] * dlt[3]);
-        q[rr] += ok0 ? t : 0.f;
-      }
-      {
-        const f32x4 dlt = v1[rr] - mean[rr];
-        const float t = (dlt[0] * dlt[0] + dlt[1] * dlt[1]) + (dlt[2] * dlt[2] + dlt[3] * dlt[3]);
-        q[rr] += ok1 ? t : 0.f;
-      }
-    }
-    wave_sum4(q);
-#pragma unroll
-    for (int rr = 0; rr < 4; ++rr) {
-      const int lr = wave * 4 + rr;
-      const int m = m0 + (lr >> 4) * 64 + ps * 16 + (lr & 15);
-      rstd[rr] = 1.0f / sqrtf(q[rr] / (float)D + p.ln_eps);
-      if (m < p.M) {
-        if (ok0) *reinterpret_cast<f32x4*>(Cf + (int64_t)m * p.ldc + c0) = v0[rr];
-        if (ok1) *reinterpret_cast<f32x4*>(Cf + (int64_t)m * p.ldc + c1) = v1[rr];
-        if (ok0) {
-          const f32x4 o = (v0[rr] - mean[rr]) * rstd[rr] * g0 + b0;
-          *reinterpret_cast<half4_t*>(Lh + (int64_t)m * p.ld_ln + c0) = half4_t{(half_t)o[0], (half_t)o[1], (half_t)o[2], (half_t)o[3]};
-        }
-        if (ok1) {
-          const f32x4 o = (v1[rr] - mean[rr]) * rstd[rr] * g1 + b1;
-          *reinterpret_cast<half4_t*>(Lh + (int64_t)m * p.ld_ln + c1) = half4_t{(half_t)o[0], (half_t)o[1], (half_t)o[2], (half_t)o[3]};
+    if constexpr (MODE == 2) {
+#pragma unroll
+      for (int rr = 0; rr < 4; ++rr) {
+        const int lr = wave * 4 + rr;
+        const int m = m0 + (lr >> 4) * 64 + ps * 16 + (lr & 15);
+#pragma unroll
+        for (int hf = 0; hf < 2; ++hf) {
+          if (hf && D <= 256) continue;
+          const bool ok = hf ? ok1 : ok0;
+          const int c = hf ? c1 : c0;
+          const f32x4 t = *reinterpret_cast<const f32x4*>(buf + lr * RL_RS + (ok ? c : 0));
+          const f32x4 v = ok ? t : z4;
+          float sg = (v[0] + v[1]) + (v[2] + v[3]);
+          sg += 0.f;
+#pragma unroll
+          for (int o = 8; o > 0; o >>= 1) sg += __shfl_xor(sg, o, 64);
+          const float mean = sg / 64.0f;
+          const f32x4 dl = ok ? v - mean : z4;
+          float qg = (dl[0] * dl[0] + dl[1] * dl[1]) + (dl[2] * dl[2] + dl[3] * dl[3]);
+          qg += 0.f;
+#pragma unroll
+          for (int o = 8; o > 0; o >>= 1) qg += __shfl_xor(qg, o, 64);
+          const float var = qg / 64.0f;
+          const float rstd = 1.0f / sqrtf(var + p.ln_eps);
+          f32x4 o = dl * rstd * (hf ? g1 : g0) + (hf ? b1 : b0);
+#pragma unroll
+          for (int e = 0; e < 4; ++e) o[e] = 0.5f * o[e] * (1.0f + erff(o[e] * 0.70710678118654752440f));
+          if (ok && m < p.M) *reinterpret_cast<half4_t*>(Lh + (int64_t)m * p.ld_ln + c) = half4_t{(half_t)o[0], (half_t)o[1], (half_t)o[2], (half_t)o[3]};
+        }
+      }
+    } else {
+      f32x4 v0[4], v1[4];
+      float s[4], q[4], mean[4], rstd[4];
+#pragma unroll
+      for (int rr = 0; rr < 4; ++rr) {
+        const int lr = wave * 4 + rr;
+        const f32x4 t0 = *reinterpret_cast<const f32x4*>(buf + lr * RL_RS + (ok0 ? c0 : 0)), t1 = *reinterpret_cast<const f32x4*>(buf + lr * RL_RS + (ok1 ? c1 : 0));
+        v0[rr] = (ok0 ? t0 : z4) + r0[rr];
+        v1[rr] = (ok1 ? t1 : z4) + r1[rr];
+        s[rr] = 0.f;
+        s[rr] += (v0[rr][0] + v0[rr][1]) + (v0[rr][2] + v0[rr][3]);
+        s[rr] += (v1[rr][0] + v1[rr][1]) + (v1[rr][2] + v1[rr][3]);
+      }
+      wave_sum4(s);
+#pragma unroll
+      for (int rr = 0; rr < 4; ++rr) {
+        mean[rr] = s[rr] / (float)D;
+        q[rr] = 0.f;
+        {
+          const f32x4 dlt = v0[rr] - mean[rr];
+          const float t = (dlt[0] * dlt[0] + dlt[1] * dlt[1]) + (dlt[2] * dlt[2] + dlt[3] * dlt[3]);
+          q[rr] += ok0 ? t : 0.f;
+        }
+        {
+          const f32x4 dlt = v1[rr] - mean[rr];
+          const float t = (dlt[0] * dlt[0] + dlt[1] * dlt[1]) + (dlt[2] * dlt[2] + dlt[3] * dlt[3]);
+          q[rr] += ok1 ? t : 0.f;
+        }
+      }
+      wave_sum4(q);
+#pragma unroll
+      for (int rr = 0; rr < 4; ++rr) {
+        const int lr = wave * 4 + rr;
+        const int m = m0 + (lr >> 4) * 64 + ps * 16 + (lr & 15);
+        rstd[rr] = 1.0f / sqrtf(q[rr] / (float)D + p.ln_eps);
+        if (m < p.M) {
+          if (MODE == 0 || Cf) {
+            if (ok0) *reinterpret_cast<f32x4*>(Cf + (int64_t)m * p.ldc + c0) = v0[rr];
+            if (ok1) *reinterpret_cast<f32x4*>(Cf + (int64_t)m * p.ldc + c1) = v1[rr];
+          }
+          if (ok0) {
+            const f32x4 o = (v0[rr] - mean[rr]) * rstd[rr] * g0 + b0;
+            if (MODE == 1 && Lf) *reinterpret_cast<f32x4*>(Lf + (int64_t)m * p.ld_ln_f32 + c0) = o;
+            if (MODE == 0 || Lh) *reinterpret_cast<half4_t*>(Lh + (int64_t)m * p.ld_ln + c0) = half4_t{(half_t)o[0], (half_t)o[1], (half_t)o[2], (half_t)o[3]};
+            if (MODE == 1 && La) {
+              const f32x4 w = o + a0[rr];
+              *reinterpret_cast<half4_t*>(La + (int64_t)m * p.ld_ln_add + c0) = half4_t{(half_t)w[0], (half_t)w[1], (half_t)w[2], (half_t)w[3]};
+            }
+          }
+          if (ok1) {
+            const f32x4 o = (v1[rr] - mean[rr]) * rstd[rr] * g1 + b1;
+            if (MODE == 1 && Lf) *reinterpret_cast<f32x4*>(Lf + (int64_t)m * p.ld_ln_f32 + c1) = o;
+            if (MODE == 0 || Lh) *reinterpret_cast<half4_t*>(Lh + (int64_t)m * p.ld_ln + c1) = half4_t{(half_t)o[0], (half_t)o[1], (half_t)o[2], (half_t)o[3]};
+            if (MODE == 1 && La) {
+              const f32x4 w = o + a1[rr];
+              *reinterpret_cast<half4_t*>(La + (int64_t)m * p.ld_ln_add + c1) = half4_t{(half_t)w[0], (half_t)w[1], (half_t)w[2], (half_t)w[3]};
+            }
+          }
         }
       }
     }
@@ -663,8 +727,18 @@
 int launch_rowln(const lmx_gemm_desc& d, hipStream_t st) {
   int dev;
   LMX_TRY(lmx_stream_device(st, &dev));
-  LMX_TRY(lmx_allow_lds(reinterpret_cast<const void*>(&gemm2_rowln_kernel), RL_SMEM, dev));
-  hipLaunchKernelGGL(gemm2_rowln_kernel, dim3((d.M + RL_BM - 1) / RL_BM), dim3(512), RL_SMEM, st, d);
+  const dim3 grid((d.M + RL_BM - 1) / RL_BM);
+#define LMX_RL(MODE)                                                                                      \
+  LMX_TRY(lmx_allow_lds(reinterpret_cast<const void*>(&gemm2_rowln_kernel<MODE>), RL_SMEM, dev)); \
+  hipLaunchKernelGGL(gemm2_rowln_kernel<MODE>, grid, dim3(512), RL_SMEM, st, d)
+  if (d.ln_group) {
+    LMX_RL(2);
+  } else if (d.C && d.ln_out && !d.ln_out_f32 && !d.ln_out_add) {
+    LMX_RL(0);
+  } else {
+    LMX_RL(1);
+  }
+#undef LMX_RL
   return lmx_launch_check("gemm2_rowln_kernel");
 }
 
diff --git a/vision-sam3-yolo-lameless_amd/csrc/sam.hip b/vision-sam3-yolo-lameless_amd/csrc/sam.hip
--- a/vision-sam3-yolo-lameless_amd/csrc/sam.hip
+++ b/vision-sam3-yolo-lameless_amd/csrc/sam.hip
@@ -118,6 +118,33 @@
       half4_t h = {(half_t)v[0], (half_t)v[1], (half_t)v[2], (half_t)v[3]};
       *reinterpret_cast<half4_t*>(reinterpret_cast<half_t*>(out) + r * ldo + c) = h;
     }
+  }
+}
+
+template <int IN_DT, bool HAS_B>
+__global__ __launch_bounds__(256) void add_bcast3_kernel(const void* __restrict__ av, int64_t lda, const float* __restrict__ b, int64_t ldb,
+                                                         int b_rows, const float* __restrict__ pe, int64_t ldp, int pe_rows,
+                                                         float* __restrict__ keys, int64_t ldk, half_t* __restrict__ keys16, int64_t ld16,
+                                                         half_t* __restrict__ kpe16, int64_t ldkp, int64_t rows, int D) {
+  const int cc = D / 4;
+  const int64_t total = rows * cc;
+  for (int64_t i = (int64_t)blockIdx.x * blockDim.x + threadIdx.x; i < total; i += (int64_t)gridDim.x * blockDim.x) {
+    const int c = (int)(i % cc) * 4;
+    const int64_t r = i / cc;
+    f32x4 v;
+    if (IN_DT == LMX_F32) {
+      v = *reinterpret_cast<const f32x4*>(reinterpret_cast<const float*>(av) + r * lda + c);
+    } else {
+      const half4_t hv = *reinterpret_cast<const half4_t*>(reinterpret_cast<const half_t*>(av) + r * lda + c);
+      v = f32x4{(float)hv[0], (float)hv[1], (float)hv[2], (float)hv[3]};
+    }
+    if (HAS_B) {
+      v += *reinterpret_cast<const f32x4*>(b + (r % b_rows) * ldb + c);
+      *reinterpret_cast<f32x4*>(keys + r * ldk + c) = v;
+    }
+    *reinterpret_cast<half4_t*>(keys16 + r * ld16 + c) = half4_t{(half_t)v[0], (half_t)v[1], (half_t)v[2], (half_t)v[3]};
+    const f32x4 w = v + *reinterpret_cast<const f32x4*>(pe + (r % pe_rows) * ldp + c);
+    *reinterpret_cast<half4_t*>(kpe16 + r * ldkp + c) = half4_t{(half_t)w[0], (half_t)w[1], (half_t)w[2], (half_t)w[3]};
   }
 }
 
@@ -482,6 +509,32 @@
   return lmx_launch_check("add_bcast_kernel");
 }
 
+extern "C" int lmx_k_add_bcast3(const void* a, int a_dtype, int64_t lda, const float* b, int64_t ldb, int b_rows, const float* pe,
+                                int64_t ldp, int pe_rows, float* keys, int64_t ldk, void* keys16, int64_t ld16, void* kpe16, int64_t ldkp,
+                                int64_t rows, int D, lmx_stream_t stream) {
+  LMX_REQUIRE(a && pe && keys16 && kpe16 && (!b || keys), "lmx_k_add_bcast3: null pointer");
+  LMX_REQUIRE(a_dtype == LMX_F32 || (a_dtype == LMX_F16 && b), "lmx_k_add_bcast3: a must be f32, or f16 with b given (a_dtype=%d)", a_dtype);
+  LMX_REQUIRE(rows > 0 && D > 0 && D % 4 == 0 && pe_rows > 0 && (!b || b_rows > 0), "lmx_k_add_bcast3: shape");
+  LMX_REQUIRE(lda >= D && ldp >= D && ld16 >= D && ldkp >= D && lda % 4 == 0 && ldp % 4 == 0 && ld16 % 4 == 0 && ldkp % 4 == 0 &&
+                  (!b || (ldb >= D && ldk >= D && ldb % 4 == 0 && ldk % 4 == 0)), "lmx_k_add_bcast3: strides");
+  LMX_REQUIRE(((((uintptr_t)a) & (a_dtype == LMX_F32 ? 15 : 7)) == 0) && aligned16(pe) && (!b || (aligned16(b) && aligned16(keys))) &&
+                  ((((uintptr_t)keys16) & 7) == 0) && ((((uintptr_t)kpe16) & 7) == 0), "lmx_k_add_bcast3: alignment");
+  hipStream_t st = reinterpret_cast<hipStream_t>(stream);
+  const int g = grid_for(rows * (D / 4));
+  half_t* k16 = reinterpret_cast<half_t*>(keys16);
+  half_t* kp16 = reinterpret_cast<half_t*>(kpe16);
+#define LMX_AB3(IN, HB) \
+  hipLaunchKernelGGL((add_bcast3_kernel<IN, HB>), dim3(g), dim3(256), 0, st, a, lda, b, ldb, b_rows, pe, ldp, pe_rows, keys, ldk, k16, ld16, kp16, ldkp, rows, D)
+  if (!b)
+    LMX_AB3(LMX_F32, false);
+  else if (a_dtype == LMX_F32)
+    LMX_AB3(LMX_F32, true);
+  else
+    LMX_AB3(LMX_F16, true);
+#undef LMX_AB3
+  return lmx_launch_check("add_bcast3_kernel");
+}
+
 extern "C" int lmx_k_hyper_mask(const void* up, const float* hyper, float* logits, int n, int G, int C, lmx_stream_t stream) {
   LMX_REQUIRE(up && hyper && logits, "lmx_k_hyper_mask: null pointer");
   LMX_REQUIRE(n > 0 && G > 0 && C > 0 && C % 8 == 0 && C <= 64 && aligned16(up), "lmx_k_hyper_mask: shape");
diff --git a/vision-sam3-yolo-lameless_amd/lmx/_lib.py b/vision-sam3-yolo-lameless_amd/lmx/_lib.py
--- a/vision-sam3-yolo-lameless_amd/lmx/_lib.py
+++ b/vision-sam3-yolo-lameless_amd/lmx/_lib.py
@@ -19,6 +19,8 @@
         ("H", C.c_int32), ("W_", C.c_int32), ("Cin", C.c_int32), ("conv_stride", C.c_int32),
         ("Ho", C.c_int32), ("Wo", C.c_int32), ("res_rows", C.c_int32), ("a_rep", C.c_int32), ("split_k", C.c_int32), ("split_stride", C.c_int64),
         ("ln_out", C.c_void_p), ("ln_gamma", C.c_void_p), ("ln_beta", C.c_void_p), ("ld_ln", C.c_int64), ("ln_eps", C.c_float),
+        ("ln_out_f32", C.c_void_p), ("ld_ln_f32", C.c_int64), ("ln_out_add", C.c_void_p), ("ld_ln_add", C.c_int64),
+        ("ln_add", C.c_void_p), ("ld_add", C.c_int64), ("ln_add_rows", C.c_int32), ("ln_group", C.c_int32),
     ]
 
 
@@ -94,6 +96,7 @@
     "lmx_h_hiera_bands": (_I, [C.POINTER(C.c_int), C.POINTER(C.c_int), _I, _I, _I, _I, C.POINTER(C.c_int)]),
     "lmx_k_band_join": (_I, [_VP, _VP, _VP, _I, _I, _I, _I, _I, _I, _VP]),
     "lmx_k_add_bcast":(_I, [_VP, _I, _I64, _VP, _I64, _I, _VP, _I, _I64, _I64, _I, _VP]),
+    "lmx_k_add_bcast3": (_I, [_VP, _I, _I64, _VP, _I64, _I, _VP, _I64, _I, _VP, _I64, _VP, _I64, _VP, _I64, _I64, _I, _VP]),
     "lmx_h_mask_features": (_I, [_VP, _I, _I, _VP]),
     "lmx_h_iou_matrix": (_I, [_VP, _I, _VP, _I, _VP]),
     "lmx_h_assign": (_I, [_VP, _I, _I, _VP, _VP]),
diff --git a/vision-sam3-yolo-lameless_amd/lmx/kernels.py b/vision-sam3-yolo-lameless_amd/lmx/kernels.py
--- a/vision-sam3-yolo-lameless_amd/lmx/kernels.py
+++ b/vision-sam3-yolo-lameless_amd/lmx/kernels.py
@@ -57,9 +57,10 @@
 
 
 def gemm_route(M, N, K, *, out_dtype=torch.float16, act=ACT_NONE, scale=False, res=False, res_rows=0, a_rep=1, pool_hw=None,
-               lda=None, ldc=None, ldr=None, ln_out=False, split_k=1):
+               lda=None, ldc=None, ldr=None, ln_out=False, split_k=1, ln_f32=False, ln_add=False, ln_add_out=None, ln_group=0, store=True):
     d = GemmDesc()
-    d.A = d.W = d.C = d.bias = _ROUTE_PTR
+    d.A = d.W = d.bias = _ROUTE_PTR
+    d.C = _ROUTE_PTR if store else None
     d.scale = _ROUTE_PTR if scale else None
     d.res = _ROUTE_PTR if res else None
     d.M, d.N, d.K = M, N, a_rep * K
@@ -73,6 +74,15 @@
     if ln_out:
         d.ln_out = d.ln_gamma = d.ln_beta = _ROUTE_PTR
         d.ld_ln, d.ln_eps = N, 1e-6
+    if ln_f32 or ln_add or ln_add_out or ln_group:
+        d.ln_gamma = d.ln_beta = _ROUTE_PTR
+        d.ln_eps, d.ln_group = 1e-6, ln_group
+    if ln_f32:
+        d.ln_out_f32, d.ld_ln_f32 = _ROUTE_PTR, N
+    if ln_add:
+        d.ln_add, d.ld_add, d.ln_add_rows = _ROUTE_PTR, N, M
+    if ln_add if ln_add_out is None else ln_add_out:
+        d.ln_out_add, d.ld_ln_add = _ROUTE_PTR, N
     if split_k > 1:
         d.split_k, d.split_stride = split_k, M * d.ldc
     return _route_name(_lib.load().lmx_h_gemm_route, C.byref(d))
@@ -118,6 +128,9 @@
 
 def gemm(a, w, bias=None, act=ACT_NONE, scale=None, res=None, out=None, out_dtype=torch.float16, res_rows=0, pool_hw=None, a_rep=1,
          ln_out=None):
+    lnd = ln_out if isinstance(ln_out, dict) else None
+    if lnd is not None:
+        return _gemm_ln(a, w, bias, res, out, lnd)
     dev = _dev(a, w, bias, scale, res, out, *(ln_out[:3] if ln_out is not None else ()))
     M, K, lda = _rows(a, "gemm A")
     N, K2, ldw = _rows(w, "gemm W")
@@ -163,6 +176,56 @@
     return out
 
 
+def _gemm_ln(a, w, bias, res, out, ln):
+    g, b = ln["gamma"], ln["beta"]
+    h, y, add, store, group = ln.get("f16"), ln.get("f32"), ln.get("add"), ln.get("store", True), ln.get("group", 0)
+    addend, h2 = add if add is not None else (None, None)
+    dev = _dev(a, w, bias, res, out, g, b, h, y, addend, h2)
+    M, K, lda = _rows(a, "gemm A")
+    N, K2, ldw = _rows(w, "gemm W")
+    if K2 != K or ldw != K2 or a.dtype != torch.float16 or w.dtype != torch.float16:
+        raise LmxError(f"gemm: A [M,K] and contiguous W [N,K] must be float16; A K={K}, W shape {tuple(w.shape)}")
+    if bias is not None and (bias.dtype != torch.float32 or bias.numel() != N):
+        raise LmxError("gemm: bias must be float32 [N]")
+    ng = group or N
+    if any(t.dtype != torch.float32 or t.numel() != ng or not t.is_contiguous() for t in (g, b)):
+        raise LmxError(f"gemm: ln_out's gamma and beta must be contiguous float32 [{ng}]")
+    d = GemmDesc()
+    d.A, d.W = a.data_ptr(), w.data_ptr()
+    d.bias = bias.data_ptr() if bias is not None else None
+    d.lda, d.M, d.N, d.K = lda, M, N, K
+    d.act, d.out_dtype, d.a_mode, d.a_rep = ACT_NONE, F32, 0, 1
+    d.ln_gamma, d.ln_beta, d.ln_eps, d.ln_group = g.data_ptr(), b.data_ptr(), float(ln["eps"]), group
+
+    def rows_of(t, what, dtype):
+        Mt, Nt, ld = _rows(t, what)
+        if (Mt, Nt) != (M, N) or t.dtype != dtype:
+            raise LmxError(f"gemm: {what} must be {dtype} [{M},{N}], got {t.dtype} {tuple(t.shape)}")
+        return t.data_ptr(), ld
+
+    if store and not group:
+        if out is None:
+            out = torch.empty((M, N), dtype=torch.float32, device=a.device)
+        d.C, d.ldc = rows_of(out, "out", torch.float32)
+    elif out is not None:
+        raise LmxError("gemm: ln_out store=False / group writes no `out`")
+    if res is not None:
+        d.res, d.ldr = rows_of(res, "residual", torch.float32)
+    if h is not None:
+        d.ln_out, d.ld_ln = rows_of(h, "ln_out f16", torch.float16)
+    if y is not None:
+        d.ln_out_f32, d.ld_ln_f32 = rows_of(y, "ln_out f32", torch.float32)
+    if addend is not None:
+        ar, an, ld_add = _rows(addend, "gemm ln_out addend")
+        if an != N or addend.dtype != torch.float32:
+            raise LmxError(f"gemm: ln_out's addend must be float32 [rows,{N}]")
+        d.ln_add, d.ld_add, d.ln_add_rows = addend.data_ptr(), ld_add, ar
+    if h2 is not None:
+        d.ln_out_add, d.ld_ln_add = rows_of(h2, "ln_out add f16", torch.float16)
+    check(_lib.load().lmx_k_gemm(C.byref(d), _stream(dev)), "lmx_k_gemm")
+    return out if store and not group else None
+
+
 def im2col_u8(img, lut, IH, IW, KH, KW, stride, pad, ldo):
     dev = _dev(img, lut)
     n, rh, rw, c = img.shape
@@ -729,6 +792,26 @@
     return out
 
 
+def add_bcast3(a, b, pe):
+    dev = _dev(a, b, pe)
+    rows, D_, lda = _rows(a, "add_bcast3 a")
+    pe_rows, Dp, ldp = _rows(pe, "add_bcast3 pe")
+    if Dp != D_ or a.dtype not in _DT or pe.dtype != torch.float32 or (b is None and a.dtype != torch.float32):
+        raise LmxError("add_bcast3: a must be float16/float32 (float32 without b), pe float32, equal width")
+    b_rows, ldb, keys = 0, 0, a
+    if b is not None:
+        b_rows, Db, ldb = _rows(b, "add_bcast3 b")
+        if Db != D_ or b.dtype != torch.float32:
+            raise LmxError("add_bcast3: b must be float32 of a's width")
+        keys = torch.empty((rows, D_), dtype=torch.float32, device=a.device)
+    keys16 = torch.empty((rows, D_), dtype=torch.float16, device=a.device)
+    kpe16 = torch.empty((rows, D_), dtype=torch.float16, device=a.device)
+    check(_lib.load().lmx_k_add_bcast3(_ptr(a), _DT[a.dtype], lda, _ptr(b), ldb, b_rows, _ptr(pe), ldp, pe_rows,
+                                       _ptr(keys if b is not None else None), keys.stride(0), _ptr(keys16), D_, _ptr(kpe16), D_, rows, D_,
+                                       _stream(dev)), "lmx_k_add_bcast3")
+    return keys, keys16, kpe16
+
+
 def attention_f32(q, k, v, B, H, Tq, Tk, hd, scale):
     dev = _dev(q, k, v)
     for t in (q, k, v):
@@ -928,10 +1011,12 @@
         a_bytes = 2 * M * (Kd // max(d.a_rep, 1))
         if d.a_mode == 1:
             a_bytes = 2 * (M // max(d.Ho * d.Wo, 1)) * d.H * d.W_ * d.Cin
-        by = a_bytes + 2 * N * Kd + osz * (M // 4 if d.a_mode == 2 else M) * (N // 2 if d.act == ACT_SWIGLU else N) + (osz * (d.res_rows or M) * N if d.res else 0)
-        by += 2 * M * N if d.ln_out else 0
+        by = a_bytes + 2 * N * Kd + (osz * (M // 4 if d.a_mode == 2 else M) * (N // 2 if d.act == ACT_SWIGLU else N) if d.C else 0) + (osz * (d.res_rows or M) * N if d.res else 0)
+        by += (2 * M * N if d.ln_out else 0) + (4 * M * N if d.ln_out_f32 else 0) + ((2 * M + 4 * min(M, d.ln_add_rows)) * N if d.ln_out_add else 0)
         fl = 2.0 * M * N * Kd
-        key = f"gemm M={M} N={N} K={Kd} out={'f32' if osz == 4 else 'f16'} conv3x3={d.a_mode} act={d.act} res={int(bool(d.res))}" + (" ln_out" if d.ln_out else "")
+        ln_key = "".join(t for t, on in ((" ln_out", d.ln_out), (" ln_f32", d.ln_out_f32), (" ln_add", d.ln_out_add), (f" ln_group={d.ln_group}", d.ln_group),
+                                         (" no_store", not d.C)) if on)
+        key = f"gemm M={M} N={N} K={Kd} out={'f32' if osz == 4 else 'f16'} conv3x3={d.a_mode} act={d.act} res={int(bool(d.res))}" + ln_key
         return ("gemm/mfma-bound" if fl / by >= RIDGE_FLOP_PER_BYTE else "gemm/hbm-bound"), fl, by, key
     if name == "lmx_k_attention":
         d = args[0]._obj
@@ -974,6 +1059,9 @@
     if name == "lmx_k_add_bcast":
         a_dt, o_dt, rows, D = args[1], args[7], args[9], args[10]
         return "streaming glue", 0.0, rows * D * ((4 if a_dt == F32 else 2) + (4 if o_dt == F32 else 2)), f"add_bcast rows={rows} D={D}"
+    if name == "lmx_k_add_bcast3":
+        a_dt, has_b, pe_rows, rows, D = args[1], bool(args[3] and args[3].value), args[8], args[15], args[16]
+        return "streaming glue", 0.0, rows * D * ((4 if a_dt == F32 else 2) + (4 if has_b else 0) + 2 + 2) + 4 * min(rows, pe_rows) * D, f"add_bcast3 rows={rows} D={D} keys={int(has_b)}"
     if name == "lmx_k_band_join":
         dt, n_, H, Hb, W, D = args[3:9]
         return "streaming glue", 0.0, 2 * (4 if dt == F32 else 2) * n_ * H * W * D, f"band_join n={n_} H={H} Hb={Hb} W={W} D={D} dtype={dt}"
diff --git a/vision-sam3-yolo-lameless_amd/lmx/sam_decoder.py b/vision-sam3-yolo-lameless_amd/lmx/sam_decoder.py
--- a/vision-sam3-yolo-lameless_amd/lmx/sam_decoder.py
+++ b/vision-sam3-yolo-lameless_amd/lmx/sam_decoder.py
@@ -134,6 +134,9 @@
                                     w2=(t16(sd[p + "mlp.lin2.weight"]), t32(sd[p + "mlp.lin2.bias"])),
                                     ln3=ln(p + "layer_norm3."), ln4=ln(p + "layer_norm4."),
                                     i2t=attn(p + "cross_attn_image_to_token.")))
+            t2i, i2t = self.layers[-1]["t2i"], self.layers[-1]["i2t"]
+            self.layers[-1]["kq"] = (torch.cat([t2i["k_proj"][0], i2t["q_proj"][0]], 0).contiguous(),
+                                     torch.cat([t2i["k_proj"][1], i2t["q_proj"][1]], 0).contiguous())
         self.final = attn("mask_decoder.transformer.final_attn_token_to_image.")
         self.ln_final = ln("mask_decoder.transformer.layer_norm_final_attn.")
         w1 = sd["mask_decoder.upscale_conv1.weight"]
@@ -148,14 +151,16 @@
         self.hypers = [ffn(f"mask_decoder.output_hypernetworks_mlps.{m}.") for m in range(4)]
         self.iou_head = ffn("mask_decoder.iou_prediction_head.")
 
-    def _attn(self, W, q16, k16, v16, n, tq, tk, res):
-        q = K.gemm(q16, *W["q_proj"])
-        k = K.gemm(k16, *W["k_proj"])
+    def _attn(self, W, q16, k16, v16, n, tq, tk, res, q=None, k=None, ln=None):
+        q = K.gemm(q16, *W["q_proj"]) if q is None else q
+        k = K.gemm(k16, *W["k_proj"]) if k is None else k
         v = K.gemm(v16, *W["v_proj"])
         inner = q.shape[1]
         hd = inner // HEADS
         a = torch.empty((n * tq, inner), dtype=torch.float16, device=q.device)
         K.attention(q, k, v, a, n, HEADS, tq, tk, hd, hd ** -0.5)
+        if ln is not None:
+            return K.gemm(a, W["out_proj"][0], bias=W["out_proj"][1], res=res, ln_out=ln)
         return K.gemm(a, W["out_proj"][0], bias=W["out_proj"][1], res=res, out_dtype=torch.float32)
 
     @staticmethod
@@ -170,8 +175,8 @@
         sel = (0,) if masks is None else tuple(masks)
         eps = 1e-6
         tokens = torch.cat([self.out_tokens[None].expand(n, -1, -1), sparse], dim=1).reshape(n * T, D).contiguous()
-        if keys is None:
-            keys = K.add_bcast(emb, self.no_mask)
+        owned = keys is None
+        keys, keys16, k16 = K.add_bcast3(emb, self.no_mask, self.key_pe) if owned else K.add_bcast3(keys, None, self.key_pe)
         queries, qpe = tokens, tokens
         for i, L in enumerate(self.layers):
             if i == 0:
@@ -182,24 +187,27 @@
                 queries = self._attn(L["sa"], q16, q16, K.cast_f16(queries), n, T, T, queries)
             queries = K.layernorm(queries, *L["ln1"], eps, out_dtype=torch.float32)
             q16 = K.add_bcast(queries, qpe, out_dtype=torch.float16)
-            k16 = K.add_bcast(keys, self.key_pe, out_dtype=torch.float16)
-            queries = self._attn(L["t2i"], q16, k16, K.cast_f16(keys), n, T, P, queries)
+            kq = K.gemm(k16, *L["kq"])
+            queries = self._attn(L["t2i"], q16, None, keys16, n, T, P, queries, k=kq[:, :D // 2])
             queries = K.layernorm(queries, *L["ln2"], eps, out_dtype=torch.float32)
             h = K.gemm(K.cast_f16(queries), *L["w1"], act=K.ACT_RELU)
             queries = K.gemm(h, *L["w2"], res=queries, out_dtype=torch.float32)
             queries = K.layernorm(queries, *L["ln3"], eps, out_dtype=torch.float32)
             q16 = K.add_bcast(queries, qpe, out_dtype=torch.float16)
-            keys = self._attn(L["i2t"], k16, q16, K.cast_f16(queries), n, P, T, keys)
-            keys = K.layernorm(keys, *L["ln4"], eps, out_dtype=torch.float32)
+            last = i == len(self.layers) - 1
+            keys_ln = None if last else keys if owned else torch.empty_like(keys)
+            keys16, k16 = torch.empty_like(keys16), torch.empty_like(k16)
+            self._attn(L["i2t"], None, q16, K.cast_f16(queries), n, P, T, keys, q=kq[:, D // 2:],
+                       ln=dict(gamma=L["ln4"][0], beta=L["ln4"][1], eps=eps, f32=keys_ln, f16=keys16, add=(self.key_pe, k16), store=False))
+            keys, owned = keys_ln, True
         q16 = K.add_bcast(queries, qpe, out_dtype=torch.float16)
-        k16 = K.add_bcast(keys, self.key_pe, out_dtype=torch.float16)
-        keys16 = K.cast_f16(keys)
         queries = self._attn(self.final, q16, k16, keys16, n, T, P, queries)
         queries = K.layernorm(queries, *self.ln_final, 1e-5, out_dtype=torch.float32)
         q3 = queries.view(n, T, D)
         iou_tok = K.cast_f16(q3[:, 0].contiguous())
-        u = K.gemm(keys16, *self.up1, out_dtype=torch.float32)
-        u = K.layernorm(u.view(n * P * 4, 64), *self.up_ln, eps, act=K.ACT_GELU)
+        u = torch.empty((n * P, 4 * 64), dtype=torch.float16, device=keys16.device)
+        K.gemm(keys16, *self.up1, ln_out=dict(gamma=self.up_ln[0], beta=self.up_ln[1], eps=eps, f16=u, group=64))
+        u = u.view(n * P * 4, 64)
         u = K.gemm(u, *self.up2, act=K.ACT_GELU)
         hs = [self._ffn(self.hypers[m], K.cast_f16(q3[:, 1 + m].contiguous())) for m in sel]
         hyper = hs[0][:, None] if len(hs) == 1 else torch.stack(hs, 1)
```

Result: no change. 807.3 frames/s, median of 6 (+0.6%).
